# MiRaCLeXeoN/sduss

Hardware: AMD Instinct MI355X
Metric: images/sec (node), SDXL 1024^2 50-step, fixed prompt, CFG (higher is better)
Workload: dtype bf16; 1 GPU; SDXL-base-1.0 UNet 1024x1024 50-step Euler, CFG 5.0, 4 requests/step (denoiser batch 8) per GPU, is_sliced=False, random-init weights of the real architecture (2.57 B params), one data-parallel replica per GPU, no collective; resolution=1024, steps_per_image=50

## Files before the change

include/mxdenoise.h:

```cpp
#ifndef MXDENOISE_H
#define MXDENOISE_H

#include <stddef.h>
#include <stdint.h>

#ifdef __cplusplus
extern "C" {
#endif

enum { MX_F32 = 0, MX_F16 = 1, MX_BF16 = 2 };

const char* mx_last_error(void);
int mx_version(void);
#define MX_PROF_KINDS 12
int mx_profile_enable(int on);
int mx_profile_collect(double* out);
int mx_profile_records(double* out, int max_records);

size_t mx_groupnorm_halo_workspace_bytes(int N, int C, int cpg);
int mx_groupnorm_halo(void* stream, const void* x, const void* gamma, const void* beta, void* y,
                      int N, int C, int H, int W, int cpg, double eps, int padding,
                      const int32_t* latent_offset, int n_latents, const int32_t* patch_map,
                      const int32_t* padding_idx, int dtype, void* workspace);
int mx_halo_only(void* stream, const void* x, void* y, int N, int C, int H, int W,
// ... 67 lines not shown
  const mx_gemm_seg* segs;
  int n_segs;
  int splitk;
  const float* ln_final;
  float* ln_final_out;
  unsigned* ln_final_cnt;
  float* gn_part_out;
  int cin_valid;
} mx_gemm_desc;

int mx_gemm(void* stream, const mx_gemm_desc* d);
int mx_gemm_launches(const mx_gemm_desc* d);
int mx_gemm_stats_slabs(const mx_gemm_desc* d);
int mx_gemm_ln_prefers_pass(const mx_gemm_desc* d);
int mx_gemm_ln_final_supported(const mx_gemm_desc* d);
int mx_gemm_gn_partials_supported(const mx_gemm_desc* d, int conv);
enum { MX_FORM_TILE_GENERIC = 0, MX_FORM_TILE_256 = 1, MX_FORM_TILE_128 = 2, MX_FORM_PERSISTENT_256 = 3, MX_FORM_SMALL_M = 4, MX_FORM_CONV_SMALL_N = 5, MX_FORM_CONV_SMALL_CIN = 6 };
int mx_gemm_form(const mx_gemm_desc* d, int conv);
int mx_gemm_kernel_name(const mx_gemm_desc* d, int conv, int launch, char* buf, int cap);
int mx_gemm_kernel_names(char* buf, int cap);
int mx_attention_kernel_name(int B, int H, int Lq, int Lk, int ldo, int prescaled, int causal, int bias, int key_chunk, int force_cross, char* buf, int cap);
int mx_attention_kernel_names(char* buf, int cap);
#define MX_STATS_PITCH(slabs) (((slabs) + 3) & ~3)
int mx_row_stats(void* stream, const void* x, int ldx, float* stats, int M, int C);
int mx_conv3x3(void* stream, const mx_gemm_desc* d);
int mx_gemm_splitk(const mx_gemm_desc* d, int conv);
void mx_gemm_release_scratch(void* stream, int all);

typedef struct mx_attn_tail_desc {
  mx_gemm_desc out1, to_q, out2;
  const void* k; int ldk;
  const void* vt; int ldvt; int64_t vt_batch_stride;
  int B, heads, L, ctx_len;
  unsigned* sync;
} mx_attn_tail_desc;
size_t mx_attn_tail_sync_bytes(int M);
int mx_attn_tail_supported(const mx_attn_tail_desc* d);
int mx_attn_tail_preferred(void);
int mx_attn_tail(void* stream, const mx_attn_tail_desc* d);
int mx_attn_tail_status(void* stream, const unsigned* sync, unsigned* word);

#define MX_VT_POS(key) (((key) & ~12) | (((key) & 4) << 1) | (((key) & 8) >> 1))
#define MX_VT_LD(Lk) (((Lk) + 15) / 16 * 16)

int mx_attention(void* stream, const void* q, int ldq, const void* k, int ldk, const void* vt, int ldvt,
                 int64_t vt_batch_stride, void* o, int ldo, int B, int H, int Lq, int Lk, float scale);
#define MX_ATTN_QSCALE(scale) ((scale) * 1.4426950408889634f)
int mx_attention_prescaled(void* stream, const void* q, int ldq, const void* k, int ldk, const void* vt, int ldvt,
                           int64_t vt_batch_stride, void* o, int ldo, int B, int H, int Lq, int Lk);
int mx_attention_cross_prescaled(void* stream, const void* q, int ldq, const void* k, int ldk, const void* vt, int ldvt,
                                 int64_t vt_batch_stride, void* o, int ldo, int B, int H, int Lq, int Lk);
typedef struct mx_attn_problem {
  const void* q; const void* k; const void* vt; void* o;
  int64_t vt_batch_stride;
  int B, Lq, Lk, ldvt;
} mx_attn_problem;
int mx_attention_prescaled_grouped(void* stream, const mx_attn_problem* probs, int n, int ldq, int ldk, int ldo, int H);
int mx_attention_prescaled_bias(void* stream, const void* q, int ldq, const void* k, int ldk, const void* vt, int ldvt,
                                int64_t vt_batch_stride, void* o, int ldo, int B, int H, int Lq, int Lk, const float* bias, int ldb);
int mx_attention_prescaled_causal(void* stream, const void* q, int ldq, const void* k, int ldk, const void* vt, int ldvt,
                                  int64_t vt_batch_stride, void* o, int ldo, int B, int H, int L);

int mx_layernorm(void* stream, const void* x, void* y, const float* gamma, const float* beta,
                 int M, int C, float eps);

int mx_rmsnorm(void* stream, const void* x, void* y, const float* w, int M, int C, float eps);

int mx_layernorm_mod(void* stream, const void* x, void* y, void* y2, const float* scale, const float* shift,
                     const float* scale2, const float* shift2, int ldmod, int M, int C, int rows_per_batch, float eps);
int mx_layernorm_mod_grouped(void* stream, const void* x, void* y, void* y2, const float* scale, const float* shift, const float* scale2,
                             const float* shift2, int ldmod, int C, float eps, const int* batches, const int* rows_per_batch, int n);
int mx_rmsnorm_heads(void* stream, void* x, int ld, int nbatch, int rows_per_batch, int batch_rows, int row_off,
                     int heads_total, int heads_q, const float* wq, const float* wk, float eps, float q_scale);

size_t mx_groupnorm_nhwc_workspace_bytes(int B, int H, int W, int C);
int mx_groupnorm_nhwc(void* stream, const void* x, void* y, const float* gamma, const float* beta,
                      int B, int H, int W, int C, int groups, float eps, int silu, int patch,
                      void* workspace);

int mx_groupnorm_nhwc_cat(void* stream, const void* x, int C1, const void* x2, void* y, const float* gamma, const float* beta,
                          int B, int H, int W, int C, int groups, float eps, int silu, int patch, void* workspace);
int mx_groupnorm_nhwc_from_partials(void* stream, const void* x, void* y, const float* gamma, const float* beta, int B, int H, int W, int C, int groups, float eps,
                                    int silu, const float* part, int chunk, const float* add_bias, const float* add_rowbias, int ldrb, void* workspace);

typedef struct mx_gn_problem { const void* x; const void* x2; void* y; int B, H, W; } mx_gn_problem;
size_t mx_groupnorm_nhwc_grouped_workspace_bytes(const mx_gn_problem* probs, int n, int C);
int mx_groupnorm_nhwc_grouped(void* stream, const mx_gn_problem* probs, int n, int C1, const float* gamma, const float* beta, int C, int groups,
                              float eps, int silu, int patch, void* workspace);

typedef struct mx_unet_config {
  int in_channels, out_channels;
  int n_levels;
  int block_out_channels[4];
  int layers_per_block;
  int down_has_attn[4];
  int transformer_layers[4];
  int num_heads[4];
  int cross_attention_dim;
  int addition_time_embed_dim;
  int projection_class_embeddings_input_dim;
  int norm_num_groups;
  float norm_eps, transformer_norm_eps, layer_norm_eps;
} mx_unet_config;

typedef struct mx_weight_entry {
  const char* name;
  uint64_t offset;
  uint64_t bytes;
} mx_weight_entry;

typedef struct mx_unet mx_unet;

mx_unet* mx_unet_create(const mx_unet_config* cfg);
void mx_unet_destroy(mx_unet* u);
int mx_unet_set_weights(mx_unet* u, const void* blob, uint64_t blob_bytes,
                        const mx_weight_entry* table, int n_entries);
int mx_unet_set_context_key(mx_unet* u, uint64_t key);
int mx_unet_context_stats(const mx_unet* u, long* hits, long* misses);
size_t mx_unet_workspace_bytes(const mx_unet* u, int batch, int H, int W, int ctx_len);
int mx_unet_validate(const mx_unet* u, int batch, int H, int W, int ctx_len);
int mx_unet_forward(mx_unet* u, void* stream, const void* latents, int io_dtype, const float* timesteps,
                    const void* ehs, const void* text_embeds, const float* time_ids, void* out,
                    int batch, int H, int W, int ctx_len, int gn_patch, void* workspace, size_t workspace_bytes);
typedef struct mx_unet_group { const void* latents; void* out; int batch, H, W; } mx_unet_group;
size_t mx_unet_workspace_bytes_mixed(const mx_unet* u, const mx_unet_group* groups, int n_groups, int ctx_len);
int mx_unet_forward_mixed(mx_unet* u, void* stream, const mx_unet_group* groups, int n_groups, int io_dtype, const float* timesteps,
                          const void* ehs, const void* text_embeds, const float* time_ids, int ctx_len, int gn_patch, void* workspace,
                          size_t workspace_bytes);
int mx_unet_forward_mixed_trace(mx_unet* u, void* stream, const mx_unet_group* groups, int n_groups, int io_dtype, const float* timesteps,
                                const void* ehs, const void* text_embeds, const float* time_ids, int ctx_len, int gn_patch, void* workspace,
                                size_t workspace_bytes, const char* stage, void* stage_out, size_t stage_out_bytes);
int mx_unet_forward_trace(mx_unet* u, void* stream, const void* latents, int io_dtype, const float* timesteps,
                          const void* ehs, const void* text_embeds, const float* time_ids, void* out,
                          int batch, int H, int W, int ctx_len, int gn_patch, void* workspace,
                          size_t workspace_bytes, const char* stage, void* stage_out, size_t stage_out_bytes);

typedef int (*mx_allgather_fn)(void* ctx, void* stream, const void* send, void* recv, size_t bytes_per_rank);
typedef struct mx_pp_comm { int rank, world; mx_allgather_fn all_gather; void* ctx; } mx_pp_comm;
size_t mx_unet_workspace_bytes_pp(const mx_unet* u, int batch, int H_local, int W, int ctx_len, int world);
int mx_unet_forward_pp(mx_unet* u, void* stream, const void* latents_local, int io_dtype, const float* timesteps, const void* ehs,
                       const void* text_embeds, const float* time_ids, void* out_local, int batch, int H_local, int W, int ctx_len,
                       const mx_pp_comm* comm, void* workspace, size_t workspace_bytes);
#define MX_PP_SYNC 0
#define MX_PP_WARMUP 1
#define MX_PP_STALE 2
typedef int (*mx_allgather_inplace_fn)(void* ctx, void* stream, void* region, size_t bytes_per_rank);
typedef struct mx_pp_stale { void* state; size_t state_bytes; int mode; int corrected_gn; mx_allgather_inplace_fn all_gather_async; } mx_pp_stale;
size_t mx_unet_pp_state_bytes(const mx_unet* u, int batch, int H_local, int W, int ctx_len, int world);
int mx_unet_forward_pp_stale(mx_unet* u, void* stream, const void* latents_local, int io_dtype, const float* timesteps, const void* ehs,
                             const void* text_embeds, const float* time_ids, void* out_local, int batch, int H_local, int W, int ctx_len,
                             const mx_pp_comm* comm, const mx_pp_stale* stale, void* workspace, size_t workspace_bytes);
int mx_unet_pp_comm_plan(const mx_unet* u, int batch, int H_local, int W, int ctx_len, const mx_pp_comm* comm);
int mx_attention_prescaled_chunked(void* stream, const void* q, int ldq, const void* k, int ldk, const void* vt, int ldvt,
                                   int64_t vt_batch_stride, void* o, int ldo, int B, int H, int Lq, int Lk, int key_chunk,
                                   int64_t k_batch_stride, int64_t k_chunk_stride, int64_t vt_chunk_stride);

typedef struct mx_mmdit_config {
  int patch_size, in_channels, out_channels;
  int num_layers;
  int num_attention_heads;
  int joint_attention_dim, pooled_projection_dim, pos_embed_max_size;
  int dual_attention[64];
  float norm_eps;
} mx_mmdit_config;

typedef struct mx_mmdit mx_mmdit;
// ... 124 lines not shown
```

sduss_amd/csrc/gemm_args.h:

```cpp
#pragma once
#include "common.h"
#include "../../include/mxdenoise.h"

namespace mx {

constexpr int kMaxSegs = MX_MAX_SEGS;
struct GemmSeg {
  const bf16_t* a; const bf16_t* a2; void* c; const bf16_t* residual; bf16_t* vt; const float* rowbias; const float* gate;
  const float* ln_stats; float* stats_out;
  int M, tile0, rows_per_batch, ldvt;
  int B, Hin, Win, Hout, Wout;
  int a_batch_rows, a_row_off, c_batch_rows, c_row_off;
};

struct GemmArgs {
  const bf16_t* a;
  const bf16_t* w;
  void* c;
  const float* bias;
  const float* rowbias;
  const bf16_t* residual;
  bf16_t* vt;
  int M, N, K;
  int lda, ldc, ldr, ldrb;
// ... 351 lines not shown
        v[0] += bf16lo_to_f32(r[0]); v[1] += bf16hi_to_f32(r[0]);
        v[2] += bf16lo_to_f32(r[1]); v[3] += bf16hi_to_f32(r[1]);
      }
      if (flags & MX_EPI_SILU) {
#pragma unroll
        for (int q = 0; q < 4; ++q) v[q] = silu_f(v[q]);
      }
      if (flags & MX_EPI_GELU_TANH) {
#pragma unroll
        for (int q = 0; q < 4; ++q) v[q] = gelu_tanh_f(v[q]);
      }
      if (flags & (MX_EPI_GELU | MX_EPI_QUICK_GELU)) {
#pragma unroll
        for (int q = 0; q < 4; ++q) v[q] = (flags & MX_EPI_GELU) ? gelu_fast(v[q]) : quick_gelu_f(v[q]);
      }
      if (qkv) {
        const int nin = n - seg_idx * p.seg;
        if (to_vt) {
          const int key0 = (p.c_batch_rows > 0 ? p.c_row_off : 0) + m - bidx * p.rows_per_batch;
          const int key = MX_VT_POS(key0);
          const int nv = p.N / p.period;
          bf16_t* dst = p.vt + ((long)bidx * nv + (long)seg_grp * p.seg + nin) * p.ldvt + key;
#pragma unroll
          for (int q = 0; q < 4; ++q) dst[(long)q * p.ldvt] = f32_to_bf16(v[q]);
        } else {
          const int ccol = seg_grp * (p.period - 1) * p.seg + seg_pos * p.seg + nin;
          u32x2 o = {pack_bf16x2(v[0], v[1]), pack_bf16x2(v[2], v[3])};
          *reinterpret_cast<u32x2*>(reinterpret_cast<bf16_t*>(p.c) + orow * p.ldc + ccol) = o;
        }
        continue;
      }
      if (flags & MX_EPI_OUT_F32) {
        f32x4 o = {v[0], v[1], v[2], v[3]};
        *reinterpret_cast<f32x4*>(reinterpret_cast<float*>(p.c) + orow * p.ldc + n) = o;
      } else {
        u32x2 o = {pack_bf16x2(v[0], v[1]), pack_bf16x2(v[2], v[3])};
        *reinterpret_cast<u32x2*>(reinterpret_cast<bf16_t*>(p.c) + orow * p.ldc + n) = o;
      }
    }
  }
}


__device__ __forceinline__ void gemm_tile_of_block(const int b, const int mt, const int nt, const int xcd_map, int& tm, int& tn) {
  constexpr int MB = 4;
  if (!xcd_map || (mt & 7) != 0) { tm = b % mt; tn = b / mt; return; }
  const int xcd = b & 7;
  const int local = b >> 3;
  const int mloc = mt >> 3;
  const int band_tiles = MB * nt;
  const int band = local / band_tiles;
  const int r = local - band * band_tiles;
  const int rows = (mloc - band * MB) < MB ? (mloc - band * MB) : MB;
  tn = r / rows;
  tm = ((band * MB + (r - tn * rows)) << 3) + xcd;
}

__device__ __forceinline__ void lane_exchange_pair(float (&a)[4], float (&b)[4]) {
#pragma unroll
  for (int d = 0; d < 4; ++d) {
    unsigned x = __float_as_uint(a[d]), y = __float_as_uint(b[d]);
    auto r = __builtin_amdgcn_permlane32_swap(x, y, false, false);
    auto t = __builtin_amdgcn_permlane16_swap(r[0], r[1], false, false);
    a[d] = __uint_as_float(t[0]);
    b[d] = __uint_as_float(t[1]);
  }
}

__device__ __forceinline__ u32x4 lane_xor1(const u32x4 x) {
  u32x4 r;
#pragma unroll
  for (int d = 0; d < 4; ++d) r[d] = (unsigned)__builtin_amdgcn_update_dpp(0, (int)x[d], 0xB1, 0xF, 0xF, true);
  return r;
}

constexpr int EPI_F_QKV = 1;
constexpr int EPI_F_ACT = 2;
constexpr int EPI_F_ALL = 3;
constexpr int EPI_F_TANH = 4;
__host__ __device__ inline int gemm_epi_features(int flags) {
  const int acts = flags & (MX_EPI_SILU | MX_EPI_GELU | MX_EPI_GELU_TANH | MX_EPI_QUICK_GELU | MX_EPI_GEGLU_TANH);
  return ((flags & MX_EPI_QKV) ? EPI_F_QKV : 0) | (acts == 0 ? 0 : acts == MX_EPI_GELU_TANH ? EPI_F_TANH : EPI_F_ACT);
}
template <int NI, int MI, bool GEGLU, bool VEC = true, bool VPF = true, bool STATS = true, int FEAT = EPI_F_ALL, bool EMIT = STATS, bool RSTD_LOAD = false, bool WT = false>
__device__ __forceinline__ void gemm_epilogue_regs(const GemmArgs& p, f32x4 (&acc)[NI][MI], const int m_wave0, const int wave_n0,
                                                   const int fr, const int fq, const float (&ln_rstd_a)[MI]) {
#pragma clang fp contract(off)
  constexpr int NIO = GEGLU ? NI / 2 : NI;
  constexpr int NP = NIO / 2;
  constexpr bool ODD = (NIO & 1) != 0;
  constexpr int DEPTH = MI <= 4 ? MI : 2;
  static_assert(!GEGLU || NI % 4 == 0, "GEGLU: hidden and gate halves must be whole pairs");
  const int flags = p.flags;
  constexpr bool ACT = (FEAT & EPI_F_ACT) != 0;
  constexpr bool TANH = (FEAT & (EPI_F_ACT | EPI_F_TANH)) != 0;
  const bool qkv = (FEAT & EPI_F_QKV) != 0 && (flags & MX_EPI_QKV) != 0;
  int seg_idx = 0, seg_grp = 0, seg_pos = 0;
  bool to_vt = false;
  if (qkv) {
    seg_idx = wave_n0 / p.seg;
    seg_grp = seg_idx / p.period;
    seg_pos = seg_idx - seg_grp * p.period;
    to_vt = seg_pos == p.period - 1;
  }
  const bool rms = qkv && (flags & MX_EPI_RMSNORM) && !to_vt;
  const float w_scale = (!rms && p.out_scale != 0.f && (!qkv || seg_pos == 0)) ? p.out_scale : 1.0f;
  const int col0 = GEGLU ? wave_n0 / 2 : qkv ? seg_grp * (p.period - 1) * p.seg + seg_pos * p.seg + (wave_n0 - seg_idx * p.seg) : wave_n0;
  const bool has_res = !GEGLU && p.residual != nullptr;
  const bool has_rb = VEC && !GEGLU && p.rowbias != nullptr, has_gate = VEC && !GEGLU && p.gate != nullptr;

  f32x4 bias_r[NI];
#pragma unroll
  for (int i = 0; i < NI; ++i) {
    bias_r[i] = f32x4{0.f, 0.f, 0.f, 0.f};
    if (p.bias && (GEGLU || i < NIO)) bias_r[i] = *reinterpret_cast<const f32x4*>(p.bias + wave_n0 + i * 16 + fq * 4);
  }
  f32x4 rmsw_r[NI];
  if (rms) {
    const float* w = seg_pos == 0 ? p.rms_wq : p.rms_wk;
#pragma unroll
    for (int i = 0; i < NI; ++i) rmsw_r[i] = *reinterpret_cast<const f32x4*>(w + ((wave_n0 - seg_idx * p.seg + i * 16 + fq * 4) & 63));
  }
  const bool stats = EMIT && !GEGLU && !qkv && p.stats_out != nullptr;

  if constexpr ((FEAT & EPI_F_QKV) != 0) {
    if (qkv && to_vt) {
      const int rpb_v = p.rows_per_batch > 0 ? p.rows_per_batch : 0x7fffffff;
      const int m_first = m_wave0 + fr;
      int bv = p.rows_per_batch > 0 ? m_first / p.rows_per_batch : 0;
      int rv = m_first - bv * (p.rows_per_batch > 0 ? p.rows_per_batch : 0);
      const int key_off = p.c_batch_rows > 0 ? p.c_row_off : 0;
      const int nv = p.N / p.period;
      const long feat0 = (long)seg_grp * p.seg + (wave_n0 - seg_idx * p.seg) + fq * 4;
      auto rstd_at = [&](int j) __attribute__((always_inline)) -> float {
        const int m = m_first + 16 * j;
        return p.ln_final[(long)(m < p.M ? m : p.M - 1) * 2 + 1];
      };
      float rs_next = RSTD_LOAD ? rstd_at(0) : 1.0f;
#pragma unroll
      for (int j = 0; j < MI; ++j) {
        const float rs_cur = rs_next;
        if (RSTD_LOAD && j + 1 < MI) rs_next = rstd_at(j + 1);
        if (m_first + 16 * j < p.M) {
          const int key = MX_VT_POS(key_off + rv);
          bf16_t* dst = p.vt + ((long)bv * nv + feat0) * p.ldvt + key;
          const float rs = RSTD_LOAD ? rs_cur : STATS ? ln_rstd_a[j] : 1.0f;
#pragma unroll
          for (int i = 0; i < NIO; ++i) {
            const f32x4 t = STATS ? fma4(acc[i][j], rs, bias_r[i]) : acc[i][j] + bias_r[i];
#pragma unroll
            for (int q = 0; q < 4; ++q) dst[(long)(i * 16 + q) * p.ldvt] = f32_to_bf16(t[q]);
          }
        }
        rv += 16;
        if (rv >= rpb_v) { rv -= rpb_v; ++bv; }
      }
      return;
    }
  }
  const bool odd_lane = (fr & 1) != 0;
  const int rpb = p.rows_per_batch > 0 ? p.rows_per_batch : 0x7fffffff;
  const int cbr = p.c_batch_rows > 0 ? p.c_batch_rows : (p.rows_per_batch > 0 ? p.rows_per_batch : 0);
  const int cro = p.c_batch_rows > 0 ? p.c_row_off : 0;
  const int b_last = p.rows_per_batch > 0 ? (p.M - 1) / p.rows_per_batch : 0;
  const int r_last = p.M - 1 - b_last * (p.rows_per_batch > 0 ? p.rows_per_batch : 0);
  const int row_last = b_last * cbr + cro + r_last;
  const int mA0 = (m_wave0 + fr) & ~1;
  int row_a[MI], row_b[MI];
  int bo_walk = 0, ro_walk = 0;
  {
    int bA = p.rows_per_batch > 0 ? mA0 / p.rows_per_batch : 0;
    int rA = mA0 - bA * (p.rows_per_batch > 0 ? p.rows_per_batch : 0);
#pragma unroll
    for (int j = 0; j < MI; ++j) {
      int bB = bA, rB = rA + 1;
      if (rB >= rpb) { rB = 0; ++bB; }
      const int mA = mA0 + 16 * j;
      row_a[j] = mA < p.M ? bA * cbr + cro + rA : row_last;
      row_b[j] = mA + 1 < p.M ? bB * cbr + cro + rB : row_last;
      if constexpr (VEC) { if (j == 0) { bo_walk = odd_lane ? bB : bA; ro_walk = odd_lane ? rB : rA; } }
      rA += 16;
      if (rA >= rpb) { rA -= rpb; ++bA; }
    }
  }
  auto token = [&](int j) __attribute__((always_inline)) { return m_wave0 + j * 16 + fr; };
  auto row_own = [&](int j) __attribute__((always_inline)) { return odd_lane ? row_b[j] : row_a[j]; };
  const char* const res_base = reinterpret_cast<const char*>(p.residual);
  char* const c_base = reinterpret_cast<char*>(p.c);
  const unsigned ldr_b = (unsigned)p.ldr * 2u, ldc_b = (unsigned)p.ldc * 2u;
  auto res_at = [&](int row, int col) __attribute__((always_inline)) { return res_base + (unsigned long long)(unsigned)row * ldr_b + (unsigned)(col * 2); };
  auto c_at = [&](int row, int col) __attribute__((always_inline)) { return c_base + (unsigned long long)(unsigned)row * ldc_b + (unsigned)(col * 2); };
  const auto c_rsrc = __builtin_amdgcn_make_buffer_rsrc(p.c, 0, WT ? (int)((unsigned)p.M * ldc_b) : 0, 0x00020000);
  auto store_c16 = [&](int row, int col, const u32x4 v) __attribute__((always_inline)) {
    if constexpr (WT) __builtin_amdgcn_raw_buffer_store_b128(v, c_rsrc, (int)((unsigned)row * ldc_b + (unsigned)(col * 2)), 0, 16);
    else *reinterpret_cast<u32x4*>(c_at(row, col)) = v;
  };
  auto store_c8 = [&](int row, int col, const u32x2 v) __attribute__((always_inline)) {
    if constexpr (WT) __builtin_amdgcn_raw_buffer_store_b64(v, c_rsrc, (int)((unsigned)row * ldc_b + (unsigned)(col * 2)), 0, 16);
    else *reinterpret_cast<u32x2*>(c_at(row, col)) = v;
  };

  auto load_res = [&](int j, int pr) __attribute__((always_inline)) -> u32x4 {
    if (!has_res) return u32x4{0u, 0u, 0u, 0u};
    return *reinterpret_cast<const u32x4*>(res_at(row_own(j), col0 + pr * 32 + fq * 8));
  };
  auto load_res_odd = [&](int j) __attribute__((always_inline)) -> u32x2 {
// ... 10 lines not shown
#pragma unroll
      for (int i = 0; i < NIO; ++i) {
        const int n = wave_n0 + i * 16 + fq * 4;
        if (has_rb) rb_r[i] = *reinterpret_cast<const f32x4*>(p.rowbias + (long)bidx * p.ldrb + n);
        if (has_gate) gate_r[i] = *reinterpret_cast<const f32x4*>(p.gate + (long)bidx * p.ldg + n);
      }
    }
  };
  if constexpr (VPF) { if (has_rb || has_gate) load_batch_vectors(0); }
  constexpr int NG = NP / 2;
  constexpr bool fullmode = NG > 0;
  const int col_full = col0 + (odd_lane ? 32 : 0) + fq * 8;
  auto load_res_full = [&](int j, int g, int which) __attribute__((always_inline)) -> u32x4 {
    if (!has_res) return u32x4{0u, 0u, 0u, 0u};
    return *reinterpret_cast<const u32x4*>(res_at(which ? row_b[j] : row_a[j], col_full + 64 * g));
  };
  auto load_res_any = [&](int j, int pr) __attribute__((always_inline)) -> u32x4 {
    if (pr < 2 * NG) return load_res_full(j, pr >> 1, pr & 1);
    return load_res(j, pr);
  };
  u32x4 res_r[DEPTH][NP > 0 ? NP : 1];
  u32x2 res_o[DEPTH];
  {
#pragma unroll
    for (int d = 0; d < DEPTH && d < MI; ++d) {
#pragma unroll
      for (int pr = 0; pr < NP; ++pr) res_r[d][pr] = load_res_any(d, pr);
      if constexpr (ODD) res_o[d] = load_res_odd(d);
    }
  }

  auto rstd_at = [&](int j) __attribute__((always_inline)) -> float {
    const int m = token(j);
    return p.ln_final[(long)(m < p.M ? m : p.M - 1) * 2 + 1];
  };
  float rstd_next = RSTD_LOAD ? rstd_at(0) : 1.0f;
#pragma unroll
  for (int j = 0; j < MI; ++j) {
    const int m = token(j);
    float v[NIO][4];
    float rms_mul = 1.0f;
    if constexpr (!VPF) { if (has_rb || has_gate) load_batch_vectors(j); }
    const float rstd_cur = rstd_next;
    if (RSTD_LOAD && j + 1 < MI) rstd_next = rstd_at(j + 1);
    const float ln_rstd = RSTD_LOAD ? rstd_cur : STATS ? ln_rstd_a[j] : 1.0f;
    float st1 = 0.f, st2 = 0.f;
    if (rms) {
      float ss = 0.f;
#pragma unroll
      for (int i = 0; i < NI; ++i)
#pragma unroll
        for (int q = 0; q < 4; ++q) { const float t = acc[i][j][q] + bias_r[i][q]; ss = fmaf(t, t, ss); }
      ss = sum_over_fq(ss);
      rms_mul = rsqrtf(fmaf(ss, 1.0f / 64.0f, p.rms_eps)) * ((seg_pos == 0 && p.out_scale != 0.f) ? p.out_scale : 1.0f);
    }
#pragma unroll
    for (int i = 0; i < NIO; ++i) {
      f32x4 t = STATS ? fma4(acc[i][j], ln_rstd, bias_r[i]) : acc[i][j] + bias_r[i];
      if constexpr (GEGLU) {
        const f32x4 g = STATS ? fma4(acc[i + NI / 2][j], ln_rstd, bias_r[i + NI / 2]) : acc[i + NI / 2][j] + bias_r[i + NI / 2];
        if (ACT && (flags & MX_EPI_GEGLU_TANH)) {
#pragma unroll
          for (int q = 0; q < 4; ++q) t[q] = t[q] * gelu_tanh_f(g[q]);
        } else {
          const gelu_f32x2 g01 = gelu_fast2(gelu_f32x2{g[0], g[1]}), g23 = gelu_fast2(gelu_f32x2{g[2], g[3]});
          t[0] *= g01[0]; t[1] *= g01[1]; t[2] *= g23[0]; t[3] *= g23[1];
        }
      } else {
        if (rms) {
#pragma unroll
          for (int q = 0; q < 4; ++q) t[q] *= rms_mul * rmsw_r[i][q];
        } else {
          t *= w_scale;
        }
        if constexpr (VEC) {
          if (has_rb) t += rb_r[i];
          if (has_gate) t *= gate_r[i];
        }
      }
#pragma unroll
      for (int q = 0; q < 4; ++q) v[i][q] = t[q];
    }
    if constexpr (VPF) { if (j + 1 < MI && (has_rb || has_gate)) load_batch_vectors(j + 1); }
    auto finish8 = [&](float (&o)[8], const u32x4 rr) __attribute__((always_inline)) {
      if (has_res) {
#pragma unroll
        for (int q = 0; q < 4; ++q) { o[2 * q] += bf16lo_to_f32(rr[q]); o[2 * q + 1] += bf16hi_to_f32(rr[q]); }
      }
      if (ACT && (flags & MX_EPI_SILU)) {
#pragma unroll
        for (int q = 0; q < 8; ++q) o[q] = silu_f(o[q]);
      }
      if (TANH && (flags & MX_EPI_GELU_TANH)) {
#pragma unroll
        for (int q = 0; q < 8; q += 2) { const gelu_f32x2 t2 = gelu_tanh2(gelu_f32x2{o[q], o[q + 1]}); o[q] = t2[0]; o[q + 1] = t2[1]; }
      }
      if (ACT && (flags & (MX_EPI_GELU | MX_EPI_QUICK_GELU))) {
#pragma unroll
        for (int q = 0; q < 8; ++q) o[q] = (flags & MX_EPI_GELU) ? gelu_fast(o[q]) : quick_gelu_f(o[q]);
      }
      if (stats) {
#pragma unroll
        for (int q = 0; q < 8; ++q) { st1 += o[q]; st2 = fmaf(o[q], o[q], st2); }
      }
    };
    if constexpr (fullmode) {
      const bool ok_a = (m & ~1) < p.M, ok_b = (m | 1) < p.M;
#pragma unroll
      for (int g = 0; g < NG; ++g) {
        lane_exchange_pair(v[4 * g], v[4 * g + 1]);
        lane_exchange_pair(v[4 * g + 2], v[4 * g + 3]);
        float oa[8], ob[8];
#pragma unroll
        for (int q = 0; q < 4; ++q) { oa[q] = v[4 * g][q]; oa[4 + q] = v[4 * g + 1][q]; ob[q] = v[4 * g + 2][q]; ob[4 + q] = v[4 * g + 3][q]; }
        const u32x4 ra = res_r[j % DEPTH][2 * g], rb = res_r[j % DEPTH][2 * g + 1];
        if (j + DEPTH < MI) { res_r[j % DEPTH][2 * g] = load_res_full(j + DEPTH, g, 0); res_r[j % DEPTH][2 * g + 1] = load_res_full(j + DEPTH, g, 1); }
        u32x4 res_a = ra, res_b = rb;
        if (has_res) {
          const u32x4 nb_ra = lane_xor1(ra), nb_rb = lane_xor1(rb);
          res_a = odd_lane ? nb_rb : ra;
          res_b = odd_lane ? rb : nb_ra;
        }
        finish8(oa, res_a);
        finish8(ob, res_b);
        const u32x4 wa = {pack_bf16x2(oa[0], oa[1]), pack_bf16x2(oa[2], oa[3]), pack_bf16x2(oa[4], oa[5]), pack_bf16x2(oa[6], oa[7])};
        const u32x4 wb = {pack_bf16x2(ob[0], ob[1]), pack_bf16x2(ob[2], ob[3]), pack_bf16x2(ob[4], ob[5]), pack_bf16x2(ob[6], ob[7])};
        const u32x4 nb_b = lane_xor1(wb), nb_a = lane_xor1(wa);
        const u32x4 st_a = odd_lane ? nb_b : wa;
        const u32x4 st_b = odd_lane ? wb : nb_a;
        if (ok_a) store_c16(row_a[j], col_full + 64 * g, st_a);
        if (ok_b) store_c16(row_b[j], col_full + 64 * g, st_b);
      }
    }
#pragma unroll
    for (int pr = 2 * NG; pr < NP; ++pr) {
      lane_exchange_pair(v[2 * pr], v[2 * pr + 1]);
      float o[8];
#pragma unroll
      for (int q = 0; q < 4; ++q) { o[q] = v[2 * pr][q]; o[4 + q] = v[2 * pr + 1][q]; }
      const u32x4 rr = res_r[j % DEPTH][pr];
      if (j + DEPTH < MI) res_r[j % DEPTH][pr] = load_res(j + DEPTH, pr);
      finish8(o, rr);
      if (m < p.M) {
        const u32x4 w = {pack_bf16x2(o[0], o[1]), pack_bf16x2(o[2], o[3]), pack_bf16x2(o[4], o[5]), pack_bf16x2(o[6], o[7])};
        store_c16(row_own(j), col0 + pr * 32 + fq * 8, w);
      }
    }
    if constexpr (ODD) {
      float o[4];
#pragma unroll
      for (int q = 0; q < 4; ++q) o[q] = v[NIO - 1][q];
      const u32x2 rr = res_o[j % DEPTH];
      if (j + DEPTH < MI) res_o[j % DEPTH] = load_res_odd(j + DEPTH);
      if (has_res) { o[0] += bf16lo_to_f32(rr[0]); o[1] += bf16hi_to_f32(rr[0]); o[2] += bf16lo_to_f32(rr[1]); o[3] += bf16hi_to_f32(rr[1]); }
      if (ACT && (flags & MX_EPI_SILU)) {
#pragma unroll
        for (int q = 0; q < 4; ++q) o[q] = silu_f(o[q]);
      }
      if (TANH && (flags & MX_EPI_GELU_TANH)) {
#pragma unroll
        for (int q = 0; q < 4; q += 2) { const gelu_f32x2 t2 = gelu_tanh2(gelu_f32x2{o[q], o[q + 1]}); o[q] = t2[0]; o[q + 1] = t2[1]; }
      }
      if (ACT && (flags & (MX_EPI_GELU | MX_EPI_QUICK_GELU))) {
#pragma unroll
        for (int q = 0; q < 4; ++q) o[q] = (flags & MX_EPI_GELU) ? gelu_fast(o[q]) : quick_gelu_f(o[q]);
      }
      if (stats) {
#pragma unroll
        for (int q = 0; q < 4; ++q) { st1 += o[q]; st2 = fmaf(o[q], o[q], st2); }
      }
      if (m < p.M) store_c8(row_own(j), col0 + NP * 32 + fq * 4, u32x2{pack_bf16x2(o[0], o[1]), pack_bf16x2(o[2], o[3])});
    }
    if (stats) {
      st1 = sum_over_fq(st1); st2 = sum_over_fq(st2);
      if (fq == 0 && m < p.M) {
        const int slab = wave_n0 / (16 * NI), pitch = (p.N / (16 * NI) + 3) & ~3;
        float* dst = p.stats_out + ((long)m * pitch + slab) * 2;
        if (WT || p.ln_final_out != nullptr) {
          const unsigned long long bits = (unsigned long long)__float_as_uint(st1) | ((unsigned long long)__float_as_uint(st2) << 32);
          __hip_atomic_store(reinterpret_cast<unsigned long long*>(dst), bits, __ATOMIC_RELAXED, __HIP_MEMORY_SCOPE_AGENT);
        } else {
          *reinterpret_cast<f32x2*>(dst) = f32x2{st1, st2};
        }
      }
    }
  }
}

}
```

sduss_amd/csrc/gemm_bf16.hip:

```cpp
#include <algorithm>
#include <cstdlib>

#include <mutex>
#include <unordered_map>

#include "common.h"
#include "../../include/mxdenoise.h"
#include "gemm_args.h"
#include "gemm_forms.h"

namespace mx {

constexpr int BM = 128;
constexpr int BK = 64;

__device__ __forceinline__ int swz(int row, int chunk) { return chunk ^ ((row >> 1) & 7); }

template <int BN, bool CONV>
__global__ __launch_bounds__(256, 2) void gemm_kernel(const GemmArgs pk) {
  constexpr int NI = BN / 32;
  constexpr int MI = 4;
  constexpr int WROWS = BN / 32;
  __shared__ __attribute__((aligned(16))) bf16_t sX[2][BM * BK];
  __shared__ __attribute__((aligned(16))) bf16_t sW[2][BN * BK];
// ... 374 lines not shown
  a.vhalo = conv ? d->vhalo : 0;
  a.a2 = conv ? nullptr : (const bf16_t*)d->a2; a.lda2 = d->lda2; a.k_split = d->k_split;
  a.a = (const bf16_t*)d->a; a.w = (const bf16_t*)d->w; a.c = d->c;
  a.bias = d->bias; a.rowbias = d->rowbias; a.residual = (const bf16_t*)d->residual; a.vt = (bf16_t*)d->vt;
  a.M = d->M; a.N = d->N; a.K = d->K; a.lda = d->lda; a.ldc = d->ldc; a.ldr = d->ldr; a.ldrb = d->ldrb;
  a.rows_per_batch = d->rows_per_batch; a.flags = d->flags; a.seg = d->seg; a.period = d->period; a.ldvt = d->ldvt;
  a.B = d->B; a.Hin = d->Hin; a.Win = d->Win; a.Cin = d->Cin; a.Hout = d->Hout; a.Wout = d->Wout;
  a.stride = d->stride; a.up = d->up; a.corner_patch = d->corner_patch;
  a.a_batch_rows = d->a_batch_rows; a.a_row_off = d->a_row_off; a.c_batch_rows = d->c_batch_rows; a.c_row_off = d->c_row_off;
  a.gate = d->gate; a.ldg = d->ldg; a.out_scale = d->out_scale;
  a.rms_wq = d->rms_wq; a.rms_wk = d->rms_wk; a.rms_eps = d->rms_eps;
  a.ln_stats = d->ln_stats; a.ln_colsum = d->ln_colsum; a.ln_slabs = d->ln_slabs; a.ln_eps = d->ln_eps; a.stats_out = nullptr;
  a.ln_final = nullptr; a.ln_final_out = nullptr; a.ln_final_cnt = nullptr; a.ln_final_slabs = 0;
  if (d->ln_final) {
    MX_CHECK(!conv && !d->ln_stats && d->ln_colsum && d->n_segs == 0, "gemm: ln_final needs ln_colsum, excludes ln_stats and grouped launches (mx_gemm only)");
    MX_CHECK(!(d->flags & MX_EPI_RMSNORM) && d->a_batch_rows <= 0 && d->c_batch_rows <= 0 && !d->a2 && !d->rowbias && !d->gate && !d->stats_out,
             "gemm: ln_final excludes RMSNORM, the row remaps, the split A operand, per-sample vectors and stats_out");
    MX_CHECK((((uintptr_t)d->ln_final & 15) | ((uintptr_t)d->ln_colsum & 15)) == 0, "gemm: ln_final / ln_colsum must be 16-byte aligned");
    a.ln_final = d->ln_final;
  }
  a.nseg = d->n_segs; a.mt_total = 0;
  const bool grouped = d->n_segs > 0;
  if (d->ln_stats) {
    MX_CHECK(!conv && d->ln_colsum && d->ln_slabs > 0, "gemm: folded LayerNorm needs ln_colsum and ln_slabs > 0 (mx_gemm only)");
    MX_CHECK(!(d->flags & MX_EPI_RMSNORM) && d->a_batch_rows <= 0 && d->c_batch_rows <= 0 && !d->a2, "gemm: folded LayerNorm excludes RMSNORM, the row remaps and the split A operand");
    MX_CHECK((((uintptr_t)d->ln_stats & 15) | ((uintptr_t)d->ln_colsum & 15)) == 0, "gemm: ln_stats / ln_colsum must be 16-byte aligned");
  }
  a.xcd_map = 1;

  if (!conv && d->a2) {
    MX_CHECK(d->k_split > 0 && d->k_split < d->K && d->k_split % BK == 0, "gemm: k_split must be a multiple of 64 inside (0, K)");
    MX_CHECK(d->lda >= d->k_split && d->lda % 8 == 0 && d->lda2 >= d->K - d->k_split && d->lda2 % 8 == 0, "gemm: bad lda / lda2 for the split A operand");
    MX_CHECK(d->a_batch_rows <= 0 && ((uintptr_t)d->a2 & 15) == 0 && rows_of(d) * d->lda2 < 2147483647L, "gemm: split A operand excludes the row remap and needs 16-byte alignment");
  } else if (!conv) {
    MX_CHECK(d->lda >= d->K && d->lda % 8 == 0, "gemm: lda must be >= K and a multiple of 8");
  } else {
    MX_CHECK(d->Cin % BK == 0 && d->K == 9 * d->Cin, "conv3x3: Cin must be a multiple of 64 and K = 9*Cin");
    MX_CHECK(d->stride == 1 || d->stride == 2, "conv3x3: stride must be 1 or 2");
    MX_CHECK(d->up == 0 || d->up == 1, "conv3x3: up must be 0 or 1");
    MX_CHECK(!(d->up && d->stride != 1), "conv3x3: upsample only with stride 1");
    if (!grouped) {
      const int Hv = d->Hin << d->up, Wv = d->Win << d->up;
      MX_CHECK(d->Hout == (Hv + d->stride - 1) / d->stride && d->Wout == (Wv + d->stride - 1) / d->stride,
               "conv3x3: output grid does not match input grid / stride");
      MX_CHECK((long)d->B * d->Hout * d->Wout == d->M, "conv3x3: M != B*Hout*Wout");
    }
    MX_CHECK(2 * d->Cin <= 16384, "conv3x3: Cin > 8192 (the pipelined loader walks a 16 KB zero page for padding taps)");
    MX_CHECK(!(d->flags & MX_EPI_GEGLU), "conv3x3: no GEGLU epilogue");
    MX_CHECK(d->vhalo == 0 || (d->vhalo == 1 && d->corner_patch == 0), "conv3x3: vhalo must be 0 or 1 and excludes the sliced corner rule");
  }
  {
    const void* ptrs[] = {d->a, d->w, d->c, d->bias, d->rowbias, d->residual, d->gate, d->rms_wq, d->rms_wk};
    for (const void* q : ptrs) MX_CHECK(((uintptr_t)q & 15) == 0, "gemm: operand pointers must be 16-byte aligned");
  }
  if (!grouped && (d->rowbias || d->gate || d->a_batch_rows > 0 || d->c_batch_rows > 0 || (d->flags & (MX_EPI_QKV | MX_EPI_RES_BCAST))))
    MX_CHECK(d->rows_per_batch > 0, "gemm: rows_per_batch required");
  if (d->gate) MX_CHECK(d->ldg >= d->N && d->ldg % 4 == 0, "gemm: bad ldg");
  if (!grouped && d->a_batch_rows > 0) MX_CHECK(!conv && d->a_row_off >= 0 && d->a_row_off + d->rows_per_batch <= d->a_batch_rows, "gemm: bad input row remap");
  if (!grouped && d->c_batch_rows > 0) MX_CHECK(d->c_row_off >= 0 && d->c_row_off + d->rows_per_batch <= d->c_batch_rows, "gemm: bad output row remap");
  if (d->rowbias) MX_CHECK(d->ldrb >= d->N && d->ldrb % 4 == 0, "gemm: bad ldrb");
  if (!grouped) {
    const long in_rows = (!conv && d->a_batch_rows > 0) ? (long)(d->M / d->rows_per_batch + 1) * d->a_batch_rows : d->M;
    MX_CHECK(in_rows * (conv ? 1 : d->lda) < 2147483647L, "gemm: operand exceeds 32-bit indexing");
  }
  MX_CHECK((long)d->N * d->K < 2147483647L, "gemm: operand exceeds 32-bit indexing");
  if (d->residual) MX_CHECK(d->ldr >= d->N && d->ldr % 4 == 0, "gemm: bad ldr");
  const bool use128 = (d->N % 128 == 0);
  const TileChoice tc = pick_tile(d, conv);
  tc_out = tc;
  a.splitk = 0; a.sk_ws = nullptr; a.sk_cnt = nullptr;
  if (tc.splitk > 1) {
    SplitKScratch sk;
    MX_CHECK(splitk_scratch((hipStream_t)stream, sk), "gemm: the split-K scratch (96 MB per stream) could not be allocated; set mx_gemm_desc.splitk = 1 to run unsplit");
    a.splitk = tc.splitk; a.sk_ws = sk.ws; a.sk_cnt = sk.cnt;
  }
  if (d->stats_out) {
    MX_CHECK(stats_slabs_of(d, conv, tc) > 0, "gemm: stats_out is not supported for this shape / epilogue (see mx_gemm_stats_slabs)");
    MX_CHECK(((uintptr_t)d->stats_out & 15) == 0, "gemm: stats_out must be 16-byte aligned");
    a.stats_out = d->stats_out;
  }
  a.gn_part = nullptr;
  if (d->gn_part_out) {
    MX_CHECK(!grouped && tc.rows == 256 && tc.bn != 256 && tc.bn != 0 && tc.splitk <= 1, "gemm: gn_part_out needs an ungrouped launch on a 256-row tile (mx_gemm_gn_partials_supported)");
    MX_CHECK(d->flags == 0 && !d->residual && !d->gate && d->out_scale == 0.f && !d->ln_stats && !d->ln_final && d->a_batch_rows <= 0 && d->c_batch_rows <= 0,
             "gemm: gn_part_out needs an epilogue of bias (+ row bias) only");
    MX_CHECK(d->M % 64 == 0 && (!d->rowbias || d->rows_per_batch % 64 == 0) && ((uintptr_t)d->gn_part_out & 15) == 0, "gemm: gn_part_out needs M % 64 == 0, rows_per_batch % 64 == 0 and 16-byte alignment");
    a.gn_part = d->gn_part_out;
  }
  if (d->ln_final_out) {
    MX_CHECK(d->stats_out && d->ln_final_cnt && !grouped && tc.rows == 256 && tc.bn != 256 && tc.bn != 0,
             "gemm: ln_final_out needs stats_out, ln_final_cnt and an ungrouped launch on a 256-row tile (mx_gemm_ln_final_supported)");
    MX_CHECK((((uintptr_t)d->ln_final_out & 15) | ((uintptr_t)d->ln_final_cnt & 3)) == 0, "gemm: ln_final_out must be 16-byte aligned");
    a.ln_final_out = d->ln_final_out; a.ln_final_cnt = d->ln_final_cnt; a.ln_final_slabs = stats_slabs_of(d, conv, tc);
  }
  if (grouped) {
    const int rows = tc.rows > 0 ? tc.rows : BM;
    uintptr_t lo = (uintptr_t)d->segs[0].a;
    int t0 = 0;
    for (int i = 0; i < d->n_segs; ++i) {
      const mx_gemm_seg& g = d->segs[i];
      GemmSeg& o = a.prob[i];
      o.a = (const bf16_t*)g.a; o.a2 = conv ? nullptr : (const bf16_t*)g.a2; o.c = g.c; o.residual = (const bf16_t*)g.residual; o.vt = (bf16_t*)g.vt;
      o.rowbias = g.rowbias; o.gate = g.gate; o.ln_stats = g.ln_stats; o.stats_out = d->stats_out ? g.stats_out : nullptr;
      o.M = g.M; o.tile0 = t0; o.rows_per_batch = g.rows_per_batch; o.ldvt = g.ldvt;
      o.B = g.B; o.Hin = g.Hin; o.Win = g.Win; o.Hout = g.Hout; o.Wout = g.Wout;
      o.a_batch_rows = g.a_batch_rows; o.a_row_off = g.a_row_off; o.c_batch_rows = g.c_batch_rows; o.c_row_off = g.c_row_off;
      t0 += cdiv(g.M, rows);
      lo = std::min(lo, (uintptr_t)g.a);
    }
    a.mt_total = t0;
    a.a = (const bf16_t*)lo;
    a.M = (int)rows_of(d);
  }
  if (d->flags & MX_EPI_GEGLU) {
    MX_CHECK(use128, "gemm: GEGLU needs N % 128 == 0");
    MX_CHECK(!(d->flags & (MX_EPI_QKV | MX_EPI_OUT_F32)) && !d->residual && !d->rowbias && d->out_scale == 0.f, "gemm: GEGLU excludes other epilogues");
    MX_CHECK(d->ldc >= d->N / 2 && d->ldc % 4 == 0, "gemm: bad ldc for GEGLU");
  } else if (d->flags & MX_EPI_QKV) {
    MX_CHECK(d->seg > 0 && d->seg % 64 == 0 && d->period >= 2 && d->N % (d->seg * d->period) == 0, "gemm: bad QKV segments");
    MX_CHECK(d->vt != nullptr, "gemm: QKV needs vt");
    if (!grouped) {
      MX_CHECK(d->ldvt >= MX_VT_LD(d->c_batch_rows > 0 ? d->c_batch_rows : d->rows_per_batch), "gemm: QKV needs ldvt >= MX_VT_LD(keys per batch)");
      MX_CHECK(d->M % d->rows_per_batch == 0, "gemm: QKV needs M % rows_per_batch == 0");
    }
    MX_CHECK(d->ldc >= d->N / d->period * (d->period - 1) && d->ldc % 4 == 0, "gemm: bad ldc for QKV");
    MX_CHECK(!(d->flags & MX_EPI_OUT_F32), "gemm: QKV output is bf16");
    MX_CHECK(!d->rowbias && !d->gate && !d->residual, "gemm: QKV excludes the per-sample vectors and the residual (its V^T segment takes none of them)");
    if (d->flags & MX_EPI_RMSNORM)
      MX_CHECK(d->rms_wq && d->rms_wk && d->period == 3 && d->N % 128 == 0 && !conv, "gemm: RMSNORM needs rms_wq/rms_wk, period 3, N % 128 == 0");
  } else {
    MX_CHECK(d->ldc >= d->N && d->ldc % 4 == 0, "gemm: bad ldc");
  }
  return 0;
}

int gemm_prepare_for_chain(void* stream, const mx_gemm_desc* d, GemmArgs& a, int& bn, int& rows, int& splitk) {
  TileChoice tc;
  if (int rc = prepare(stream, d, false, a, tc)) return rc;
  bn = tc.bn; rows = tc.rows; splitk = tc.splitk;
  return 0;
}

static int launch(void* stream, const mx_gemm_desc* d, bool conv) {
  GemmArgs a;
  TileChoice tc;
  if (int rc = prepare(stream, d, conv, a, tc)) return rc;
  const bool grouped = d->n_segs > 0;
  const bool use128 = (d->N % 128 == 0);
  const int v2bn = tc.bn;
  dim3 block(256);
  hipStream_t s = (hipStream_t)stream;
  if (prof_enabled()) {
    const double kk = conv ? 9.0 * d->Cin : (double)d->K;
    const double Mt = (double)rows_of(d);
    double in_elems = conv ? (double)d->B * d->Hin * d->Win * d->Cin : Mt * d->K;
    if (conv && grouped) { in_elems = 0; for (int i = 0; i < d->n_segs; ++i) in_elems += (double)d->segs[i].B * d->segs[i].Hin * d->segs[i].Win * d->Cin; }
    const double flops = 2.0 * Mt * (double)d->N * kk;
    const double bytes = 2.0 * (in_elems + (double)d->N * d->K + Mt * d->N);
    const int kind = v2bn == 256 ? PROF_GEMM_V3_256 : v2bn ? (conv ? PROF_CONV_V2_160 : PROF_GEMM_V2_160) + (v2bn == 160 ? 0 : 2) : (conv ? PROF_CONV128 : PROF_GEMM128) + (use128 ? 0 : 1);
    prof_begin(s, kind, flops, bytes, (int)Mt, d->N, (int)kk);
  }
  const int mt128 = grouped ? a.mt_total : cdiv(d->M, BM);
  if (d->ln_final) MX_CHECK(v2bn == 256, "gemm: ln_final is the 256 x 256 kernel's form of the folded LayerNorm; this shape does not run there (use ln_stats)");
  const int form = gemm_kernel_of(d, conv, tc);
  MX_CHECK(form >= 0, v2bn == 256 ? "gemm: no 256 x 256 instantiation serves ln_final with this epilogue (GEGLU, QKV or plain bias only)"
                                   : "gemm: no kernel instantiation serves this descriptor");
  if (is_small_m_form(form)) {
    MX_CHECK(launch_small_m(s, a, form) == 0, "gemm: the small-M launcher was handed a form outside its list");
// ... 3 lines not shown
    launch_conv_small_cin(s, a);
  } else if (v2bn == 256) {
    MX_CHECK(launch_v4(s, a, form) == 0, "gemm: no 256 x 256 instantiation serves ln_final with this epilogue (GEGLU, QKV or plain bias only)");
  } else if (v2bn) {
    if (tc.rows == 256) MX_CHECK(launch_v5(s, a, v2bn, tc.rows, form) == 0, "gemm: the 256-row launcher was handed a form outside its list");
    else MX_CHECK(launch_v2(s, a, v2bn, form) == 0, "gemm: the 128-row launcher was handed a form outside its list");
  } else {
    const dim3 grid(mt128, use128 ? d->N / 128 : cdiv(d->N, 64));
    switch (form) {
#define MX_GEN(id, k, targs) case id: hipLaunchKernelGGL((k<MX_FORM_UNPAREN targs>), grid, block, 0, s, a); break;
      MX_GEMM_GENERIC_FORMS(MX_GEN)
#undef MX_GEN
      default: MX_CHECK(false, "gemm: the generic launcher was handed a form outside its list");
    }
  }
  prof_end(s);
  MX_LAUNCH_CHECK();
  return 0;
}

}

namespace mx {
static bool tail_split(const mx_gemm_desc* d, mx_gemm_desc& d1, mx_gemm_desc& d2) {
  if (d->n_segs != 0 || d->M <= 0 || d->N <= 0 || d->K <= 0 || d->N % 256 != 0) return false;
  if (d->flags & (MX_EPI_QKV | MX_EPI_OUT_F32 | MX_EPI_RES_BCAST | MX_EPI_RMSNORM)) return false;
  if (d->stats_out || d->ln_stats || d->ln_final || d->ln_final_out || d->a_batch_rows > 0 || d->c_batch_rows > 0 || d->splitk > 1) return false;
  if (pick_tile(d, false).bn != 256) return false;
  const int ncu = cu_count();
  if (ncu <= 0) return false;
  const long mt = cdiv(d->M, 256), nt = d->N / 256, tiles = mt * nt;
  const long full = tiles / ncu, rem = tiles % ncu;
  if (full < 1 || rem == 0 || rem * 2 > ncu || (full * ncu) % mt != 0) return false;
  const long nt1 = full * ncu / mt;
  if (nt1 <= 0 || nt1 >= nt) return false;
  const int N1 = (int)nt1 * 256, N2 = d->N - N1;
  const bool geglu = (d->flags & MX_EPI_GEGLU) != 0;
  const long cofs = geglu ? N1 / 2 : N1;
  d1 = *d; d2 = *d;
  d1.N = N1; d2.N = N2;
  d1.splitk = 1; d2.splitk = 1;
  d2.w = (const char*)d->w + (size_t)N1 * d->K * 2;
  if (d->bias) d2.bias = d->bias + N1;
  d2.c = (char*)d->c + (size_t)cofs * 2;
  if (geglu && d->residual) return false;
  if (d->residual) d2.residual = (const char*)d->residual + (size_t)N1 * 2;
  if (d->rowbias) d2.rowbias = d->rowbias + N1;
  if (d->gate) d2.gate = d->gate + N1;
  const TileChoice t2 = pick_tile(&d2, false);
  if (t2.bn == 0 || t2.bn == 256 || t2.rows + t2.bn > 384) return false;
  if (m_tiles_of(&d2, t2.rows) * (N2 / t2.bn) > ncu) return false;
  return pick_tile(&d1, false).bn == 256;
}
}

extern "C" int mx_gemm(void* stream, const mx_gemm_desc* d) {
  mx_gemm_desc d1, d2;
  if (d != nullptr && mx::tail_split(d, d1, d2)) { if (int rc = mx::launch(stream, &d1, false)) return rc; return mx::launch(stream, &d2, false); }
  return mx::launch(stream, d, false);
}
extern "C" int mx_gemm_launches(const mx_gemm_desc* d) { mx_gemm_desc d1, d2; return d != nullptr && mx::tail_split(d, d1, d2) ? 2 : 1; }
extern "C" int mx_gemm_form(const mx_gemm_desc* d, int conv) {
  if (!d || mx::rows_of(d) <= 0 || d->N <= 0 || d->K <= 0) return MX_FORM_TILE_GENERIC;
  if (mx::small_m_serves(d, conv != 0)) return MX_FORM_SMALL_M;
  if (conv && mx::conv_small_n_serves(d)) return MX_FORM_CONV_SMALL_N;
  if (conv && mx::conv_small_cin_serves(d)) return MX_FORM_CONV_SMALL_CIN;
  const mx::TileChoice tc = mx::pick_tile(d, conv != 0);
  return tc.bn == 256 ? MX_FORM_PERSISTENT_256 : tc.bn == 0 ? MX_FORM_TILE_GENERIC : tc.rows == 256 ? MX_FORM_TILE_256 : MX_FORM_TILE_128;
}
extern "C" int mx_gemm_stats_slabs(const mx_gemm_desc* d) {
  if (!d || mx::rows_of(d) <= 0 || d->N <= 0 || d->K <= 0) return 0;
  mx_gemm_desc q = *d;
  if (!q.stats_out) q.stats_out = reinterpret_cast<float*>(16);
  return mx::stats_slabs_of(&q, false, mx::pick_tile(&q, false));
}
extern "C" int mx_gemm_ln_prefers_pass(const mx_gemm_desc* d) {
  if (!d || mx::rows_of(d) <= 0 || d->N <= 0 || d->K <= 0) return 0;
  mx_gemm_desc plain = *d;
  plain.ln_stats = nullptr; plain.stats_out = nullptr;
  return mx::pick_tile(&plain, false).bn == 256;
}
extern "C" int mx_gemm_gn_partials_supported(const mx_gemm_desc* d, int conv) {
  if (!d || d->n_segs > 0 || d->M <= 0 || d->N <= 0 || d->K <= 0 || d->M % 64 != 0) return 0;
  if (d->flags != 0 || d->residual || d->gate || d->out_scale != 0.f || d->ln_stats || d->ln_final || d->a_batch_rows > 0 || d->c_batch_rows > 0) return 0;
  if (d->rowbias && (d->rows_per_batch <= 0 || d->rows_per_batch % 64 != 0)) return 0;
  const mx::TileChoice tc = mx::pick_tile(d, conv != 0);
  return tc.rows == 256 && tc.bn != 256 && tc.bn != 0 && tc.splitk <= 1;
}
extern "C" int mx_gemm_ln_final_supported(const mx_gemm_desc* d) {
  if (!d || d->n_segs > 0 || d->M <= 0 || d->N <= 0 || d->K <= 0) return 0;
  mx_gemm_desc q = *d;
  if (!q.stats_out) q.stats_out = reinterpret_cast<float*>(16);
  const mx::TileChoice tc = mx::pick_tile(&q, false);
  return tc.rows == 256 && tc.bn != 256 && tc.bn != 0 && mx::stats_slabs_of(&q, false, tc) > 0;
}
extern "C" int mx_conv3x3(void* stream, const mx_gemm_desc* d) { return mx::launch(stream, d, true); }
extern "C" void mx_gemm_release_scratch(void* stream, int all) { mx::splitk_release((hipStream_t)stream, all != 0); }
extern "C" int mx_gemm_splitk(const mx_gemm_desc* d, int conv) {
  if (!d || mx::rows_of(d) <= 0 || d->N <= 0 || d->K <= 0) return 0;
  return mx::pick_tile(d, conv != 0).splitk;
}

namespace mx {
static const char* const kGemmKernelNames[GK_COUNT] = {
  MX_GEMM_GENERIC_FORMS(MX_FORM_NAME_T) MX_GEMM_V2_FORMS(MX_FORM_NAME_T) MX_GEMM_V5_FORMS(MX_FORM_NAME_T) MX_GEMM_V4_FORMS(MX_FORM_NAME_T)
  MX_GEMM_SMALL_M_FORMS(MX_FORM_NAME_T) MX_GEMM_CONV_SMALL_FORMS(MX_FORM_NAME_P)
};
}
extern "C" int mx_gemm_kernel_name(const mx_gemm_desc* d, int conv, int launch, char* buf, int cap) {
  if (!d || mx::rows_of(d) <= 0 || d->N <= 0 || d->K <= 0 || launch < 0) return -1;
  mx_gemm_desc d1, d2;
  const mx_gemm_desc* q = d;
  if (!conv && mx::tail_split(d, d1, d2)) { if (launch > 1) return 0; q = launch == 0 ? &d1 : &d2; }
  else if (launch > 0) return 0;
  const int form = mx::gemm_kernel_of(q, conv != 0, mx::pick_tile(q, conv != 0));
  if (form < 0) return -1;
  return mx::copy_name(mx::kGemmKernelNames[form], buf, cap);
}
extern "C" int mx_gemm_kernel_names(char* buf, int cap) { return mx::join_names(mx::kGemmKernelNames, mx::GK_COUNT, buf, cap); }
```

sduss_amd/csrc/gemm_v5_body.h:

```cpp
#pragma once
#include "common.h"
#include "../../include/mxdenoise.h"
#include "gemm_args.h"
#include "gemm_dma_loader.h"

namespace mx {

constexpr int NSTAGE5 = 3;

#if defined(MX_EXP) && MX_EXP == 8
static __device__ unsigned long long g_v5_stamps[1024 * 2 * 4];
#define MX5_STAMP(slot) do { if (lane == 0 && (wave == 0 || wave == 7) && blockIdx.x < 1024) \
    g_v5_stamps[(blockIdx.x * 2 + (wave == 7)) * 4 + (slot)] = __builtin_amdgcn_s_memrealtime(); } while (0)
#else
#define MX5_STAMP(slot) do {} while (0)
#endif

template <int BN, int MI, bool CONV, int FEAT, bool GEGLU, bool VEC, bool WT = false>
__device__ __forceinline__ void gemm_v5_tile(const GemmArgs& pk, int tm, const int tn, bf16_t* const smem) {
  constexpr int BM5 = 64 * MI;
  constexpr int NI = BN / 32;
  constexpr int LOADS = DmaTile<BN, MI>::LOADS;

  const int tid = threadIdx.x;
  const int lane = tid & 63;
  const int wave = __builtin_amdgcn_readfirstlane(tid >> 6);
  const int wm = wave >> 1;
  const int wn = wave & 1;
  const bool group_b = wave >= 4;
  MX5_STAMP(0);
  GemmArgs p = pk;
  gemm_select_seg(p, pk, tm);
  const int nk = p.K / DMA_BK;
  constexpr bool SPLIT_K = false;
  constexpr int k_first = 0;
#include "gemm_dma_loader.inc"

  const int fr = lane & 15;
  const int fq = lane >> 4;
  unsigned wrd[2], xrd[2];
#pragma unroll
  for (int ks = 0; ks < 2; ++ks) {
    const int wrow = wn * (BN / 2) + fr, xrow = wm * 16 * MI + fr;
    wrd[ks] = (unsigned)(((BM5 * DMA_BK) + wrow * DMA_BK + swz(wrow, ks * 4 + fq) * 8) * 2);
    xrd[ks] = (unsigned)((xrow * DMA_BK + swz(xrow, ks * 4 + fq) * 8) * 2);
  }

  setup_tile();
  issue_group(0); advance_cursor();
  issue_group(1); advance_cursor();
  wait_vmcnt<LOADS>();

  f32x4 acc[NI][MI];
#pragma unroll
  for (int i = 0; i < NI; ++i)
#pragma unroll
    for (int j = 0; j < MI; ++j) acc[i][j] = f32x4{0.f, 0.f, 0.f, 0.f};
  float ln_rstd[MI];
#pragma unroll
  for (int j = 0; j < MI; ++j) ln_rstd[j] = 1.0f;
  if constexpr (!CONV) {
    if (p.ln_stats != nullptr) gemm_ln_init<NI, MI>(p, acc, tm * BM5 + wm * 16 * MI, tn * BN + wn * (BN / 2), fr, fq, ln_rstd);
  }
  MX_BAR();
  if (group_b) MX_BAR();
  MX5_STAMP(1);

  int stage = 0;
  for (int kt = 0; kt < nk; ++kt) {
    const char* sb = reinterpret_cast<const char*>(smem) + stage * (STAGE_ELEMS * 2);
    bf16x8 wf[2][NI], xf[2][MI];
#pragma unroll
    for (int ks = 0; ks < 2; ++ks) {
#pragma unroll
      for (int i = 0; i < NI; ++i) wf[ks][i] = *reinterpret_cast<const bf16x8*>(sb + wrd[ks] + i * (16 * DMA_BK * 2));
#pragma unroll
      for (int j = 0; j < MI; ++j) xf[ks][j] = *reinterpret_cast<const bf16x8*>(sb + xrd[ks] + j * (16 * DMA_BK * 2));
    }
    const int st2 = stage >= 1 ? stage - 1 : NSTAGE5 - 1;
    issue_group(st2);
    advance_cursor();
    wait_vmcnt<LOADS>();
    asm volatile("s_waitcnt lgkmcnt(0)" ::: "memory");
    __builtin_amdgcn_sched_barrier(0);
    MX_BAR();
    __builtin_amdgcn_s_setprio(1);
#pragma unroll
    for (int ks = 0; ks < 2; ++ks)
#pragma unroll
      for (int i = 0; i < NI; ++i)
#pragma unroll
        for (int j = 0; j < MI; ++j) acc[i][j] = __builtin_amdgcn_mfma_f32_16x16x32_bf16(wf[ks][i], xf[ks][j], acc[i][j], 0, 0, 0);
    __builtin_amdgcn_s_setprio(0);
    MX_BAR();
    stage = stage == NSTAGE5 - 1 ? 0 : stage + 1;
  }
  MX5_STAMP(2);
  if (!group_b) MX_BAR();

  const int m0 = tm * BM5, n0 = tn * BN;
  static_assert(!GEGLU || (NI % 4 == 0 && !CONV), "the gated epilogue pairs whole 32-feature halves");
  gemm_epilogue_regs<NI, MI, GEGLU, VEC, true, true, FEAT, true, false, WT>(p, acc, m0 + wm * 16 * MI, n0 + wn * (BN / 2), fr, fq, ln_rstd);
  if constexpr (!GEGLU && FEAT == 0 && MI == 4) {
    if (pk.gn_part != nullptr) gemm_gn_partials<NI, MI>(p, acc, m0 + wm * 16 * MI, n0 + wn * (BN / 2), fr, fq);
  }
  MX5_STAMP(3);
  wait_vmcnt<0>();
  if constexpr (!CONV && !GEGLU && BM5 == 256) {
    if (pk.ln_final_out != nullptr) gemm_ln_finalize(p, tm, pk.N / BN, reinterpret_cast<volatile int*>(smem));
  }
}


}
```

sduss_amd/csrc/norm.hip:

```cpp
#include <cstdlib>

#include "common.h"
#include "../../include/mxdenoise.h"

namespace mx {

struct GnGeom {
  int B, H, W, C;
  int tpr;
  int L;
  int th, tw;
  int tiles_y, tiles_x;
  const bf16_t* x2;
  int C1;
};

struct GnProb {
  GnGeom g;
  const bf16_t* x; bf16_t* y;
  float* part; float* coef;
  float* gpart;
  long y_img;
  int ppb;
  int patch;
};
struct GnGroup {
  GnProb p[MX_MAX_SEGS];
  int blk0[MX_MAX_SEGS + 1];
  int n;
};
__device__ __forceinline__ const GnProb& gn_locate(const GnGroup& G, int& local) {
  local = blockIdx.x;
  int s = 0;
#pragma unroll
  for (int i = 1; i < MX_MAX_SEGS; ++i) if (i < G.n && local >= G.blk0[i]) s = i;
  local -= G.blk0[s];
  return G.p[s];
}

__device__ __forceinline__ const bf16_t* gn_src(const bf16_t* x, const GnGeom& g, long pix, int ch) {
  if (g.x2 == nullptr) return x + pix * g.C + ch;
  return ch < g.C1 ? x + pix * g.C1 + ch : g.x2 + pix * (g.C - g.C1) + (ch - g.C1);
}

__global__ void gn_stats_kernel(const GnGroup G, const int groups) {
  extern __shared__ __attribute__((aligned(16))) float red[];
  const int t = threadIdx.x;
  int local;
  const GnProb& P = gn_locate(G, local);
  const GnGeom& g = P.g;
  const bf16_t* __restrict__ x = P.x;
  float* __restrict__ part = P.part;
  const int ntl = g.tiles_y * g.tiles_x;
  const int b = local / ntl;
  const int tile = local - b * ntl;
  const int ty = tile / g.tiles_x, tx = tile - ty * g.tiles_x;
  const int cv = t % g.tpr;
  const int pl = t / g.tpr;
  float s[8], ss[8];
#pragma unroll
  for (int e = 0; e < 8; ++e) { s[e] = 0.f; ss[e] = 0.f; }
  if (pl < g.L) {
    const int npix = g.th * g.tw;
    for (int pi = pl; pi < npix; pi += g.L) {
      const int py = pi / g.tw, px = pi - py * g.tw;
      const long pix = ((long)b * g.H + ty * g.th + py) * g.W + tx * g.tw + px;
      const u32x4 v = *reinterpret_cast<const u32x4*>(gn_src(x, g, pix, cv * 8));
#pragma unroll
      for (int e = 0; e < 4; ++e) {
        const float lo = bf16lo_to_f32(v[e]), hi = bf16hi_to_f32(v[e]);
        s[2 * e] += lo; ss[2 * e] += lo * lo;
        s[2 * e + 1] += hi; ss[2 * e + 1] += hi * hi;
      }
    }
#pragma unroll
    for (int e = 0; e < 8; ++e) {
      red[((long)pl * g.C + cv * 8 + e) * 2] = s[e];
      red[((long)pl * g.C + cv * 8 + e) * 2 + 1] = ss[e];
    }
  }
  __syncthreads();
  float* __restrict__ gpart = P.gpart;
  float* chs = red + (long)g.L * g.C * 2;
  for (int c = t; c < g.C; c += blockDim.x) {
    float a = 0.f, q = 0.f;
    for (int l = 0; l < g.L; ++l) { a += red[((long)l * g.C + c) * 2]; q += red[((long)l * g.C + c) * 2 + 1]; }
    if (gpart != nullptr) { chs[2 * c] = a; chs[2 * c + 1] = q; continue; }
    float* dst = part + (((long)b * (g.tiles_y * g.tiles_x) + tile) * g.C + c) * 2;
    dst[0] = a; dst[1] = q;
  }
  if (gpart != nullptr) {
    __syncthreads();
    const int cpg = g.C / groups;
    for (int gi = t; gi < groups; gi += blockDim.x) {
      float a = 0.f, q = 0.f;
      for (int i = 0; i < cpg; ++i) { a += chs[(gi * cpg + i) * 2]; q += chs[(gi * cpg + i) * 2 + 1]; }
      *reinterpret_cast<float2*>(gpart + (((long)b * ntl + tile) * groups + gi) * 2) = float2{a, q};
    }
  }
}

__device__ __forceinline__ double wave_sum_d(double v) {
#pragma unroll
  for (int o = 32; o > 0; o >>= 1) v += __shfl_xor(v, o, 64);
  return v;
}

constexpr int kFoldThreads = 256;
__global__ __launch_bounds__(kFoldThreads) void gn_fold_kernel(const GnGroup G, const float* __restrict__ gamma, const float* __restrict__ beta,
                                                               int groups, float eps, const float* __restrict__ add_bias = nullptr,
                                                               const float* __restrict__ add_rowbias = nullptr, int ldrb = 0) {
  int local;
  const GnProb& P = gn_locate(G, local);
  const GnGeom& g = P.g;
  const float* __restrict__ part = P.part;
  float* __restrict__ coef = P.coef;
  const int patch = P.patch;
  const int b = local / groups;
  const int grp = local - b * groups;
  const int cpg = g.C / groups;
  const int ntiles = g.tiles_y * g.tiles_x;
  const int lane = threadIdx.x;
  const int ppy = patch > 0 ? g.H / patch : 1;
  const int ppx = patch > 0 ? g.W / patch : 1;
  const int npatch = ppy * ppx;
  const int tpy = g.tiles_y / ppy, tpx = g.tiles_x / ppx;
  const int nitems = tpy * tpx * cpg;
  const double cnt = (double)tpy * tpx * g.th * g.tw * cpg;
  double acc_mean = 0.0, acc_var = 0.0;
  __shared__ double wsum[kFoldThreads / 64][2];
  for (int pidx = 0; pidx < npatch; ++pidx) {
    const int py = pidx / ppx, px = pidx - py * ppx;
    double s = 0.0, q = 0.0;
    for (int it = lane; it < nitems; it += kFoldThreads) {
      const int tl = it / cpg, c = it - tl * cpg;
      const int iy = tl / tpx, ix = tl - iy * tpx;
      const int tile = (py * tpy + iy) * g.tiles_x + px * tpx + ix;
      const float2 v = *reinterpret_cast<const float2*>(part + (((long)b * ntiles + tile) * g.C + grp * cpg + c) * 2);
      if (add_bias != nullptr) {
        const int chn = grp * cpg + c;
        const double cc = (double)add_bias[chn] + (add_rowbias != nullptr ? (double)add_rowbias[(long)b * ldrb + chn] : 0.0);
        const double npx = (double)(g.th * g.tw);
        s += (double)v.x + npx * cc;
        q += (double)v.y + 2.0 * cc * (double)v.x + npx * cc * cc;
      } else {
        s += (double)v.x;
        q += (double)v.y;
      }
    }
    s = wave_sum_d(s);
    q = wave_sum_d(q);
    __syncthreads();
    if ((lane & 63) == 0) { wsum[lane >> 6][0] = s; wsum[lane >> 6][1] = q; }
    __syncthreads();
    s = (wsum[0][0] + wsum[1][0]) + (wsum[2][0] + wsum[3][0]);
    q = (wsum[0][1] + wsum[1][1]) + (wsum[2][1] + wsum[3][1]);
    const double mean = s / cnt;
    double var = q / cnt - mean * mean;
    if (var < 0.0) var = 0.0;
    acc_mean += mean;
    acc_var += var;
  }
  const double mean = acc_mean / npatch;
  const double rstd = 1.0 / sqrt(acc_var / npatch + (double)eps);
  for (int c = lane; c < cpg; c += kFoldThreads) {
    const int ch = grp * cpg + c;
    const float sc = (float)(rstd * (double)gamma[ch]);
    const float sf = (float)((double)beta[ch] - rstd * (double)gamma[ch] * mean);
    coef[((long)b * g.C + ch) * 2] = sc;
    coef[((long)b * g.C + ch) * 2 + 1] = sf;
  }
}

constexpr int kFoldGroups = 64;
template <bool SILU, bool FOLD>
__global__ void gn_apply_kernel(const GnGroup G, const float* __restrict__ gamma, const float* __restrict__ beta, const int groups, const float eps) {
  const int t = threadIdx.x;
  int local;
  const GnProb& P = gn_locate(G, local);
  const GnGeom& g = P.g;
  const bf16_t* __restrict__ x = P.x;
  bf16_t* __restrict__ y = P.y;
  const float* __restrict__ coef = P.coef;
  const int pix_per_block = P.ppb;
  const long y_img = P.y_img;
  const int nblk = (g.H * g.W + pix_per_block - 1) / pix_per_block;
  const int b = local / nblk;
  const int pblk = local - b * nblk;
  const int cv = t % g.tpr;
  const int pl = t / g.tpr;
  float sc[8], sf[8];
  if constexpr (FOLD) {
    __shared__ double fsub[kFoldGroups][8][2];
    __shared__ double mr[kFoldGroups][2];
    const int ntl = g.tiles_y * g.tiles_x;
    const float* __restrict__ gp = P.gpart + (long)b * ntl * groups * 2;
    for (int it = t; it < groups * 8; it += blockDim.x) {
      const int gi = it >> 3, sub = it & 7;
      double s = 0.0, q = 0.0;
      for (int tl = sub; tl < ntl; tl += 8) {
        const float2 v = *reinterpret_cast<const float2*>(gp + ((long)tl * groups + gi) * 2);
        s += (double)v.x; q += (double)v.y;
      }
      fsub[gi][sub][0] = s; fsub[gi][sub][1] = q;
    }
    __syncthreads();
    const int cpg = g.C / groups;
    const double cnt = (double)g.H * g.W * cpg;
    for (int gi = t; gi < groups; gi += blockDim.x) {
      double s = 0.0, q = 0.0;
#pragma unroll
      for (int sub = 0; sub < 8; ++sub) { s += fsub[gi][sub][0]; q += fsub[gi][sub][1]; }
      const double mean = s / cnt;
      double var = q / cnt - mean * mean;
      if (var < 0.0) var = 0.0;
      mr[gi][0] = mean;
      mr[gi][1] = 1.0 / sqrt(var + (double)eps);
    }
    __syncthreads();
    if (pl >= g.L) return;
#pragma unroll
    for (int e = 0; e < 8; ++e) {
      const int ch = cv * 8 + e;
      const int gi = ch / cpg;
      const double rg = mr[gi][1] * (double)gamma[ch];
      sc[e] = (float)rg;
      sf[e] = (float)((double)beta[ch] - rg * mr[gi][0]);
    }
  } else {
    if (pl >= g.L) return;
// ... 37 lines not shown
__global__ __launch_bounds__(64) void gn_pp_coef_kernel(const double* __restrict__ all_sums, const float* __restrict__ gamma,
                                                        const float* __restrict__ beta, float* __restrict__ coef, int B, int C,
                                                        int groups, int world, double cnt, float eps,
                                                        const double* __restrict__ fresh_own, int own_rank) {
  const int grp = blockIdx.x, b = blockIdx.y, lane = threadIdx.x;
  const int cpg = C / groups;
  double s = 0.0, q = 0.0;
  for (int r = 0; r < world; ++r) {
    s += all_sums[(((long)r * B + b) * groups + grp) * 2];
    q += all_sums[(((long)r * B + b) * groups + grp) * 2 + 1];
  }
  double var_fallback = 0.0;
  if (fresh_own) {
    const long o = (((long)own_rank * B + b) * groups + grp) * 2, f = ((long)b * groups + grp) * 2;
    s += (double)world * (fresh_own[f] - all_sums[o]);
    q += (double)world * (fresh_own[f + 1] - all_sums[o + 1]);
    const double lc = cnt / world, lm = fresh_own[f] / lc;
    var_fallback = fresh_own[f + 1] / lc - lm * lm;
    if (var_fallback < 0.0) var_fallback = 0.0;
  }
  const double mean = s / cnt;
  double var = q / cnt - mean * mean;
  if (var < 0.0) var = var_fallback;
  const double rstd = 1.0 / sqrt(var + (double)eps);
  for (int c = lane; c < cpg; c += 64) {
    const int ch = grp * cpg + c;
    coef[((long)b * C + ch) * 2] = (float)(rstd * (double)gamma[ch]);
    coef[((long)b * C + ch) * 2 + 1] = (float)((double)beta[ch] - rstd * (double)gamma[ch] * mean);
  }
}

static int gn_geom(GnGeom& g, int B, int H, int W, int C, int patch) {
  MX_CHECK(C % 8 == 0 && C / 8 <= 1024, "groupnorm: C must be a multiple of 8 and <= 8192");
  g.B = B; g.H = H; g.W = W; g.C = C;
  g.x2 = nullptr; g.C1 = C;
  g.tpr = C / 8;
  g.L = 1024 / g.tpr;
  if (g.L > 32) g.L = 32;
  constexpr int tile_pix = 256;
  int tw = (patch > 0) ? patch : W;
  int th = tile_pix / tw; if (th < 1) th = 1;
  const int hlim = (patch > 0) ? patch : H;
  while (hlim % th != 0) --th;
  while (th > 1 && th * tw >= 64 && (long)B * (H / th) * (W / tw) < 2L * cu_count()) { th /= 2; while (hlim % th != 0) --th; }
  g.th = th; g.tw = tw;
  if (patch > 0) MX_CHECK(H % patch == 0 && W % patch == 0, "groupnorm: H, W must be multiples of patch");
  g.tiles_y = H / th; g.tiles_x = W / tw;
  return 0;
}

}

namespace mx {
size_t gn_workspace_exact(int B, int H, int W, int C, int patch) {
  GnGeom g;
  if (patch >= H && patch >= W) patch = 0;
  if (gn_geom(g, B, H, W, C, patch)) return 0;
  return ((size_t)B * g.tiles_y * g.tiles_x * C * 2 + (size_t)B * C * 2) * sizeof(float);
}
}

extern "C" size_t mx_groupnorm_nhwc_workspace_bytes(int B, int H, int W, int C) {
  const size_t tiles = (size_t)H * W / 4 + 1;
  return ((size_t)B * tiles * C * 2 + (size_t)B * C * 2) * sizeof(float) + 256;
}

extern "C" int mx_groupnorm_nhwc(void* stream, const void* x, void* y, const float* gamma, const float* beta,
                                 int B, int H, int W, int C, int groups, float eps, int silu, int patch,
                                 void* workspace) {
  return mx_groupnorm_nhwc_cat(stream, x, C, nullptr, y, gamma, beta, B, H, W, C, groups, eps, silu, patch, workspace);
}

namespace mx {
static size_t gn_fill(GnGroup& G, int i, const void* x, int C1, const void* x2, void* y, long y_img, int B, int H, int W, int C, int patch, char* ws) {
  GnProb& P = G.p[i];
  if (patch >= H && patch >= W) patch = 0;
  if (patch != 0 && patch < 2) { set_error("groupnorm: patch must be 0 or >= 2"); return 0; }
  if (gn_geom(P.g, B, H, W, C, patch)) return 0;
  if (x2) { P.g.x2 = (const bf16_t*)x2; P.g.C1 = C1; }
  const size_t ntiles = (size_t)P.g.tiles_y * P.g.tiles_x;
  P.x = (const bf16_t*)x; P.y = (bf16_t*)y; P.y_img = y_img; P.patch = patch;
  P.part = (float*)ws;
  P.gpart = nullptr;
  P.coef = P.part + (size_t)B * ntiles * C * 2;
  const int hw = H * W;
  P.ppb = P.g.L * 8 > hw ? hw : P.g.L * 8;
  return (((size_t)B * ntiles * C * 2 + (size_t)B * C * 2) * sizeof(float) + 255) & ~(size_t)255;
}
static void gn_prefix(GnGroup& G, int which, int groups) {
  long t = 0;
  for (int i = 0; i < G.n; ++i) {
    G.blk0[i] = (int)t;
    const GnGeom& g = G.p[i].g;
    t += which == 0 ? (long)g.B * g.tiles_y * g.tiles_x : which == 1 ? (long)g.B * groups : (long)g.B * cdiv(g.H * g.W, G.p[i].ppb);
  }
  for (int i = G.n; i <= MX_MAX_SEGS; ++i) G.blk0[i] = (int)t;
}
static int gn_launch_stats(hipStream_t s, GnGroup& G, int C, int groups = 0) {
  const GnGeom& g = G.p[0].g;
  const int threads = ((g.tpr * g.L + 63) / 64) * 64;
  const size_t smem = ((size_t)g.L * C * 2 + (groups > 0 ? (size_t)C * 2 : 0)) * sizeof(float);
  MX_CHECK(smem <= 160 * 1024, "groupnorm: LDS budget exceeded");
  gn_prefix(G, 0, 0);
  hipLaunchKernelGGL(gn_stats_kernel, dim3(G.blk0[MX_MAX_SEGS]), dim3(threads), smem, s, G, groups);
  MX_LAUNCH_CHECK();
  return 0;
}
static int gn_launch_apply(hipStream_t s, GnGroup& G, int silu, bool fold = false, const float* gamma = nullptr, const float* beta = nullptr, int groups = 0, float eps = 0.f) {
  const GnGeom& g = G.p[0].g;
  const int threads = ((g.tpr * g.L + 63) / 64) * 64;
  gn_prefix(G, 2, 0);
  const dim3 grid(G.blk0[MX_MAX_SEGS]), block(threads);
  if (fold) {
    if (silu) hipLaunchKernelGGL((gn_apply_kernel<true, true>), grid, block, 0, s, G, gamma, beta, groups, eps);
    else hipLaunchKernelGGL((gn_apply_kernel<false, true>), grid, block, 0, s, G, gamma, beta, groups, eps);
  } else {
    if (silu) hipLaunchKernelGGL((gn_apply_kernel<true, false>), grid, block, 0, s, G, gamma, beta, groups, eps);
    else hipLaunchKernelGGL((gn_apply_kernel<false, false>), grid, block, 0, s, G, gamma, beta, groups, eps);
  }
  MX_LAUNCH_CHECK();
  return 0;
}
static bool gn_fold_in_apply() {
  static const bool on = [] { const char* e = getenv("MX_GN_FOLD"); return !(e && e[0] == '0'); }();
  return on;
}
}

extern "C" size_t mx_groupnorm_nhwc_grouped_workspace_bytes(const mx_gn_problem* probs, int n, int C) {
  size_t t = 0;
  for (int i = 0; probs && i < n; ++i) t += mx_groupnorm_nhwc_workspace_bytes(probs[i].B, probs[i].H, probs[i].W, C);
  return t;
}

extern "C" int mx_groupnorm_nhwc_grouped(void* stream, const mx_gn_problem* probs, int n, int C1, const float* gamma, const float* beta, int C,
                                         int groups, float eps, int silu, int patch, void* workspace) {
  using namespace mx;
  MX_CHECK(probs && n >= 1 && n <= MX_MAX_SEGS && gamma && beta && workspace, "groupnorm: grouped launch needs 1..MX_MAX_SEGS problems and its operands");
  MX_CHECK(groups > 0 && C % groups == 0, "groupnorm: C % groups != 0");
  GnGroup G;
  G.n = n;
  char* ws = (char*)workspace;
  double bytes = 0;
  for (int i = 0; i < n; ++i) {
    const mx_gn_problem& q = probs[i];
    MX_CHECK(q.x && q.y && q.B > 0 && q.H > 0 && q.W > 0, "groupnorm: null operand / empty problem");
    MX_CHECK(q.x2 == nullptr || (C1 > 0 && C1 < C && C1 % 8 == 0 && (C - C1) % 8 == 0), "groupnorm: bad channel split");
    MX_CHECK((q.x2 != nullptr) == (probs[0].x2 != nullptr), "groupnorm: grouped launch: either every problem reads a channel concatenation or none");
    const size_t used = gn_fill(G, i, q.x, C1, q.x2, q.y, (long)q.H * q.W * C, q.B, q.H, q.W, C, patch, ws);
    if (!used) return 1;
    MX_CHECK(used <= mx_groupnorm_nhwc_workspace_bytes(q.B, q.H, q.W, C), "groupnorm: internal workspace bound exceeded");
    ws += mx_groupnorm_nhwc_workspace_bytes(q.B, q.H, q.W, C);
    bytes += 3.0 * 2.0 * q.B * q.H * (double)q.W * C;
  }
  hipStream_t s = (hipStream_t)stream;
  prof_begin(s, PROF_NORM, 0.0, bytes);
  bool fold = gn_fold_in_apply() && groups <= kFoldGroups;
  for (int i = 0; i < n; ++i) fold = fold && G.p[i].patch == 0;
  if (fold) {
    for (int i = 0; i < n; ++i) G.p[i].gpart = G.p[i].part;
    if (gn_launch_stats(s, G, C, groups)) return 1;
    if (gn_launch_apply(s, G, silu, true, gamma, beta, groups, eps)) return 1;
    prof_end(s);
    return 0;
  }
  if (gn_launch_stats(s, G, C)) return 1;
  gn_prefix(G, 1, groups);
  hipLaunchKernelGGL(gn_fold_kernel, dim3(G.blk0[MX_MAX_SEGS]), dim3(kFoldThreads), 0, s, G, gamma, beta, groups, eps);
  MX_LAUNCH_CHECK();
  if (gn_launch_apply(s, G, silu)) return 1;
  prof_end(s);
  return 0;
}

extern "C" int mx_groupnorm_nhwc_cat(void* stream, const void* x, int C1, const void* x2, void* y, const float* gamma, const float* beta,
                                     int B, int H, int W, int C, int groups, float eps, int silu, int patch,
                                     void* workspace) {
  mx_gn_problem q;
  q.x = x; q.x2 = x2; q.y = y; q.B = B; q.H = H; q.W = W;
  return mx_groupnorm_nhwc_grouped(stream, &q, 1, C1, gamma, beta, C, groups, eps, silu, patch, workspace);
}

extern "C" int mx_groupnorm_nhwc_from_partials(void* stream, const void* x, void* y, const float* gamma, const float* beta, int B, int H, int W, int C, int groups,
                                               float eps, int silu, const float* part, int chunk, const float* add_bias, const float* add_rowbias, int ldrb,
                                               void* workspace) {
  using namespace mx;
  MX_CHECK(x && y && gamma && beta && part && workspace && B > 0 && H > 0 && W > 0, "groupnorm: null operand / empty problem");
  MX_CHECK(groups > 0 && C % groups == 0 && chunk > 0 && (H * W) % chunk == 0 && ((uintptr_t)part & 15) == 0, "groupnorm: bad groups / chunk / alignment");
  GnGroup G;
  G.n = 1;
  if (!gn_fill(G, 0, x, C, nullptr, y, (long)H * W * C, B, H, W, C, 0, (char*)workspace)) return 1;
  GnGroup F = G;
  F.p[0].part = const_cast<float*>(part);
  F.p[0].g.tiles_y = H * W / chunk; F.p[0].g.tiles_x = 1; F.p[0].g.th = chunk; F.p[0].g.tw = 1;
  hipStream_t s = (hipStream_t)stream;
  prof_begin(s, PROF_NORM, 0.0, 2.0 * 2.0 * B * H * (double)W * C);
  gn_prefix(F, 1, groups);
  MX_CHECK(add_rowbias == nullptr || (add_bias != nullptr && ldrb >= C), "groupnorm: add_rowbias needs add_bias and ldrb >= C");
  hipLaunchKernelGGL(gn_fold_kernel, dim3(F.blk0[MX_MAX_SEGS]), dim3(kFoldThreads), 0, s, F, gamma, beta, groups, eps, add_bias, add_rowbias, ldrb);
  MX_LAUNCH_CHECK();
  if (gn_launch_apply(s, G, silu)) return 1;
  prof_end(s);
  return 0;
}

namespace mx {
int launch_gn_pp_partial(hipStream_t s, const void* x, int C1, const void* x2, int B, int H, int W, int C, int groups, void* workspace, double* sums) {
  GnGroup G;
  G.n = 1;
  if (!gn_fill(G, 0, x, C1, x2, nullptr, 0, B, H, W, C, 0, (char*)workspace)) return 1;
  if (gn_launch_stats(s, G, C)) return 1;
  hipLaunchKernelGGL(gn_pp_sums_kernel, dim3(groups, B), dim3(64), 0, s, (const float*)G.p[0].part, sums, G.p[0].g, groups);
  MX_LAUNCH_CHECK();
  return 0;
}
int launch_gn_pp_finish(hipStream_t s, const void* x, int C1, const void* x2, void* y, long y_img_elems, const float* gamma, const float* beta, const double* all_sums,
                        int world, int B, int H, int W, int C, int groups, int H_total, float eps, int silu, void* workspace,
                        const double* fresh_own, int own_rank) {
  GnGroup G;
  G.n = 1;
  if (!gn_fill(G, 0, x, C1, x2, y, y_img_elems, B, H, W, C, 0, (char*)workspace)) return 1;
  const double cnt = (double)H_total * W * (C / groups);
  hipLaunchKernelGGL(gn_pp_coef_kernel, dim3(groups, B), dim3(64), 0, s, all_sums, gamma, beta, G.p[0].coef, B, C, groups, world, cnt, eps, fresh_own, own_rank);
  return gn_launch_apply(s, G, silu);
}
}

namespace mx {

template <int VPL>
__global__ __launch_bounds__(256) void layernorm_kernel(const bf16_t* __restrict__ x, bf16_t* __restrict__ y,
                                                        const float* __restrict__ gamma,
                                                        const float* __restrict__ beta, int M, int C, float eps) {
  const int lane = threadIdx.x & 63;
  const int row = blockIdx.x * 4 + (threadIdx.x >> 6);
  if (row >= M) return;
  const int nch = C / 8;
  const bf16_t* xr = x + (long)row * C;
  float v[VPL][8];
  float sum = 0.f;
#pragma unroll
  for (int i = 0; i < VPL; ++i) {
    const int ch = lane + 64 * i;
    if (ch < nch) {
      const u32x4 u = *reinterpret_cast<const u32x4*>(xr + ch * 8);
#pragma unroll
      for (int e = 0; e < 4; ++e) {
        v[i][2 * e] = bf16lo_to_f32(u[e]);
        v[i][2 * e + 1] = bf16hi_to_f32(u[e]);
        sum += v[i][2 * e] + v[i][2 * e + 1];
      }
    } else {
#pragma unroll
      for (int e = 0; e < 8; ++e) v[i][e] = 0.f;
    }
  }
  const float mean = wave_sum(sum) / (float)C;
  float sq = 0.f;
#pragma unroll
  for (int i = 0; i < VPL; ++i) {
    const int ch = lane + 64 * i;
    if (ch < nch) {
#pragma unroll
      for (int e = 0; e < 8; ++e) { const float d = v[i][e] - mean; sq += d * d; }
    }
  }
  const float rstd = rsqrtf(wave_sum(sq) / (float)C + eps);
  bf16_t* yr = y + (long)row * C;
#pragma unroll
  for (int i = 0; i < VPL; ++i) {
    const int ch = lane + 64 * i;
    if (ch < nch) {
      const f32x4 one4 = {1.f, 1.f, 1.f, 1.f}, zero4 = {0.f, 0.f, 0.f, 0.f};
      const f32x4 g0 = gamma ? *reinterpret_cast<const f32x4*>(gamma + ch * 8) : one4;
      const f32x4 g1 = gamma ? *reinterpret_cast<const f32x4*>(gamma + ch * 8 + 4) : one4;
      const f32x4 b0 = gamma ? *reinterpret_cast<const f32x4*>(beta + ch * 8) : zero4;
      const f32x4 b1 = gamma ? *reinterpret_cast<const f32x4*>(beta + ch * 8 + 4) : zero4;
      float o[8];
#pragma unroll
      for (int e = 0; e < 4; ++e) {
        o[e] = (v[i][e] - mean) * rstd * g0[e] + b0[e];
        o[e + 4] = (v[i][e + 4] - mean) * rstd * g1[e] + b1[e];
      }
      u32x4 u = {pack_bf16x2(o[0], o[1]), pack_bf16x2(o[2], o[3]), pack_bf16x2(o[4], o[5]), pack_bf16x2(o[6], o[7])};
      *reinterpret_cast<u32x4*>(yr + ch * 8) = u;
    }
// ... 278 lines not shown
```

sduss_amd/csrc/unet_sdxl.cpp:

```cpp
#include <hip/hip_runtime.h>

#include <algorithm>
#include <cstring>
#include <functional>
#include <map>
#include <string>
#include <vector>

#include "../../include/mxdenoise.h"
#include "common.h"
#include "graph_cache.h"
#include "patch_cache.h"
#include "plan_base.h"

namespace mx {
int launch_prep_latent(hipStream_t s, const void* in, int dtype, void* out, int B, int Cin, int HW, int CP);
int launch_nhwc_to_nchw(hipStream_t s, const void* in, void* out, int dtype, int B, int C, int HW, int ld);
int launch_time_embed(hipStream_t s, const float* timesteps, const void* text_embeds, const float* time_ids,
                      void* tsin, void* addin, int B, int d0, int text_dim, int da);
int launch_concat(hipStream_t s, const void* a, const void* b, void* out, long M, int C1, int C2);
size_t gn_workspace_exact(int B, int H, int W, int C, int patch);
int launch_sq_diff_partial(hipStream_t s, const void* a, const void* b, long elems_per_sample, int B, double* partial, const int* slot = nullptr);
int launch_gn_pp_partial(hipStream_t s, const void* x, int C1, const void* x2, int B, int H, int W, int C, int groups, void* workspace, double* sums);
int launch_gn_pp_finish(hipStream_t s, const void* x, int C1, const void* x2, void* y, long y_img_elems, const float* gamma, const float* beta, const double* all_sums,
                        int world, int B, int H, int W, int C, int groups, int H_total, float eps, int silu, void* workspace,
                        const double* fresh_own = nullptr, int own_rank = 0);
}
extern "C" int mx_attention_prescaled_chunked(void* stream, const void* q, int ldq, const void* k, int ldk, const void* vt, int ldvt,
                                              int64_t vt_batch_stride, void* o, int ldo, int B, int H, int Lq, int Lk, int key_chunk,
                                              int64_t k_batch_stride, int64_t k_chunk_stride, int64_t vt_chunk_stride);

using mx::bf16_t;

struct mx_unet {
  mx_unet_config cfg;
  mx::WeightTable weights;
  mx::GraphCache graphs;
  std::map<std::vector<long>, std::vector<size_t>> pp_sizes;
  struct CtxEntry {
    uint64_t key = 0; int B = 0, ctx_len = 0; bool valid = false; uint64_t stamp = 0;
    std::vector<bf16_t*> k, vt; std::vector<size_t> k_bytes, vt_bytes;
    hipEvent_t ev = nullptr; hipStream_t last = nullptr; bool recorded = false;
  };
  uint64_t ctx_key = 0;
  std::vector<CtxEntry> ctx_store;
  uint64_t ctx_clock = 0;
  long ctx_hits = 0, ctx_misses = 0;
  void ctx_clear() {
    for (auto& e : ctx_store) {
      if (e.last) (void)hipStreamSynchronize(e.last);
      for (auto* q : e.k) if (q) (void)hipFree(q);
      for (auto* q : e.vt) if (q) (void)hipFree(q);
      if (e.ev) (void)hipEventDestroy(e.ev);
    }
    ctx_store.clear();
  }
  ~mx_unet() { ctx_clear(); }
};

namespace {

constexpr int kConvInPad = 64;

static std::vector<std::pair<int, int>> kv_widths(const mx_unet_config& c) {
  const int nlev = c.n_levels;
  std::vector<std::pair<int, int>> widths;
  auto add = [&](int dim, int n) { for (auto& wv : widths) if (wv.first == dim) { wv.second += n; return; } widths.push_back({dim, n}); };
  for (int i = 0; i < nlev; ++i) if (c.down_has_attn[i]) add(c.block_out_channels[i], c.layers_per_block * c.transformer_layers[i]);
  add(c.block_out_channels[nlev - 1], c.transformer_layers[nlev - 1]);
  for (int i = 0; i < nlev; ++i) { const int lv = nlev - 1 - i; if (c.down_has_attn[lv]) add(c.block_out_channels[lv], (c.layers_per_block + 1) * c.transformer_layers[lv]); }
  return widths;
}

struct Plan : mx::DenoiserPlan {
  mx_unet* u;
  int ctx_len, gn_patch;
  int ch[MX_MAX_SEGS], cw[MX_MAX_SEGS];
  long rows() const { long m = 0; for (int g = 0; g < ng; ++g) m += (long)gB[g] * ch[g] * cw[g]; return m; }
  long row0(int g) const { long m = 0; for (int k = 0; k < g; ++k) m += (long)gB[k] * ch[k] * cw[k]; return m; }
  char* bc_top = nullptr;
  std::vector<int> bc_sel;
  static constexpr int kBcTables = 2;
  static int bc_part_rows(int lpb) { return lpb + 2; }
  static size_t bc_scratch_bytes(int lpb, int rows) { return bc_head_bytes(bc_part_rows(lpb), kBcTables, rows); }
  int* bc_dsel() const { return bc_table(bc_part_rows(u->cfg.layers_per_block), 1); }
  bool pc = false;
  int pc_p0 = 0, pc_np = 0, pc_nask = 0, pc_maxh = 0, pc_maxw = 0, pc_slots = 0;
  bool pc_partial = false;
  std::vector<mx::PcSample> pc_samp;
// ... 183 lines not shown
    const int slabs = mx_gemm_stats_slabs(&d);
    if (finalise) {
      if (slabs <= 0 || !mx_gemm_ln_final_supported(&d) || (d.M + 255) / 256 > kLnCnt) return fail("finalised row statistics: the producing launch cannot write them");
      d.ln_final_out = st.fin; d.ln_final_cnt = st.cnt; d.ln_eps = u->cfg.layer_norm_eps;
    }
    if (slabs > 0) { d.stats_out = st.buf; st.slabs = slabs; return gemm(d, false); }
    st.slabs = 1;
    if (!gemm(d, false)) return false;
    if (!quiet() && mx_row_stats(stream, d.c, d.ldc, st.buf, d.M, d.N)) return fail(std::string("row_stats: ") + mx_last_error());
    return true;
  }
  void use_ln(mx_gemm_desc& d, const RowStats& st, const std::string& csname, bool final = false) {
    if (final) d.ln_final = st.fin; else { d.ln_stats = st.buf; d.ln_slabs = st.slabs; }
    d.ln_colsum = wf(csname, d.N); d.ln_eps = u->cfg.layer_norm_eps;
  }
  bool linear(const bf16_t* a, int lda, const std::string& wname, const std::string& bname, void* c, int ldc, int M, int N,
              int K, const void* residual = nullptr, int ldr = 0, int flags = 0, float out_scale = 0.f, const bf16_t* a2 = nullptr, int lda2 = 0,
              const RowStats* ln = nullptr, RowStats* stats_out = nullptr, bool ln_final = false, bool finalise = false) {
    mx_gemm_desc d; std::memset(&d, 0, sizeof(d));
    d.out_scale = out_scale;
    if (a2) { d.a2 = a2; d.lda2 = lda2; d.k_split = lda; }
    d.a = a; d.lda = lda; d.w = wb(wname, (size_t)N * K); d.bias = bname.empty() ? nullptr : wf(bname, N);
    d.c = c; d.ldc = ldc; d.M = M; d.N = N; d.K = K; d.residual = residual; d.ldr = ldr; d.flags = flags;
    if (ln) use_ln(d, *ln, wname.substr(0, wname.size() - 6) + "colsum", ln_final);
    if (stats_out) return gemm_with_stats(d, *stats_out, finalise);
    return gemm(d, false);
  }
  int conv_cin_valid = 0;
  bool conv(const bf16_t* x, int Hin, int Win, int Cin, const std::string& prefix, bf16_t* out, int Cout, int stride, int up,
            int corner_patch, const float* rowbias = nullptr, int ldrb = 0, const void* residual = nullptr, int vhalo = 0, float* gn_part = nullptr,
            bool* gn_done = nullptr) {
    mx_gemm_desc d; std::memset(&d, 0, sizeof(d));
    d.vhalo = vhalo;
    const int Hv = Hin << up, Wv = Win << up;
    d.a = x; d.w = wb(prefix + ".weight", (size_t)Cout * 9 * Cin); d.bias = wf(prefix + ".bias", Cout);
    d.c = out; d.ldc = Cout; d.B = gB[0]; d.Hin = Hin; d.Win = Win; d.Cin = Cin;
    d.Hout = (Hv + stride - 1) / stride; d.Wout = (Wv + stride - 1) / stride; d.stride = stride; d.up = up;
    d.corner_patch = corner_patch;
    d.M = gB[0] * d.Hout * d.Wout; d.N = Cout; d.K = 9 * Cin;
    d.rowbias = rowbias; d.ldrb = ldrb; d.rows_per_batch = d.Hout * d.Wout;
    d.residual = residual; d.ldr = Cout;
    mx_gemm_seg sg[MX_MAX_SEGS];
    if (ng > 1) {
      std::memset(sg, 0, sizeof(sg));
      long in0 = 0, out0 = 0;
      for (int g = 0; g < ng; ++g) {
        mx_gemm_seg& q = sg[g];
        q.B = gB[g]; q.Hin = ch[g]; q.Win = cw[g];
        q.Hout = ((ch[g] << up) + stride - 1) / stride; q.Wout = ((cw[g] << up) + stride - 1) / stride;
        q.M = gB[g] * q.Hout * q.Wout; q.rows_per_batch = q.Hout * q.Wout;
        q.a = x + in0 * Cin; q.c = out + out0 * Cout;
        q.residual = residual ? (const bf16_t*)residual + out0 * Cout : nullptr;
        q.rowbias = rowbias ? rowbias + (long)gb0[g] * ldrb : nullptr;
        in0 += (long)gB[g] * ch[g] * cw[g]; out0 += q.M;
      }
      d.segs = sg; d.n_segs = ng;
    }
    if (gn_part && gn_done && ng == 1 && mx_gemm_gn_partials_supported(&d, 1)) { d.gn_part_out = gn_part; *gn_done = true; }
    d.cin_valid = conv_cin_valid;
    return gemm(d, true);
  }
  bool groupnorm(const bf16_t* x, bf16_t* y, const std::string& prefix, int h, int wd, int C, float eps, bool silu, int patch,
                 const bf16_t* x2 = nullptr, int C1 = 0) {
    if (!ok()) return false;
    const size_t m = ar.mark();
    mx_gn_problem pr[MX_MAX_SEGS];
    long r0 = 0;
    for (int k = 0; k < ng; ++k) {
      pr[k].x = x + r0 * (x2 ? C1 : C); pr[k].x2 = x2 ? x2 + r0 * (C - C1) : nullptr; pr[k].y = y + r0 * C;
      pr[k].B = gB[k]; pr[k].H = ch[k]; pr[k].W = cw[k];
      r0 += (long)gB[k] * ch[k] * cw[k];
    }
    const size_t need = ng > 1 ? mx_groupnorm_nhwc_grouped_workspace_bytes(pr, ng, C) : mx::gn_workspace_exact(gB[0], h, wd, C, patch);
    void* ws = ar.alloc(need);
    if (!ws) return fail("workspace too small");
    const float* g = wf(prefix + ".weight", C); const float* b = wf(prefix + ".bias", C);
    if (ok() && !quiet()) {
      if (mx_groupnorm_nhwc_grouped(stream, pr, ng, x2 ? C1 : C, g, b, C, u->cfg.norm_num_groups, eps, silu ? 1 : 0, patch, ws))
        fail(std::string("groupnorm: ") + mx_last_error());
    }
    ar.release(m);
    return ok();
  }
  bool groupnorm_from_partials(const bf16_t* x, bf16_t* y, const std::string& prefix, int h, int wd, int C, float eps, bool silu, const float* part,
                               const float* add_bias, const float* add_rowbias, int ldrb) {
    if (!ok()) return false;
    const size_t m = ar.mark();
    void* ws = ar.alloc(mx::gn_workspace_exact(gB[0], h, wd, C, 0));
    if (!ws) return fail("workspace too small");
    const float* g = wf(prefix + ".weight", C); const float* b = wf(prefix + ".bias", C);
    if (ok() && !quiet()) {
      if (mx_groupnorm_nhwc_from_partials(stream, x, y, g, b, gB[0], h, wd, C, u->cfg.norm_num_groups, eps, silu ? 1 : 0, part, 64, add_bias, add_rowbias, ldrb, ws))
        fail(std::string("groupnorm: ") + mx_last_error());
    }
    ar.release(m);
    return ok();
  }
  bool attention(const bf16_t* q, int ldq, const bf16_t* k, int ldk, const bf16_t* vt, int ldvt, long vt_bstride, bf16_t* o,
                 int ldo, int heads, int Lq, int Lk) {
    if (!ok()) return false;
    if (quiet()) return true;
    if (mx_attention_prescaled(stream, q, ldq, k, ldk, vt, ldvt, vt_bstride, o, ldo, B, heads, Lq, Lk))
      return fail(std::string("attention: ") + mx_last_error());
    return true;
  }
  bool attention_grouped(const mx_attn_problem* pr, int ldq, int ldk, int ldo, int heads) {
    if (!ok()) return false;
    if (quiet()) return true;
    if (mx_attention_prescaled_grouped(stream, pr, ng, ldq, ldk, ldo, heads)) return fail(std::string("attention: ") + mx_last_error());
    return true;
  }
  int level_patch(int level) const { return gn_patch > 0 ? std::max(gn_patch >> level, 1) : 0; }

  bf16_t* resnet(const std::string& p, const bf16_t* x, int h, int wd, int Cin, int Cout, int level, const bf16_t* x2 = nullptr, int C2 = 0) {
    const int M = (int)rows();
    const int C1 = Cin - C2;
    bf16_t* out = alloc<bf16_t>((size_t)M * Cout);
    const size_t m = ar.mark();
    const int patch = level_patch(level);
    if (is_pp()) {
      bf16_t* n1p = alloc_padded(h, wd, Cin);
      groupnorm_pp(x, interior(n1p, wd, Cin), (long)(h + 2) * wd * Cin, p + ".norm1", h, wd, Cin, u->cfg.norm_eps, true, level, x2, C1);
      halo_exchange(n1p, h, wd, Cin);
      bf16_t* h1 = alloc<bf16_t>((size_t)M * Cout);
      conv(n1p, h, wd, Cin, p + ".conv1", h1, Cout, 1, 0, 0, temb_all ? temb_all + temb_off : nullptr, temb_total, nullptr, 1);
      temb_off += Cout;
      bf16_t* n2p = alloc_padded(h, wd, Cout);
      groupnorm_pp(h1, interior(n2p, wd, Cout), (long)(h + 2) * wd * Cout, p + ".norm2", h, wd, Cout, u->cfg.norm_eps, true, level);
      halo_exchange(n2p, h, wd, Cout);
      const bf16_t* sc = x;
      if (Cin != Cout) {
        bf16_t* s2 = alloc<bf16_t>((size_t)M * Cout);
        if (x2) linear(x, C1, p + ".conv_shortcut.weight", p + ".conv_shortcut.bias", s2, Cout, M, Cout, Cin, nullptr, 0, 0, 0.f, x2, C2);
        else linear(x, Cin, p + ".conv_shortcut.weight", p + ".conv_shortcut.bias", s2, Cout, M, Cout, Cin);
        sc = s2;
      }
      conv(n2p, h, wd, Cout, p + ".conv2", out, Cout, 1, 0, 0, nullptr, 0, sc, 1);
      ar.release(m);
      dump(p, out, (size_t)M * Cout);
      return out;
    }
    if (pc) {
      bf16_t* n1 = alloc<bf16_t>((size_t)M * Cin);
      groupnorm(x, n1, p + ".norm1", h, wd, Cin, u->cfg.norm_eps, true, patch, x2, C1);
      bf16_t* h1 = alloc<bf16_t>((size_t)M * Cout);
      pc_conv(n1, h, wd, Cin, p + ".conv1", h1, Cout, 1, 0, patch, level, temb_all ? temb_all + temb_off : nullptr, temb_total, nullptr);
      temb_off += Cout;
      bf16_t* n2 = alloc<bf16_t>((size_t)M * Cout);
      groupnorm(h1, n2, p + ".norm2", h, wd, Cout, u->cfg.norm_eps, true, patch);
      const bf16_t* sc = x;
      if (Cin != Cout) {
        bf16_t* s2 = alloc<bf16_t>((size_t)M * Cout);
        if (x2) linear(x, C1, p + ".conv_shortcut.weight", p + ".conv_shortcut.bias", s2, Cout, M, Cout, Cin, nullptr, 0, 0, 0.f, x2, C2);
        else linear(x, Cin, p + ".conv_shortcut.weight", p + ".conv_shortcut.bias", s2, Cout, M, Cout, Cin);
        sc = s2;
      }
      pc_conv(n2, h, wd, Cout, p + ".conv2", out, Cout, 1, 0, patch, level, nullptr, 0, sc);
      ar.release(m);
      dump(p, out, (size_t)M * Cout);
      return out;
    }
    bf16_t* n1 = alloc<bf16_t>((size_t)M * Cin);
    groupnorm(x, n1, p + ".norm1", h, wd, Cin, u->cfg.norm_eps, true, patch, x2, C1);
    bf16_t* h1 = alloc<bf16_t>((size_t)M * Cout);
    float* gpart = nullptr;
    bool gdone = false;
    if (ng == 1 && patch == 0 && M % 64 == 0 && (h * wd) % 64 == 0) gpart = (float*)ar.alloc((size_t)(M / 64) * Cout * 2 * sizeof(float));
    conv(n1, h, wd, Cin, p + ".conv1", h1, Cout, 1, 0, patch, temb_all ? temb_all + temb_off : nullptr, temb_total, nullptr, 0, gpart, &gdone);
    temb_off += Cout;
    bf16_t* n2 = alloc<bf16_t>((size_t)M * Cout);
    if (gdone) groupnorm_from_partials(h1, n2, p + ".norm2", h, wd, Cout, u->cfg.norm_eps, true, gpart, wf(p + ".conv1.bias", Cout),
                                       temb_all ? temb_all + (temb_off - Cout) : nullptr, temb_total);
    else groupnorm(h1, n2, p + ".norm2", h, wd, Cout, u->cfg.norm_eps, true, patch);
    const bf16_t* sc = x;
    if (Cin != Cout) {
      bf16_t* s2 = alloc<bf16_t>((size_t)M * Cout);
      if (x2) linear(x, C1, p + ".conv_shortcut.weight", p + ".conv_shortcut.bias", s2, Cout, M, Cout, Cin, nullptr, 0, 0, 0.f, x2, C2);
      else linear(x, Cin, p + ".conv_shortcut.weight", p + ".conv_shortcut.bias", s2, Cout, M, Cout, Cin);
      sc = s2;
    }
    conv(n2, h, wd, Cout, p + ".conv2", out, Cout, 1, 0, patch, nullptr, 0, sc);
    ar.release(m);
    dump(p, out, (size_t)M * Cout);
    return out;
  }

  KV* kv_for(int dim) {
    for (auto& k : kv) if (k.dim == dim) return &k;
    return nullptr;
  }

  bf16_t* transformer(const std::string& p, const bf16_t* x, int h, int wd, int C, int heads, int layers, int level) {
    const int L = h * wd;
    const int M = (int)rows();
    const int ctx = u->cfg.cross_attention_dim;
    int gL[MX_MAX_SEGS], gldvt[MX_MAX_SEGS]; long gr0[MX_MAX_SEGS], gvt0[MX_MAX_SEGS], vt_elems = 0;
    for (int g = 0; g < ng; ++g) {
      gL[g] = ch[g] * cw[g]; gldvt[g] = MX_VT_LD(gL[g]); gr0[g] = row0(g); gvt0[g] = vt_elems;
      vt_elems += (long)gB[g] * C * gldvt[g];
    }
    bf16_t* out = alloc<bf16_t>((size_t)M * C);
    const size_t m0 = ar.mark();
    bf16_t* n = alloc<bf16_t>((size_t)M * C);
    if (is_pp()) groupnorm_pp(x, n, (long)L * C, p + ".norm", h, wd, C, u->cfg.transformer_norm_eps, false, level);
    else groupnorm(x, n, p + ".norm", h, wd, C, u->cfg.transformer_norm_eps, false, level_patch(level));
    bf16_t* y = alloc<bf16_t>((size_t)M * C);
    RowStats st;
    st.buf = (float*)ar.alloc((size_t)M * MX_STATS_PITCH(C / 64) * 2 * sizeof(float));
    if (!st.buf) fail("workspace too small");
    bf16_t* ln = n;
    const int ldvt = MX_VT_LD(L);
    bf16_t* qk = alloc<bf16_t>((size_t)M * 2 * C);
    bf16_t* vt = alloc<bf16_t>((size_t)vt_elems);
    bf16_t* ao = alloc<bf16_t>((size_t)M * C);
    bf16_t* q2 = alloc<bf16_t>((size_t)M * C);
    bf16_t* ff = alloc<bf16_t>((size_t)M * 4 * C);
    mx_gemm_seg qsegs[MX_MAX_SEGS];
    auto qkv_desc = [&](const std::string& b, const bf16_t* a) {
      mx_gemm_desc d; std::memset(&d, 0, sizeof(d));
      d.a = a; d.lda = C; d.w = wb(b + ".attn1.to_qkv.weight", (size_t)3 * C * C); d.bias = wf(b + ".attn1.to_qkv.bias", 3 * C);
      d.c = qk; d.ldc = 2 * C;
      d.M = M; d.N = 3 * C; d.K = C; d.flags = MX_EPI_QKV; d.seg = C; d.period = 3; d.vt = vt; d.ldvt = ldvt;
      d.rows_per_batch = L; d.out_scale = MX_ATTN_QSCALE(0.125f);
      if (ng > 1) {
        std::memset(qsegs, 0, sizeof(qsegs));
        for (int g = 0; g < ng; ++g) {
          qsegs[g].a = a + gr0[g] * C; qsegs[g].c = qk + gr0[g] * 2 * C; qsegs[g].vt = vt + gvt0[g];
          qsegs[g].M = gB[g] * gL[g]; qsegs[g].rows_per_batch = gL[g]; qsegs[g].ldvt = gldvt[g];
        }
        d.segs = qsegs; d.n_segs = ng;
      }
      return d;
    };
    auto use_ln_grouped = [&](mx_gemm_desc& d, const RowStats& st_) {
      if (d.n_segs > 0) for (int g = 0; g < ng; ++g) qsegs[g].ln_stats = st_.buf + gr0[g] * MX_STATS_PITCH(st_.slabs) * 2;
    };
    auto lin_desc = [&](const bf16_t* a, void* c, int ldc, int N, int flags, float out_scale) {
      mx_gemm_desc d; std::memset(&d, 0, sizeof(d));
      d.a = a; d.lda = C; d.w = a; d.c = c; d.ldc = ldc; d.M = M; d.N = N; d.K = C; d.flags = flags; d.out_scale = out_scale;
      return d;
    };
    bool pass1, pass2, pass3;
    {
      mx_gemm_desc d1 = qkv_desc(p + ".transformer_blocks.0", y);
      mx_gemm_desc d2 = lin_desc(y, q2, C, C, 0, MX_ATTN_QSCALE(0.125f));
      mx_gemm_desc d3 = lin_desc(y, ff, 4 * C, 8 * C, MX_EPI_GEGLU, 0.f);
      pass1 = mx_gemm_ln_prefers_pass(&d1) != 0; pass2 = mx_gemm_ln_prefers_pass(&d2) != 0; pass3 = mx_gemm_ln_prefers_pass(&d3) != 0;
    }
    const bool pass3_shape = pass3;
    bool fin1 = false, fin3 = false;
    if (!is_pp() && ln_cnt != nullptr && (M + 255) / 256 <= kLnCnt) {
      auto can_finalise = [&](int K, bool residual) {
        mx_gemm_desc d = lin_desc(y, y, C, C, 0, 0.f);
        d.K = K; d.lda = K; if (residual) { d.residual = y; d.ldr = C; }
        return mx_gemm_ln_final_supported(&d) != 0;
      };
      fin1 = ng == 1 && pass1 && can_finalise(C, false) && (layers == 1 || can_finalise(4 * C, true));
      fin3 = pass3 && can_finalise(C, true);
      if (pc) fin3 = false;
      if (fin1 || fin3 || (pc && pass3_shape)) { st.fin = (float*)ar.alloc((size_t)M * 2 * sizeof(float)); st.cnt = ln_cnt; if (!st.fin) fail("workspace too small"); }
    }
    const bool pc_fin3 = pc && pass3_shape && st.fin != nullptr;
    if (fin1) pass1 = false;
    if (fin3) pass3 = false;
    bool tail = mx_attn_tail_preferred() != 0 && !pc && !is_pp() && ng == 1 && !pass2 && tail_sync != nullptr && M <= tail_rows && L % 256 == 0;
    if (getenv("MX_ATTN_TAIL_DEBUG") && !quiet())
      fprintf(stderr, "[mx attn_tail] transformer %s: tail %d (pc %d pp %d ng %d pass2 %d sync %p M %d rows %ld L %d)\n", p.c_str(), (int)tail, (int)pc, (int)is_pp(), ng,
              (int)pass2, (void*)tail_sync, M, tail_rows, L);
    bf16_t* ao2 = nullptr;
    RowStats stA;
    if (tail) {
      ao2 = alloc<bf16_t>((size_t)M * C);
      stA.buf = (float*)ar.alloc((size_t)M * MX_STATS_PITCH(C / 64) * 2 * sizeof(float));
      if (!stA.buf) fail("workspace too small");
    }
    bf16_t* pqc = nullptr; bf16_t* paoc = nullptr; bf16_t* ptc = nullptr;
    if (pc) { pqc = alloc<bf16_t>((size_t)M * C); paoc = alloc<bf16_t>((size_t)M * C); ptc = alloc<bf16_t>((size_t)M * C); }
    auto normalise = [&]() {
      if (ok() && !quiet() && mx_layernorm(stream, y, ln, nullptr, nullptr, M, C, u->cfg.layer_norm_eps)) fail(std::string("layernorm: ") + mx_last_error());
    };
    linear(n, C, p + ".proj_in.weight", p + ".proj_in.bias", y, C, M, C, C, nullptr, 0, 0, 0.f, nullptr, 0, nullptr, pass1 ? nullptr : &st, false, fin1);
    bf16_t* k_send = nullptr; bf16_t* k_all = nullptr; bf16_t* vt_all = nullptr;
    if (is_pp()) {
      if (L % 64 != 0) fail("patch-parallel: local tokens per image must be a multiple of 64 at every attention level");
      k_send = alloc<bf16_t>((size_t)M * C);
      k_all = alloc<bf16_t>((size_t)pp_world * M * C);
      vt_all = alloc<bf16_t>((size_t)pp_world * B * C * ldvt);
    }
// ... 85 lines not shown
        mx_gemm_desc d = qkv_desc(b, pass1 ? ln : y);
        if (!pass1) { use_ln(d, st, b + ".attn1.to_qkv.colsum", fin1); if (!fin1) use_ln_grouped(d, st); } else wf(b + ".attn1.to_qkv.colsum", 3 * C);
        gemm(d, false);
      }
      if (is_pp()) {
        if (ok() && !dry && hipMemcpy2DAsync(k_send, (size_t)C * 2, qk + C, (size_t)2 * C * 2, (size_t)C * 2, M, hipMemcpyDeviceToDevice, stream) != hipSuccess)
          fail("patch-parallel: K pack failed");
        all_gather(k_send, k_all, (size_t)M * C * 2);
        all_gather(vt, vt_all, (size_t)B * C * ldvt * 2);
        if (ok() && !dry &&
            mx_attention_prescaled_chunked(stream, qk, 2 * C, k_all, C, vt_all, ldvt, (int64_t)C * ldvt, ao, C, B, heads, L, pp_world * L, L,
                                           (int64_t)L * C, (int64_t)M * C, (int64_t)B * C * ldvt))
          fail(std::string("attention: ") + mx_last_error());
      } else if (ng > 1) {
        mx_attn_problem pr[MX_MAX_SEGS];
        for (int g = 0; g < ng; ++g) {
          pr[g].q = qk + gr0[g] * 2 * C; pr[g].k = qk + gr0[g] * 2 * C + C; pr[g].vt = vt + gvt0[g]; pr[g].o = ao + gr0[g] * C;
          pr[g].vt_batch_stride = (int64_t)C * gldvt[g]; pr[g].B = gB[g]; pr[g].Lq = gL[g]; pr[g].Lk = gL[g]; pr[g].ldvt = gldvt[g];
        }
        attention_grouped(pr, 2 * C, 2 * C, C, heads);
      } else {
        attention(qk, 2 * C, qk + C, 2 * C, vt, ldvt, (long)C * ldvt, ao, C, heads, L, L);
      }
      bool chained = false;
      if (tail && ok()) {
        auto lin_d = [&](const bf16_t* a_, const std::string& stem, void* c_, const void* res) {
          mx_gemm_desc d; std::memset(&d, 0, sizeof(d));
          d.a = a_; d.lda = C; d.w = wb(stem + ".weight", (size_t)C * C); d.bias = wf(stem + ".bias", C); d.c = c_; d.ldc = C; d.M = M; d.N = C; d.K = C;
          d.residual = res; d.ldr = res ? C : 0;
          return d;
        };
        mx_attn_tail_desc td; std::memset(&td, 0, sizeof(td));
        td.out1 = lin_d(ao, b + ".attn1.to_out.0", y, y);
        td.out1.stats_out = stA.buf;
        const int slabs = mx_gemm_stats_slabs(&td.out1);
        td.to_q = lin_d(y, b + ".attn2.to_q", q2, nullptr);
        td.to_q.out_scale = MX_ATTN_QSCALE(0.125f);
        td.to_q.ln_stats = stA.buf; td.to_q.ln_slabs = slabs; td.to_q.ln_colsum = wf(b + ".attn2.to_q.colsum", C); td.to_q.ln_eps = u->cfg.layer_norm_eps;
        td.out2 = lin_d(ao2, b + ".attn2.to_out.0", y, y);
        if (!pass3) {
          td.out2.stats_out = st.buf;
          if (fin3) { td.out2.ln_final_out = st.fin; td.out2.ln_final_cnt = st.cnt; td.out2.ln_eps = u->cfg.layer_norm_eps; }
        }
        const int li = kvp->next;
        td.k = kvp->k + (size_t)li * C; td.ldk = kvp->ldk; td.vt = kvp->vt + (size_t)li * C * kvp->ldvt; td.ldvt = kvp->ldvt; td.vt_batch_stride = kvp->vt_bstride;
        td.B = B; td.heads = heads; td.L = L; td.ctx_len = ctx_len; td.sync = tail_sync;
        if (ok() && slabs > 0 && (quiet() || mx_attn_tail_supported(&td) != 0)) {
          chained = true;
          ++kvp->next;
          if (!pass3) st.slabs = slabs;
          if (!quiet() && mx_attn_tail(stream, &td)) fail(std::string("attn_tail: ") + mx_last_error());
        } else {
          if (getenv("MX_ATTN_TAIL_DEBUG")) fprintf(stderr, "[mx attn_tail] layer %s: slabs %d -> separate launches\n", b.c_str(), slabs);
          tail = false;
        }
      }
      if (!chained) {
        linear(ao, C, b + ".attn1.to_out.0.weight", b + ".attn1.to_out.0.bias", y, C, M, C, C, y, C, 0, 0.f, nullptr, 0, nullptr, pass2 ? nullptr : &st);
        if (pass2) normalise();
        linear(pass2 ? ln : y, C, b + ".attn2.to_q.weight", b + ".attn2.to_q.bias", q2, C, M, C, C, nullptr, 0, 0, MX_ATTN_QSCALE(0.125f), nullptr, 0,
               pass2 ? nullptr : &st);
        if (ok()) {
          const int li = kvp->next++;
          if (ng > 1) {
            mx_attn_problem pr[MX_MAX_SEGS];
            for (int g = 0; g < ng; ++g) {
              pr[g].q = q2 + gr0[g] * C; pr[g].k = kvp->k + (size_t)li * C + (size_t)gb0[g] * ctx_len * kvp->ldk;
              pr[g].vt = kvp->vt + (size_t)li * C * kvp->ldvt + (size_t)gb0[g] * kvp->vt_bstride; pr[g].o = ao + gr0[g] * C;
              pr[g].vt_batch_stride = kvp->vt_bstride; pr[g].B = gB[g]; pr[g].Lq = gL[g]; pr[g].Lk = ctx_len; pr[g].ldvt = kvp->ldvt;
            }
            attention_grouped(pr, C, kvp->ldk, C, heads);
          } else
          attention(q2, C, kvp->k + (size_t)li * C, kvp->ldk, kvp->vt + (size_t)li * C * kvp->ldvt, kvp->ldvt, kvp->vt_bstride,
                    ao, C, heads, L, ctx_len);
        }
        linear(ao, C, b + ".attn2.to_out.0.weight", b + ".attn2.to_out.0.bias", y, C, M, C, C, y, C, 0, 0.f, nullptr, 0, nullptr, pass3 ? nullptr : &st, false, fin3);
      }
      if (pass3) normalise();
      linear(pass3 ? ln : y, C, b + ".ff.net.0.proj.weight", b + ".ff.net.0.proj.bias", ff, 4 * C, M, 8 * C, C, nullptr, 0, MX_EPI_GEGLU, 0.f, nullptr, 0,
             pass3 ? nullptr : &st, nullptr, fin3);
      linear(ff, 4 * C, b + ".ff.net.2.weight", b + ".ff.net.2.bias", y, C, M, C, 4 * C, y, C, 0, 0.f, nullptr, 0, nullptr,
             (k + 1 < layers && !pass1) ? &st : nullptr, false, fin1 && k + 1 < layers);
    }
    linear(y, C, p + ".proj_out.weight", p + ".proj_out.bias", out, C, M, C, C, x, C);
    ar.release(m0);
    (void)ctx;
    dump(p, out, (size_t)M * C);
    return out;
  }

  bool run(const void* latents, int io_dtype, const float* timesteps, const void* ehs, const void* text_embeds,
           const float* time_ids, void* outp) {
    const mx_unet_config& c = u->cfg;
    const int nlev = c.n_levels;
    const int C0 = c.block_out_channels[0];
    const int T = 4 * C0;
    const int text_dim = c.projection_class_embeddings_input_dim - 6 * c.addition_time_embed_dim;
    const int addw = c.projection_class_embeddings_input_dim;
    const int ctx = c.cross_attention_dim;

    ln_cnt = (unsigned*)ar.alloc((size_t)kLnCnt * sizeof(unsigned));
    if (ok() && !quiet() && ln_cnt && hipMemsetAsync(ln_cnt, 0, (size_t)kLnCnt * sizeof(unsigned), stream) != hipSuccess) fail("ln tickets: memset failed");
    tail_rows = 0;
    for (int g = 0; g < ng; ++g) tail_rows += (long)gB[g] * gH[g] * gW[g];
    if (tail_rows > 0 && tail_rows < 2147483647L) {
      const size_t nb = mx_attn_tail_sync_bytes((int)tail_rows);
      tail_sync = (unsigned*)ar.alloc(nb);
      if (ok() && !quiet() && tail_sync && hipMemsetAsync(tail_sync, 0, nb, stream) != hipSuccess) fail("attention tail tickets: memset failed");
    }
    bf16_t* tsin = alloc<bf16_t>((size_t)B * C0);
    bf16_t* addin = alloc<bf16_t>((size_t)B * addw);
    if (ok() && !dry &&
        mx::launch_time_embed(stream, timesteps, text_embeds, time_ids, tsin, addin, B, C0, text_dim, c.addition_time_embed_dim))
      fail(mx_last_error());
    bf16_t* t1 = alloc<bf16_t>((size_t)B * T);
    bf16_t* t2 = alloc<bf16_t>((size_t)B * T);
    bf16_t* a1 = alloc<bf16_t>((size_t)B * T);
    bf16_t* semb = alloc<bf16_t>((size_t)B * T);
    linear(tsin, C0, "time_embedding.linear_1.weight", "time_embedding.linear_1.bias", t1, T, B, T, C0, nullptr, 0, MX_EPI_SILU);
    linear(t1, T, "time_embedding.linear_2.weight", "time_embedding.linear_2.bias", t2, T, B, T, T);
    linear(addin, addw, "add_embedding.linear_1.weight", "add_embedding.linear_1.bias", a1, T, B, T, addw, nullptr, 0, MX_EPI_SILU);
    linear(a1, T, "add_embedding.linear_2.weight", "add_embedding.linear_2.bias", semb, T, B, T, T, t2, T, MX_EPI_SILU);
    temb_total = 0;
    {
      int prev = C0;
      for (int i = 0; i < nlev; ++i) { for (int j = 0; j < c.layers_per_block; ++j) temb_total += c.block_out_channels[i]; prev = c.block_out_channels[i]; }
      (void)prev;
      temb_total += 2 * c.block_out_channels[nlev - 1];
      for (int i = 0; i < nlev; ++i) temb_total += (c.layers_per_block + 1) * c.block_out_channels[nlev - 1 - i];
    }
    temb_all = alloc<float>((size_t)B * temb_total);
    temb_off = 0;
    linear(semb, T, "temb_proj_all.weight", "temb_proj_all.bias", temb_all, temb_total, B, temb_total, T, nullptr, 0, MX_EPI_OUT_F32);

    kv.clear();
    {
      const std::vector<std::pair<int, int>> widths = kv_widths(c);
      const int ldvt = MX_VT_LD(ctx_len);
      size_t wi = 0;
      for (auto& wv : widths) {
        const int dim = wv.first, nl = wv.second;
        KV e; e.dim = dim; e.next = 0; e.ldk = nl * dim; e.ldvt = ldvt; e.vt_bstride = (long)nl * dim * ldvt;
        if (ctx_e && !dry) { e.k = ctx_e->k[wi]; e.vt = ctx_e->vt[wi]; }
        else { e.k = alloc<bf16_t>((size_t)B * ctx_len * nl * dim); e.vt = alloc<bf16_t>((size_t)B * nl * dim * ldvt); }
        ++wi;
        if (!(ctx_e && ctx_hit && !dry)) {
          mx_gemm_desc d; std::memset(&d, 0, sizeof(d));
          d.a = ehs; d.lda = ctx; d.w = wb("attn2_kv_all." + std::to_string(dim) + ".weight", (size_t)nl * 2 * dim * ctx);
          d.c = e.k; d.ldc = nl * dim; d.M = B * ctx_len; d.N = nl * 2 * dim; d.K = ctx; d.flags = MX_EPI_QKV; d.seg = dim; d.period = 2;
          d.vt = e.vt; d.ldvt = ldvt; d.rows_per_batch = ctx_len;
          gemm(d, false);
        }
        kv.push_back(e);
      }
    }

    int h = H, wd = W;
    for (int g = 0; g < ng; ++g) { ch[g] = gH[g]; cw[g] = gW[g]; }
    if (ng > 1 && (is_pp() || (bc && !pc))) fail("a mixed-resolution batch runs neither patch-parallel nor through the per-sample block cache");
    bf16_t* x0 = alloc<bf16_t>((size_t)rows() * kConvInPad);
    for (int g = 0; g < ng && ok() && !dry; ++g)
      if (mx::launch_prep_latent(stream, g_lat[g], io_dtype, x0 + row0(g) * kConvInPad, gB[g], c.in_channels, ch[g] * cw[g], kConvInPad)) fail(mx_last_error());
    bf16_t* x = alloc<bf16_t>((size_t)rows() * C0);
    if (is_pp()) {
      bf16_t* x0p = alloc_padded(h, wd, kConvInPad);
      copy_to_padded(x0, x0p, h, wd, kConvInPad);
      halo_exchange(x0p, h, wd, kConvInPad);
      conv(x0p, h, wd, kConvInPad, "conv_in", x, C0, 1, 0, 0, nullptr, 0, nullptr, 1);
    } else
    { conv_cin_valid = c.in_channels <= 8 ? 8 : 0; conv(x0, h, wd, kConvInPad, "conv_in", x, C0, 1, 0, 0); conv_cin_valid = 0; }
    dump("conv_in", x, (size_t)rows() * C0);

    struct Skip { bf16_t* t; int C; int h, wd; int level; };
    std::vector<Skip> skips;
    skips.push_back({x, C0, h, wd, 0});
    int lvl = 0;
    int Ccur = C0;
    auto down_block = [&](int i) {
      const int Cout = c.block_out_channels[i];
      for (int j = 0; j < c.layers_per_block && ok(); ++j) {
        const std::string rp = "down_blocks." + std::to_string(i) + ".resnets." + std::to_string(j);
        x = resnet(rp, x, h, wd, Ccur, Cout, i);
        Ccur = Cout;
        if (c.down_has_attn[i]) {
          const std::string ap = "down_blocks." + std::to_string(i) + ".attentions." + std::to_string(j);
          x = transformer(ap, x, h, wd, Cout, c.num_heads[i], c.transformer_layers[i], i);
        }
        skips.push_back({x, Cout, h, wd, i});
      }
      if (i != nlev - 1) {
        const std::string dp = "down_blocks." + std::to_string(i) + ".downsamplers.0";
        size_t drows = 0;
        for (int g = 0; g < ng; ++g) drows += (size_t)gB[g] * ((ch[g] + 1) / 2) * ((cw[g] + 1) / 2);
        bf16_t* d = alloc<bf16_t>(drows * Cout);
        if (is_pp()) {
          if (h % 2) fail("patch-parallel: local rows must stay even down to the last level");
          const size_t mk = ar.mark();
          bf16_t* xp = alloc_padded(h, wd, Cout);
          copy_to_padded(x, xp, h, wd, Cout);
          halo_exchange(xp, h, wd, Cout);
          conv(xp, h, wd, Cout, dp + ".conv", d, Cout, 2, 0, 0, nullptr, 0, nullptr, 1);
          ar.release(mk);
        } else if (pc)
        pc_conv(x, h, wd, Cout, dp + ".conv", d, Cout, 2, 0, level_patch(i), i, nullptr, 0, nullptr);
        else
        conv(x, h, wd, Cout, dp + ".conv", d, Cout, 2, 0, level_patch(i));
        h /= 2; wd /= 2;
        for (int g = 0; g < ng; ++g) { ch[g] = (ch[g] + 1) / 2; cw[g] = (cw[g] + 1) / 2; }
        x = d;
        lvl = i + 1;
        dump(dp, x, (size_t)rows() * Cout);
        skips.push_back({x, Cout, h, wd, i + 1});
      }
    };
    auto mid_block = [&]() {
      const int Cm = c.block_out_channels[nlev - 1];
      x = resnet("mid_block.resnets.0", x, h, wd, Cm, Cm, nlev - 1);
      x = transformer("mid_block.attentions.0", x, h, wd, Cm, c.num_heads[nlev - 1], c.transformer_layers[nlev - 1], nlev - 1);
      x = resnet("mid_block.resnets.1", x, h, wd, Cm, Cm, nlev - 1);
    };
    auto up_block = [&](int i) {
      const int level = nlev - 1 - i;
      const int Cout = c.block_out_channels[level];
      for (int j = 0; j < c.layers_per_block + 1 && ok(); ++j) {
        const Skip sk = skips.back(); skips.pop_back();
        const std::string rp = "up_blocks." + std::to_string(i) + ".resnets." + std::to_string(j);
        x = resnet(rp, x, h, wd, Ccur + sk.C, Cout, level, sk.t, sk.C);
        Ccur = Cout;
        if (c.down_has_attn[level]) {
          const std::string ap = "up_blocks." + std::to_string(i) + ".attentions." + std::to_string(j);
          x = transformer(ap, x, h, wd, Cout, c.num_heads[level], c.transformer_layers[level], level);
        }
      }
      if (i != nlev - 1) {
        const std::string upn = "up_blocks." + std::to_string(i) + ".upsamplers.0";
        bf16_t* d = alloc<bf16_t>((size_t)rows() * 4 * Cout);
        if (is_pp()) {
          const size_t mk = ar.mark();
          bf16_t* xp = alloc_padded(h, wd, Cout);
          copy_to_padded(x, xp, h, wd, Cout);
          halo_exchange(xp, h, wd, Cout);
          conv(xp, h, wd, Cout, upn + ".conv", d, Cout, 1, 1, 0, nullptr, 0, nullptr, 1);
          ar.release(mk);
        } else if (pc)
        pc_conv(x, h, wd, Cout, upn + ".conv", d, Cout, 1, 1, level_patch(level - 1), level, nullptr, 0, nullptr);
        else
        conv(x, h, wd, Cout, upn + ".conv", d, Cout, 1, 1, level_patch(level - 1));
        h *= 2; wd *= 2;
        for (int g = 0; g < ng; ++g) { ch[g] *= 2; cw[g] *= 2; }
        x = d;
        lvl = level - 1;
        dump(upn, x, (size_t)rows() * Cout);
      }
    };

    struct Ten { bf16_t* p; size_t per_sample; int C = 0; int level = 0; };
    auto run_block_pc = [&](int idx, bool is_up, const std::vector<Ten>& ins, const std::function<void()>& body) {
      const int nf = (int)ins.size();
      std::vector<char*> in_cache(nf);
      for (int f = 0; f < nf; ++f) in_cache[f] = pc_region(ins[f].level, ins[f].C);
      auto outputs = [&](size_t n0) {
        std::vector<Ten> outs;
        if (!is_up) for (size_t k = std::min(n0, skips.size()); k < skips.size(); ++k) outs.push_back({skips[k].t, 0, skips[k].C, skips[k].level});
        if (outs.empty() || outs.back().p != x) outs.push_back({x, 0, Ccur, lvl});
        return outs;
      };
      if (dry) {
        const size_t n0 = skips.size();
        body();
        for (auto& o : outputs(n0)) pc_region(o.level, o.C);
        return;
      }
      if (!ok()) return;
      std::vector<float> mse((size_t)pc_np * nf, MX_MSE_UNCACHED);
      if (bc_any_valid) {
        size_t off = 0;
        std::vector<size_t> offs(nf);
        for (int f = 0; f < nf && ok(); ++f) {
          const int pl = pc_p0 >> ins[f].level;
          offs[f] = off;
          if (mx::launch_pc_patch_sq_diff(stream, ins[f].p, in_cache[f], pc_row_elems(ins[f].level, ins[f].C), ins[f].C, pc_dall, pc_np, pc_dsamp, ins[f].level, pl,
                                          pc_dpart + off)) fail(mx_last_error());
          off += (size_t)pc_np * pl;
        }
        std::vector<double> hp(off);
        if (ok() && (hipMemcpyAsync(hp.data(), pc_dpart, off * sizeof(double), hipMemcpyDeviceToHost, stream) != hipSuccess ||
                     hipStreamSynchronize(stream) != hipSuccess)) fail("patch cache: reading the input differences failed");
        for (int f = 0; f < nf; ++f) {
          const int pl = pc_p0 >> ins[f].level;
          for (int j = 0; j < pc_np; ++j) {
            if (!bc_valid[pc_all[j].b]) continue;
            double t = 0.0;
            for (int r = 0; r < pl; ++r) t += hp[offs[f] + (size_t)j * pl + r];
            mse[(size_t)j * nf + f] = (float)(t / ((double)pl * pl * ins[f].C));
          }
        }
      }
      if (!ok()) return;
      std::vector<unsigned char> run(pc_np, 1);
      std::vector<float> tpp(pc_np);
      for (int j = 0; j < pc_np; ++j) tpp[j] = h_timesteps[pc_all[j].b];
      if (bc->predict(bc->ctx, idx, is_up ? 1 : 0, pc_np, nf, tpp.data(), mse.data(), run.data())) { fail("patch cache: the predictor failed"); return; }
      pc_ask.clear(); pc_ask_first.assign(B + 1, 0);
      for (int j = 0; j < pc_np; ++j) {
        if (!bc_valid[pc_all[j].b]) run[j] = 1;
        if (run[j]) { pc_ask.push_back(pc_all[j]); pc_ask_first[pc_all[j].b + 1]++; }
      }
      for (int b = 0; b < B; ++b) pc_ask_first[b + 1] += pc_ask_first[b];
      pc_nask = (int)pc_ask.size();
      pc_partial = pc_nask < pc_np;
      const bool any = pc_nask > 0;
      pc_total += (unsigned long long)pc_np; pc_asked += (unsigned long long)pc_nask;
      if (any && pc_partial && hipMemcpyAsync(pc_dask, pc_ask.data(), pc_ask.size() * sizeof(mx::PcPatch), hipMemcpyHostToDevice, stream) != hipSuccess) {
        fail("patch cache: sending the list of asking patches failed"); return;
      }
      for (int f = 0; f < nf && ok(); ++f) pc_store(ins[f].p, in_cache[f], ins[f].level, ins[f].C);
      const size_t n0 = skips.size();
      mute = !any;
      body();
      mute = false;
      for (auto& o : outputs(n0)) {
        char* oc = pc_region(o.level, o.C);
        if (!ok()) return;
        if (any ? !pc_store(o.p, oc, o.level, o.C) : !pc_load(o.p, oc, o.level, o.C)) return;
      }
      if (any) blocks_run |= 1u << idx;
    };
    auto run_block = [&](int idx, bool is_up, const std::vector<Ten>& ins, const std::function<void()>& body) {
      if (!bc) { body(); return; }
      if (pc) { run_block_pc(idx, is_up, ins, body); return; }
// ... 21 lines not shown
        for (int f = 0; f < nf && ok(); ++f)
          if (mx::launch_sq_diff_partial(stream, ins[f].p, in_cache[f], (long)ins[f].per_sample, B, part + (size_t)f * B * 64, bc_dslot)) fail(mx_last_error());
        std::vector<double> hp((size_t)nf * B * 64);
        if (ok() && (hipMemcpyAsync(hp.data(), part, hp.size() * sizeof(double), hipMemcpyDeviceToHost, stream) != hipSuccess ||
                     hipStreamSynchronize(stream) != hipSuccess)) fail("block cache: reading the input differences failed");
        for (int f = 0; f < nf; ++f)
          for (int b = 0; b < B; ++b) {
            if (!bc_valid[b]) continue;
            double t = 0.0;
            for (int k = 0; k < 64; ++k) t += hp[((size_t)f * B + b) * 64 + k];
            mse[(size_t)b * nf + f] = (float)(t / (double)ins[f].per_sample);
          }
      }
      if (!ok()) return;
      std::vector<unsigned char> run(B, 1);
      if (bc->predict(bc->ctx, idx, is_up ? 1 : 0, B, nf, h_timesteps.data(), mse.data(), run.data())) { fail("block cache: the predictor failed"); return; }
      bool any = !bc_all_valid;
      for (int b = 0; b < B; ++b) any = any || run[b] != 0;
      std::vector<int>& sel = bc_sel;
      sel.assign(B, -1);
      bool partial = false;
      if (any) for (int b = 0; b < B; ++b) if (!run[b] && bc_valid[b]) { sel[b] = bc->slots ? bc->slots[b] : b; partial = true; }
      if (partial && ok() && hipMemcpyAsync(bc_dsel(), sel.data(), (size_t)B * sizeof(int), hipMemcpyHostToDevice, stream) != hipSuccess)
        fail("block cache: sending the selection table failed");
      for (int f = 0; f < nf && ok(); ++f)
        bc_store(in_cache[f], ins[f].p, ins[f].per_sample * 2);
      const size_t n_skips0 = skips.size();
      mute = !any;
      body();
      mute = false;
      std::vector<Ten> outs;
      if (!is_up) for (size_t k = std::min(n_skips0, skips.size()); k < skips.size(); ++k) outs.push_back({skips[k].t, (size_t)skips[k].h * skips[k].wd * skips[k].C});
      if (outs.empty() || outs.back().p != x) outs.push_back({x, (size_t)h * wd * Ccur});
      for (auto& o : outs) {
        char* oc = region(o.per_sample);
        if ((size_t)(bc_top - (char*)bc->state) > bc->state_bytes) { fail("block cache: state buffer too small (mx_unet_block_cache_bytes)"); return; }
        if (!ok()) return;
        if (any && bc_all_valid && bc->observe && o.p == x) {
          double* part = (double*)bc->state;
          std::vector<double> hp((size_t)B * 64);
          std::vector<float> om(B);
          if (mx::launch_sq_diff_partial(stream, o.p, oc, (long)o.per_sample, B, part, bc_dslot)) { fail(mx_last_error()); return; }
          if (hipMemcpyAsync(hp.data(), part, hp.size() * sizeof(double), hipMemcpyDeviceToHost, stream) != hipSuccess ||
              hipStreamSynchronize(stream) != hipSuccess) { fail("block cache: reading the output differences failed"); return; }
          for (int b = 0; b < B; ++b) {
            double t = 0.0;
            for (int k = 0; k < 64; ++k) t += hp[(size_t)b * 64 + k];
            om[b] = (float)(t / (double)o.per_sample);
          }
          bc->observe(bc->ctx, idx, B, om.data());
        }
        if (any && partial && mx::launch_copy_rows(stream, o.p, oc, o.per_sample * 2, B, bc_dsel(), 0)) { fail(mx_last_error()); return; }
        if (any ? !bc_store(oc, o.p, o.per_sample * 2) : !bc_load(o.p, oc, o.per_sample * 2)) return;
      }
      if (any) blocks_run |= 1u << idx;
    };
    auto up_inputs = [&](int n) {
      std::vector<Ten> v{{x, (size_t)h * wd * Ccur, Ccur, lvl}};
      const int have = std::min<int>(n, (int)skips.size());
      for (int k = 0; k < have; ++k) { const Skip& sk = skips[skips.size() - have + k]; v.push_back({sk.t, (size_t)sk.h * sk.wd * sk.C, sk.C, sk.level}); }
      return v;
    };
    int block = 0;
    if (bc && !pc) {
      if (bc_rows < B) bc_rows = B;
      bc_top = (dry ? (char*)(uintptr_t)0x1000 : (char*)bc->state) + bc_scratch_bytes(c.layers_per_block, bc_rows);
    }
    if (pc) bc_top = (dry ? (char*)(uintptr_t)0x1000 : (char*)bc->state) + pc_head_bytes(pc_slots, pc_maxh, pc_maxw, pc_p0);
    for (int i = 0; i < nlev && ok(); ++i, ++block) run_block(block, false, {{x, (size_t)h * wd * Ccur, Ccur, lvl}}, [&] { down_block(i); });
    if (ok()) { run_block(block, false, {{x, (size_t)h * wd * Ccur, Ccur, lvl}}, [&] { mid_block(); }); ++block; }
    for (int i = 0; i < nlev && ok(); ++i, ++block) run_block(block, true, up_inputs(c.layers_per_block + 1), [&] { up_block(i); });
    {
      const size_t M = (size_t)rows();
      const int Co = c.out_channels;
      const int ldo = (Co + 3) / 4 * 4;
      bf16_t* o = alloc<bf16_t>(M * ldo);
      if (is_pp()) {
        bf16_t* np_ = alloc_padded(h, wd, C0);
        groupnorm_pp(x, interior(np_, wd, C0), (long)(h + 2) * wd * C0, "conv_norm_out", h, wd, C0, c.norm_eps, true, 0);
        halo_exchange(np_, h, wd, C0);
        conv(np_, h, wd, C0, "conv_out", o, ldo, 1, 0, 0, nullptr, 0, nullptr, 1);
      } else {
      bf16_t* n = alloc<bf16_t>(M * C0);
      groupnorm(x, n, "conv_norm_out", h, wd, C0, c.norm_eps, true, level_patch(0));
      conv(n, h, wd, C0, "conv_out", o, ldo, 1, 0, level_patch(0));
      }
      dump("conv_out", o, M * ldo);
      for (int g = 0; g < ng && ok() && !dry; ++g)
        if (mx::launch_nhwc_to_nchw(stream, o + row0(g) * ldo, g_out[g], io_dtype, gB[g], Co, ch[g] * cw[g], ldo)) fail(mx_last_error());
    }
    if (stage && !dry && ok() && !stage_hit) fail(std::string("unknown stage '") + stage + "'");
    return ok();
  }
};

int check_cfg(const mx_unet_config* c) {
  MX_CHECK(c != nullptr, "unet: null config");
  MX_CHECK(c->n_levels >= 1 && c->n_levels <= 4, "unet: n_levels must be 1..4");
  MX_CHECK(c->in_channels > 0 && c->in_channels <= kConvInPad, "unet: in_channels must be <= 64");
  MX_CHECK(c->out_channels > 0 && c->out_channels <= 64, "unet: bad out_channels");
  for (int i = 0; i < c->n_levels; ++i) {
    MX_CHECK(c->block_out_channels[i] % 64 == 0, "unet: block_out_channels must be multiples of 64");
    MX_CHECK(c->block_out_channels[i] % c->norm_num_groups == 0, "unet: channels % norm_num_groups != 0");
    if (c->down_has_attn[i]) MX_CHECK(c->num_heads[i] * 64 == c->block_out_channels[i], "unet: head_dim must be 64");
  }
  MX_CHECK(c->down_has_attn[c->n_levels - 1], "unet: the mid block needs attention at the last level");
  MX_CHECK(c->cross_attention_dim % 64 == 0, "unet: cross_attention_dim must be a multiple of 64");
  MX_CHECK(c->projection_class_embeddings_input_dim % 64 == 0, "unet: projection_class_embeddings_input_dim must be a multiple of 64");
  MX_CHECK(c->addition_time_embed_dim % 2 == 0, "unet: addition_time_embed_dim must be even");
  return 0;
}

mx_unet::CtxEntry* ctx_prepare(mx_unet* u, hipStream_t stream, int B, int ctx_len, bool& hit) {
  hit = false;
  if (u->ctx_key == 0 || mx::GraphCache::env_on()) return nullptr;
  constexpr size_t kMaxEntries = 4;
  mx_unet::CtxEntry* e = nullptr;
  for (auto& q : u->ctx_store) if (q.valid && q.key == u->ctx_key && q.B == B && q.ctx_len == ctx_len) { e = &q; hit = true; break; }
  if (!e) {
    if (u->ctx_store.size() < kMaxEntries) { u->ctx_store.reserve(kMaxEntries); u->ctx_store.emplace_back(); e = &u->ctx_store.back(); }
    else { e = &u->ctx_store[0]; for (auto& q : u->ctx_store) if (q.stamp < e->stamp) e = &q; }
    e->valid = false;
    const std::vector<std::pair<int, int>> widths = kv_widths(u->cfg);
    const int ldvt = MX_VT_LD(ctx_len);
    if (!e->ev && hipEventCreateWithFlags(&e->ev, hipEventDisableTiming) != hipSuccess) { (void)hipGetLastError(); e->ev = nullptr; return nullptr; }
    e->k.resize(widths.size(), nullptr); e->vt.resize(widths.size(), nullptr); e->k_bytes.resize(widths.size(), 0); e->vt_bytes.resize(widths.size(), 0);
    for (size_t i = 0; i < widths.size(); ++i) {
      const size_t kb = (size_t)B * ctx_len * widths[i].second * widths[i].first * sizeof(bf16_t);
      const size_t vb = (size_t)B * widths[i].second * widths[i].first * ldvt * sizeof(bf16_t);
      if (e->k_bytes[i] < kb || e->vt_bytes[i] < vb) {
        if (e->last) (void)hipStreamSynchronize(e->last);
        if (e->k[i]) (void)hipFree(e->k[i]);
        if (e->vt[i]) (void)hipFree(e->vt[i]);
        e->k[i] = nullptr; e->vt[i] = nullptr; e->k_bytes[i] = e->vt_bytes[i] = 0;
        if (hipMalloc(&e->k[i], kb) != hipSuccess || hipMalloc(&e->vt[i], vb) != hipSuccess) { (void)hipGetLastError(); return nullptr; }
        e->k_bytes[i] = kb; e->vt_bytes[i] = vb;
      }
    }
    e->key = u->ctx_key; e->B = B; e->ctx_len = ctx_len;
  }
  if (e->recorded && e->last != stream && hipStreamWaitEvent(stream, e->ev, 0) != hipSuccess) { (void)hipGetLastError(); hit = false; return nullptr; }
  e->stamp = ++u->ctx_clock;
  if (hit) ++u->ctx_hits; else ++u->ctx_misses;
  return e;
}

struct Model {
  const char* name = "unet";
  mx_unet::CtxEntry* ctx_e = nullptr;
  bool ctx_hit = false;
  static int check_shape(const mx_unet* u, int H, int W, int gn_patch) {
    const int div = 1 << (u->cfg.n_levels - 1);
    MX_CHECK(H % div == 0 && W % div == 0, "unet: H, W must be divisible by 2^(levels-1)");
    MX_CHECK(gn_patch >= 0, "unet: gn_patch must be >= 0");
    if (gn_patch > 0) {
      MX_CHECK(H % gn_patch == 0 && W % gn_patch == 0, "unet: H, W must be multiples of gn_patch");
      MX_CHECK((gn_patch >> (u->cfg.n_levels - 1)) >= 2 || gn_patch >= H, "unet: gn_patch too small for the deepest level (needs >= 2 pixels there)");
    }
    return 0;
  }
  int check(const mx_unet* u, const mx::ForwardCall& c) {
    const int div = 1 << (u->cfg.n_levels - 1);
    for (int g = 0; c.groups && g < c.n_groups; ++g) {
      const mx_unet_group& q = c.groups[g];
      MX_CHECK(q.H % div == 0 && q.W % div == 0, "unet: bad group shape");
      if (c.gn_patch > 0)
        MX_CHECK((q.H % c.gn_patch == 0 && q.W % c.gn_patch == 0) || (c.gn_patch >= q.H && c.gn_patch >= q.W), "unet: every group's H, W must be multiples of gn_patch");
// ... 342 lines not shown
```

sduss_amd/lib.py:

```python
from __future__ import annotations

import ctypes as C
import os
from typing import Optional

_HERE = os.path.dirname(os.path.abspath(__file__))
LIB_PATH = os.path.join(_HERE, "libmxdenoise.so")

MX_F32, MX_F16, MX_BF16 = 0, 1, 2
EPI_SILU, EPI_GEGLU, EPI_OUT_F32, EPI_QKV, EPI_GELU_TANH, EPI_RES_BCAST, EPI_RMSNORM, EPI_GELU, EPI_QUICK_GELU, EPI_GEGLU_TANH = 1, 2, 4, 8, 16, 32, 64, 128, 256, 512


class MxError(RuntimeError):
    """Raised for every non-zero status of the C ABI (the reference's launcher only printed
    cudaGetLastError and went on -- norm_silu_concat.cu:434-437; SURVEY.md section 8b asks to raise)."""


MAX_SEGS = 4


class GemmSeg(C.Structure):
    _fields_ = [
        ("a", C.c_void_p), ("a2", C.c_void_p), ("c", C.c_void_p), ("residual", C.c_void_p), ("vt", C.c_void_p), ("rowbias", C.c_void_p),
        ("gate", C.c_void_p), ("ln_stats", C.c_void_p), ("stats_out", C.c_void_p),
# ... 93 lines not shown

class CLIPConfigC(C.Structure):
    _fields_ = [("vocab_size", C.c_int), ("hidden_size", C.c_int), ("intermediate_size", C.c_int), ("num_hidden_layers", C.c_int),
                ("num_attention_heads", C.c_int), ("max_position_embeddings", C.c_int), ("hidden_act", C.c_int), ("projection_dim", C.c_int),
                ("eos_token_id", C.c_int), ("hidden_layer", C.c_int), ("layer_norm_eps", C.c_float)]


class T5ConfigC(C.Structure):
    _fields_ = [("vocab_size", C.c_int), ("d_model", C.c_int), ("d_ff", C.c_int), ("num_layers", C.c_int), ("num_heads", C.c_int),
                ("layer_norm_epsilon", C.c_float)]


class VAEConfigC(C.Structure):
    _fields_ = [("latent_channels", C.c_int), ("out_channels", C.c_int), ("n_levels", C.c_int), ("block_out_channels", C.c_int * 4),
                ("layers_per_block", C.c_int), ("norm_num_groups", C.c_int), ("norm_eps", C.c_float)]


class WeightEntry(C.Structure):
    _fields_ = [("name", C.c_char_p), ("offset", C.c_uint64), ("bytes", C.c_uint64)]


_vp, _i, _f, _d, _i64, _sz = C.c_void_p, C.c_int, C.c_float, C.c_double, C.c_int64, C.c_size_t
SYMBOLS = {
    "mx_last_error": (C.c_char_p, []),
    "mx_version": (_i, []),
    "mx_profile_enable": (_i, [_i]),
    "mx_profile_collect": (_i, [C.POINTER(C.c_double)]),
    "mx_profile_records": (_i, [C.POINTER(C.c_double), _i]),
    "mx_groupnorm_halo_workspace_bytes": (_sz, [_i, _i, _i]),
    "mx_groupnorm_halo": (_i, [_vp, _vp, _vp, _vp, _vp, _i, _i, _i, _i, _i, _d, _i, _vp, _i, _vp, _vp, _i, _vp]),
    "mx_halo_only": (_i, [_vp, _vp, _vp, _i, _i, _i, _i, _vp, _i]),
    "mx_gemm": (_i, [_vp, C.POINTER(GemmDesc)]),
    "mx_conv3x3": (_i, [_vp, C.POINTER(GemmDesc)]),
    "mx_gemm_stats_slabs": (_i, [C.POINTER(GemmDesc)]),
    "mx_gemm_ln_prefers_pass": (_i, [C.POINTER(GemmDesc)]),
    "mx_row_stats": (_i, [_vp, _vp, _i, _vp, _i, _i]),
    "mx_attention": (_i, [_vp, _vp, _i, _vp, _i, _vp, _i, _i64, _vp, _i, _i, _i, _i, _i, _f]),
    "mx_attention_prescaled": (_i, [_vp, _vp, _i, _vp, _i, _vp, _i, _i64, _vp, _i, _i, _i, _i, _i]),
    "mx_attention_cross_prescaled": (_i, [_vp, _vp, _i, _vp, _i, _vp, _i, _i64, _vp, _i, _i, _i, _i, _i]),
    "mx_attn_tail_sync_bytes": (_sz, [_i]),
    "mx_attn_tail_supported": (_i, [C.POINTER(AttnTailDesc)]),
    "mx_attn_tail_preferred": (_i, []),
    "mx_attn_tail": (_i, [_vp, C.POINTER(AttnTailDesc)]),
    "mx_attn_tail_status": (_i, [_vp, _vp, C.POINTER(C.c_uint)]),
    "mx_layernorm": (_i, [_vp, _vp, _vp, _vp, _vp, _i, _i, _f]),
    "mx_groupnorm_nhwc_workspace_bytes": (_sz, [_i, _i, _i, _i]),
    "mx_groupnorm_nhwc": (_i, [_vp, _vp, _vp, _vp, _vp, _i, _i, _i, _i, _i, _f, _i, _i, _vp]),
    "mx_groupnorm_nhwc_cat": (_i, [_vp, _vp, _i, _vp, _vp, _vp, _vp, _i, _i, _i, _i, _i, _f, _i, _i, _vp]),
    "mx_attention_prescaled_grouped": (_i, [_vp, C.POINTER(AttnProblem), _i, _i, _i, _i, _i]),
    "mx_groupnorm_nhwc_grouped_workspace_bytes": (_sz, [C.POINTER(GnProblem), _i, _i]),
    "mx_groupnorm_nhwc_grouped": (_i, [_vp, C.POINTER(GnProblem), _i, _i, _vp, _vp, _i, _i, _f, _i, _i, _vp]),
    "mx_unet_workspace_bytes_mixed": (_sz, [_vp, C.POINTER(UNetGroup), _i, _i]),
    "mx_unet_forward_mixed": (_i, [_vp, _vp, C.POINTER(UNetGroup), _i, _i, _vp, _vp, _vp, _vp, _i, _i, _vp, _sz]),
    "mx_unet_forward_mixed_trace": (_i, [_vp, _vp, C.POINTER(UNetGroup), _i, _i, _vp, _vp, _vp, _vp, _i, _i, _vp, _sz, C.c_char_p, _vp, _sz]),
    "mx_mmdit_workspace_bytes_mixed": (_sz, [_vp, C.POINTER(UNetGroup), _i, _i]),
    "mx_mmdit_forward_mixed": (_i, [_vp, _vp, C.POINTER(UNetGroup), _i, _i, _vp, _vp, _vp, _i, _vp, _sz]),
    "mx_unet_create": (_vp, [C.POINTER(UNetConfigC)]),
    "mx_unet_destroy": (None, [_vp]),
    "mx_unet_set_context_key": (_i, [_vp, C.c_uint64]),
    "mx_unet_context_stats": (_i, [_vp, C.POINTER(C.c_long), C.POINTER(C.c_long)]),
    "mx_unet_set_weights": (_i, [_vp, _vp, C.c_uint64, C.POINTER(WeightEntry), _i]),
    "mx_unet_workspace_bytes": (_sz, [_vp, _i, _i, _i, _i]),
    "mx_unet_validate": (_i, [_vp, _i, _i, _i, _i]),
    "mx_unet_forward": (_i, [_vp, _vp, _vp, _i, _vp, _vp, _vp, _vp, _vp, _i, _i, _i, _i, _i, _vp, _sz]),
    "mx_forest_predict": (_i, [_vp, _vp, _vp, _vp, _vp, _vp, _i, _vp, _i, _i, _vp]),
    "mx_mmdit_workspace_bytes_pp": (_sz, [_vp, _i, _i, _i, _i, _i]),
    "mx_mmdit_pp_state_bytes": (_sz, [_vp, _i, _i, _i, _i, _i]),
    "mx_mmdit_forward_pp": (_i, [_vp, _vp, _vp, _i, _vp, _vp, _vp, _vp, _i, _i, _i, _i, _vp, _vp, _vp, _sz]),
    "mx_mmdit_pp_comm_plan": (_i, [_vp, _i, _i, _i, _i, _vp]),
    "mx_unet_pp_state_bytes": (_sz, [_vp, _i, _i, _i, _i, _i]),
    "mx_unet_forward_pp_stale": (_i, [_vp, _vp, _vp, _i, _vp, _vp, _vp, _vp, _vp, _i, _i, _i, _i, _vp, _vp, _vp, _sz]),
    "mx_unet_block_cache_bytes": (_sz, [_vp, _i, _i, _i]),
    "mx_gemm_splitk": (_i, [_vp, _i]),
    "mx_gemm_release_scratch": (None, [_vp, _i]),
    "mx_gemm_ln_final_supported": (_i, [C.POINTER(GemmDesc)]),
    "mx_gemm_launches": (_i, [C.POINTER(GemmDesc)]),
    "mx_gemm_gn_partials_supported": (_i, [C.POINTER(GemmDesc), _i]),
    "mx_gemm_form": (_i, [C.POINTER(GemmDesc), _i]),
    "mx_gemm_kernel_name": (_i, [C.POINTER(GemmDesc), _i, _i, C.c_char_p, _i]),
    "mx_gemm_kernel_names": (_i, [C.c_char_p, _i]),
    "mx_attention_kernel_name": (_i, [_i, _i, _i, _i, _i, _i, _i, _i, _i, _i, C.c_char_p, _i]),
    "mx_attention_kernel_names": (_i, [C.c_char_p, _i]),
    "mx_groupnorm_nhwc_from_partials": (_i, [_vp, _vp, _vp, _vp, _vp, _i, _i, _i, _i, _i, C.c_float, _i, _vp, _i, _vp, _vp, _i, _vp]),
    "mx_unet_patch_cache_bytes": (_sz, [_vp, _i, _i, _i, _i]),
    "mx_mmdit_patch_cache_bytes": (_sz, [_vp, _i, _i, _i, _i, _i]),
    "mx_mmdit_workspace_bytes_cached_mixed": (_sz, [_vp, C.POINTER(UNetGroup), _i, _i, _i]),
    "mx_mmdit_forward_cached_mixed": (_i, [_vp, _vp, C.POINTER(UNetGroup), _i, _i, _vp, _vp, _vp, _i, _i, _vp, _sz, _vp]),
    "mx_unet_workspace_bytes_cached_mixed": (_sz, [_vp, C.POINTER(UNetGroup), _i, _i, _i]),
    "mx_unet_forward_cached_mixed": (_i, [_vp, _vp, C.POINTER(UNetGroup), _i, _i, _vp, _vp, _vp, _vp, _i, _i, _vp, _sz, _vp]),
    "mx_unet_forward_cached": (_i, [_vp, _vp, _vp, _i, _vp, _vp, _vp, _vp, _vp, _i, _i, _i, _i, _i, _vp, _sz, _vp]),
    "mx_mmdit_block_cache_bytes": (_sz, [_vp, _i, _i, _i, _i]),
    "mx_mmdit_forward_cached": (_i, [_vp, _vp, _vp, _i, _vp, _vp, _vp, _vp, _i, _i, _i, _i, _vp, _sz, _vp]),
    "mx_unet_forward_trace": (_i, [_vp, _vp, _vp, _i, _vp, _vp, _vp, _vp, _vp, _i, _i, _i, _i, _i, _vp, _sz,
                                   C.c_char_p, _vp, _sz]),
    "mx_unet_workspace_bytes_pp": (_sz, [_vp, _i, _i, _i, _i, _i]),
    "mx_unet_forward_pp": (_i, [_vp, _vp, _vp, _i, _vp, _vp, _vp, _vp, _vp, _i, _i, _i, _i, C.POINTER(PPComm), _vp, _sz]),
    "mx_unet_pp_comm_plan": (_i, [_vp, _i, _i, _i, _i, C.POINTER(PPComm)]),
    "mx_attention_prescaled_chunked": (_i, [_vp, _vp, _i, _vp, _i, _vp, _i, _i64, _vp, _i, _i, _i, _i, _i, _i, _i64, _i64, _i64]),
    "mx_layernorm_mod": (_i, [_vp, _vp, _vp, _vp, _vp, _vp, _vp, _vp, _i, _i, _i, _i, _f]),
    "mx_layernorm_mod_grouped": (_i, [_vp, _vp, _vp, _vp, _vp, _vp, _vp, _vp, _i, _i, _f, _vp, _vp, _i]),
    "mx_rmsnorm_heads": (_i, [_vp, _vp, _i, _i, _i, _i, _i, _i, _i, _vp, _vp, _f, _f]),
    "mx_mmdit_create": (_vp, [C.POINTER(MMDiTConfigC)]),
    "mx_mmdit_destroy": (None, [_vp]),
    "mx_mmdit_set_weights": (_i, [_vp, _vp, C.c_uint64, C.POINTER(WeightEntry), _i]),
    "mx_mmdit_workspace_bytes": (_sz, [_vp, _i, _i, _i, _i]),
    "mx_mmdit_validate": (_i, [_vp, _i, _i, _i, _i]),
    "mx_mmdit_forward": (_i, [_vp, _vp, _vp, _i, _vp, _vp, _vp, _vp, _i, _i, _i, _i, _vp, _sz]),
    "mx_mmdit_forward_trace": (_i, [_vp, _vp, _vp, _i, _vp, _vp, _vp, _vp, _i, _i, _i, _i, _vp, _sz, C.c_char_p, _vp, _sz]),
    "mx_vae_create": (_vp, [C.POINTER(VAEConfigC)]),
    "mx_vae_destroy": (None, [_vp]),
    "mx_vae_set_weights": (_i, [_vp, _vp, C.c_uint64, C.POINTER(WeightEntry), _i]),
    "mx_vae_workspace_bytes": (_sz, [_vp, _i, _i, _i]),
    "mx_vae_validate": (_i, [_vp, _i, _i, _i]),
    "mx_vae_decode": (_i, [_vp, _vp, _vp, _i, _vp, _i, _i, _i, _i, _vp, _sz]),
    "mx_clip_create": (_vp, [C.POINTER(CLIPConfigC)]),
    "mx_clip_destroy": (None, [_vp]),
    "mx_clip_set_weights": (_i, [_vp, _vp, C.c_uint64, C.POINTER(WeightEntry), _i]),
    "mx_clip_workspace_bytes": (_sz, [_vp, _i]),
    "mx_clip_validate": (_i, [_vp, _i]),
    "mx_clip_encode": (_i, [_vp, _vp, _vp, _vp, _vp, _i, _vp, _sz]),
    "mx_attention_prescaled_causal": (_i, [_vp, _vp, _i, _vp, _i, _vp, _i, _i64, _vp, _i, _i, _i, _i]),
    "mx_attention_prescaled_bias": (_i, [_vp, _vp, _i, _vp, _i, _vp, _i, _i64, _vp, _i, _i, _i, _i, _i, _vp, _i]),
    "mx_rmsnorm": (_i, [_vp, _vp, _vp, _vp, _i, _i, _f]),
    "mx_t5_create": (_vp, [C.POINTER(T5ConfigC)]),
    "mx_t5_destroy": (None, [_vp]),
    "mx_t5_set_weights": (_i, [_vp, _vp, C.c_uint64, C.POINTER(WeightEntry), _i]),
    "mx_t5_workspace_bytes": (_sz, [_vp, _i, _i]),
    "mx_t5_validate": (_i, [_vp, _i, _i]),
    "mx_t5_encode": (_i, [_vp, _vp, _vp, _vp, _i, _i, _vp, _sz]),
    "mx_cfg_flow_step": (_i, [_vp, _vp, _vp, _vp, _vp, _f, _i, _i64, _i]),
    "mx_euler_scale_input": (_i, [_vp, _vp, _vp, _vp, _i, _i, _i64, _i]),
    "mx_cfg_euler_step": (_i, [_vp, _vp, _vp, _vp, _vp, _f, _i, _i64, _i]),
}

_lib: Optional[C.CDLL] = None


def load() -> C.CDLL:
    global _lib
    if _lib is not None:
        return _lib
    path = os.environ.get("MXDENOISE_LIB", LIB_PATH)
    if not os.path.exists(path):
        raise MxError(f"{path} not found: build it with `python -c 'import __graft_entry__ as g; g.build()'` "
                      f"(or `make -C sduss_amd/csrc`). There is no CPU fallback for the product path.")
    lib = C.CDLL(path)
    for name, (res, args) in SYMBOLS.items():
        fn = getattr(lib, name)
        fn.restype = res
        fn.argtypes = args
    _lib = lib
    return lib


def check(status: int, what: str = "") -> None:
    if status != 0:
        msg = load().mx_last_error().decode("utf-8", "replace")
        raise MxError(f"{what}: {msg}" if what else msg)


def torch_dtype_code(dtype) -> int:
    import torch
    if dtype == torch.float32:
        return MX_F32
    if dtype == torch.float16:
        return MX_F16
# ... 44 lines not shown
```

sduss_amd/ops.py:

```python
from __future__ import annotations

import ctypes as C
from typing import Optional

import torch

from . import lib as _lib


def _p(t: Optional[torch.Tensor]):
    return None if t is None else t.data_ptr()


def _bf16(t):
    assert t.is_cuda and t.dtype == torch.bfloat16 and t.is_contiguous(), "expected a contiguous CUDA bf16 tensor"
    return t


def gemm(a: torch.Tensor, w: torch.Tensor, bias: Optional[torch.Tensor] = None, residual: Optional[torch.Tensor] = None,
         rowbias: Optional[torch.Tensor] = None, rows_per_batch: int = 0, silu: bool = False, geglu: bool = False,
         out_f32: bool = False, out_scale: float = 0.0, ln_stats: Optional[torch.Tensor] = None, ln_colsum: Optional[torch.Tensor] = None,
         ln_eps: float = 1e-5, want_stats: bool = False, splitk: int = 0, ln_final: Optional[torch.Tensor] = None, want_final: bool = False,
         final_buffers=None):
    l = _lib.load()
    _bf16(a); _bf16(w)
    m, k = a.shape
    n = w.shape[0]
    d = _lib.GemmDesc()
    flags = (_lib.EPI_SILU if silu else 0) | (_lib.EPI_GEGLU if geglu else 0) | (_lib.EPI_OUT_F32 if out_f32 else 0)
    nout = n // 2 if geglu else n
    c = torch.empty((m, nout), dtype=torch.float32 if out_f32 else torch.bfloat16, device=a.device)
    d.a, d.w, d.c = a.data_ptr(), w.data_ptr(), c.data_ptr()
    d.bias, d.rowbias, d.residual = _p(bias), _p(rowbias), _p(residual)
    d.M, d.N, d.K, d.lda, d.ldc = m, n, k, k, nout
    d.ldr = residual.shape[1] if residual is not None else 0
    d.ldrb = rowbias.shape[1] if rowbias is not None else 0
    d.rows_per_batch, d.flags, d.out_scale = rows_per_batch, flags, out_scale
    d.splitk = splitk
    if ln_stats is not None:
        st_, slabs_ = ln_stats
        assert st_.dtype == torch.float32 and ln_colsum.dtype == torch.float32 and st_.shape == (m, stats_pitch(slabs_), 2)
        d.ln_stats, d.ln_colsum, d.ln_slabs, d.ln_eps = st_.data_ptr(), ln_colsum.data_ptr(), slabs_, ln_eps
    if ln_final is not None:
        assert ln_final.dtype == torch.float32 and ln_final.shape == (m, 2) and ln_colsum.dtype == torch.float32
        d.ln_final, d.ln_colsum, d.ln_eps = ln_final.data_ptr(), ln_colsum.data_ptr(), ln_eps
    stats = None
    final = None
    if want_stats:
        slabs = l.mx_gemm_stats_slabs(C.byref(d))
        stats = torch.full((m, stats_pitch(max(slabs, 1)), 2), float("nan"), dtype=torch.float32, device=a.device)
        if slabs > 0:
            d.stats_out = stats.data_ptr()
            if want_final and l.mx_gemm_ln_final_supported(C.byref(d)):
                if final_buffers is not None:
                    final, cnt = final_buffers
                else:
                    final = torch.full((m, 2), float("nan"), dtype=torch.float32, device=a.device)
                    cnt = torch.zeros((m + 255) // 256, dtype=torch.int32, device=a.device)
                d.ln_final_out, d.ln_final_cnt, d.ln_eps = final.data_ptr(), cnt.data_ptr(), ln_eps
    _lib.check(l.mx_gemm(_lib.current_stream(), C.byref(d)), "mx_gemm")
    if want_stats:
        if not d.stats_out:
            _lib.check(l.mx_row_stats(_lib.current_stream(), c.data_ptr(), nout, stats.data_ptr(), m, nout), "mx_row_stats")
        if want_final:
            if final is not None and final_buffers is None:
                assert int(cnt.abs().sum()) == 0, "ln_final_cnt must be zero again after the launch"
            return c, (stats, max(slabs, 1)), final
        return c, (stats, max(slabs, 1))
    return c


def stats_pitch(slabs: int) -> int:
    return (slabs + 3) & ~3


def row_stats(x: torch.Tensor) -> torch.Tensor:
    l = _lib.load()
    _bf16(x)
    m, c = x.shape
    st = torch.full((m, 4, 2), float("nan"), dtype=torch.float32, device=x.device)
    _lib.check(l.mx_row_stats(_lib.current_stream(), x.data_ptr(), c, st.data_ptr(), m, c), "mx_row_stats")
    return st, 1


def vt_ld(lk: int) -> int:
    return (lk + 15) // 16 * 16


def vt_pos(lk: int) -> torch.Tensor:
    k = torch.arange(lk)
    return (k & ~12) | ((k & 4) << 1) | ((k & 8) >> 1)


def pack_vt(v: torch.Tensor, pad: float = 0.0) -> torch.Tensor:
    b, lk, c = v.shape
    vt = torch.full((b, c, vt_ld(lk)), pad, dtype=v.dtype, device=v.device)
    vt[:, :, vt_pos(lk).to(v.device)] = v.permute(0, 2, 1)
    return vt


def unpack_vt(vt: torch.Tensor, lk: int) -> torch.Tensor:
    return vt[:, :, vt_pos(lk).to(vt.device)].permute(0, 2, 1)


def gemm_qkv(a: torch.Tensor, w: torch.Tensor, seg: int, period: int, rows_per_batch: int, q_scale: float = 0.0,
             ln_stats: Optional[torch.Tensor] = None, ln_colsum: Optional[torch.Tensor] = None, ln_eps: float = 1e-5,
             bias: Optional[torch.Tensor] = None, ln_final: Optional[torch.Tensor] = None):
    l = _lib.load()
    _bf16(a); _bf16(w)
    m, k = a.shape
    n = w.shape[0]
    nb = m // rows_per_batch
    ldvt = vt_ld(rows_per_batch)
    c = torch.empty((m, n // period * (period - 1)), dtype=torch.bfloat16, device=a.device)
    vt = torch.zeros((nb, n // period, ldvt), dtype=torch.bfloat16, device=a.device)
    d = _lib.GemmDesc()
    d.a, d.w, d.c, d.vt = a.data_ptr(), w.data_ptr(), c.data_ptr(), vt.data_ptr()
    d.M, d.N, d.K, d.lda, d.ldc = m, n, k, k, c.shape[1]
    d.rows_per_batch, d.flags, d.seg, d.period, d.ldvt = rows_per_batch, _lib.EPI_QKV, seg, period, ldvt
    d.out_scale = q_scale
    d.bias = _p(bias)
    if ln_stats is not None:
        d.ln_stats, d.ln_colsum, d.ln_slabs, d.ln_eps = ln_stats[0].data_ptr(), ln_colsum.data_ptr(), ln_stats[1], ln_eps
    if ln_final is not None:
        d.ln_final, d.ln_colsum, d.ln_eps = ln_final.data_ptr(), ln_colsum.data_ptr(), ln_eps
    _lib.check(l.mx_gemm(_lib.current_stream(), C.byref(d)), "mx_gemm(qkv)")
    return c, vt


def conv3x3(x: torch.Tensor, w: torch.Tensor, bias: Optional[torch.Tensor], stride: int = 1, up: int = 0,
            corner_patch: int = 0, rowbias: Optional[torch.Tensor] = None, residual: Optional[torch.Tensor] = None, splitk: int = 0, want_gn_partials: bool = False,
            cin_valid: int = 0):
    l = _lib.load()
    _bf16(x); _bf16(w)
    b, h, wd, cin = x.shape
    cout = w.shape[0]
    hv, wv = h << up, wd << up
    ho, wo = (hv + stride - 1) // stride, (wv + stride - 1) // stride
    c = torch.empty((b, ho, wo, cout), dtype=torch.bfloat16, device=x.device)
    d = _lib.GemmDesc()
    d.a, d.w, d.c, d.bias, d.rowbias, d.residual = x.data_ptr(), w.data_ptr(), c.data_ptr(), _p(bias), _p(rowbias), _p(residual)
    d.M, d.N, d.K, d.ldc, d.ldr = b * ho * wo, cout, 9 * cin, cout, cout
    d.ldrb = rowbias.shape[1] if rowbias is not None else 0
# ... 33 lines not shown
def attn_tail(ao: torch.Tensor, y: torch.Tensor, w1: torch.Tensor, b1: torch.Tensor, wq: torch.Tensor, bq: torch.Tensor, colsum_q: torch.Tensor,
              k: torch.Tensor, vt: torch.Tensor, w2: torch.Tensor, b2: torch.Tensor, heads: int, L: int, ctx_len: int, ln_eps: float = 1e-5,
              chained: bool = True, finalise: bool = True, sync: Optional[torch.Tensor] = None):
    l = _lib.load()
    for t_ in (ao, y, w1, wq, w2, k, vt):
        _bf16(t_)
    m, c = y.shape
    b = m // L
    dev = y.device
    y = y.clone()
    q2 = torch.empty_like(y)
    ao2 = torch.empty_like(y)
    td = _lib.AttnTailDesc()

    def lin(d, a_, w_, bias, c_, res):
        d.a, d.w, d.c, d.bias = a_.data_ptr(), w_.data_ptr(), c_.data_ptr(), bias.data_ptr()
        d.M, d.N, d.K, d.lda, d.ldc = m, c, c, c, c
        if res is not None:
            d.residual, d.ldr = res.data_ptr(), c
    lin(td.out1, ao, w1, b1, y, y)
    lin(td.to_q, y, wq, bq, q2, None)
    lin(td.out2, ao2, w2, b2, y, y)
    td.out1.stats_out = 16
    slabs = l.mx_gemm_stats_slabs(C.byref(td.out1))
    assert slabs > 0, "out1 cannot write slab statistics at this shape"
    st1 = torch.full((m, stats_pitch(slabs), 2), float("nan"), dtype=torch.float32, device=dev)
    st2 = torch.full((m, stats_pitch(slabs), 2), float("nan"), dtype=torch.float32, device=dev)
    td.out1.stats_out = st1.data_ptr()
    td.to_q.ln_stats, td.to_q.ln_colsum, td.to_q.ln_slabs, td.to_q.ln_eps = st1.data_ptr(), colsum_q.data_ptr(), slabs, ln_eps
    td.to_q.out_scale = ATTN_QSCALE
    td.out2.stats_out = st2.data_ptr()
    final = cnt = None
    if finalise:
        final = torch.full((m, 2), float("nan"), dtype=torch.float32, device=dev)
        cnt = torch.zeros((m + 255) // 256, dtype=torch.int32, device=dev)
        td.out2.ln_final_out, td.out2.ln_final_cnt, td.out2.ln_eps = final.data_ptr(), cnt.data_ptr(), ln_eps
    td.k, td.ldk, td.vt, td.ldvt, td.vt_batch_stride = k.data_ptr(), k.shape[1], vt.data_ptr(), vt.shape[2], vt.shape[1] * vt.shape[2]
    td.B, td.heads, td.L, td.ctx_len = b, heads, L, ctx_len
    stream = _lib.current_stream()
    if chained:
        if sync is None:
            sync = torch.zeros(l.mx_attn_tail_sync_bytes(m) // 4, dtype=torch.int32, device=dev)
        td.sync = sync.data_ptr()
        assert l.mx_attn_tail_supported(C.byref(td)), "mx_attn_tail cannot serve this shape"
        _lib.check(l.mx_attn_tail(stream, C.byref(td)), "mx_attn_tail")
    else:
        _lib.check(l.mx_gemm(stream, C.byref(td.out1)), "mx_gemm")
        _lib.check(l.mx_gemm(stream, C.byref(td.to_q)), "mx_gemm")
        _lib.check(l.mx_attention_cross_prescaled(stream, q2.data_ptr(), c, k.data_ptr(), k.shape[1], vt.data_ptr(), vt.shape[2], vt.shape[1] * vt.shape[2],
                                                  ao2.data_ptr(), c, b, heads, L, ctx_len), "mx_attention_cross_prescaled")
        _lib.check(l.mx_gemm(stream, C.byref(td.out2)), "mx_gemm")
    return y, (st2, slabs), final, q2, ao2, sync


def attn_tail_status(sync: torch.Tensor) -> int:
    l = _lib.load()
    w = C.c_uint(0)
    _lib.check(l.mx_attn_tail_status(_lib.current_stream(), sync.data_ptr(), C.byref(w)), "mx_attn_tail_status")
    return w.value


def layernorm(x: torch.Tensor, gamma: torch.Tensor, beta: torch.Tensor, eps: float = 1e-5) -> torch.Tensor:
    l = _lib.load()
    _bf16(x)
    y = torch.empty_like(x)
    _lib.check(l.mx_layernorm(_lib.current_stream(), x.data_ptr(), y.data_ptr(), gamma.data_ptr(), beta.data_ptr(),
                              x.shape[0], x.shape[1], eps), "mx_layernorm")
    return y


def groupnorm_nhwc_from_partials(x: torch.Tensor, gamma: torch.Tensor, beta: torch.Tensor, groups: int, eps: float, silu: bool, part: torch.Tensor,
                                 chunk: int = 64, add_bias: Optional[torch.Tensor] = None, add_rowbias: Optional[torch.Tensor] = None) -> torch.Tensor:
    l = _lib.load()
    _bf16(x)
    b, h, w, c = x.shape
    y = torch.empty_like(x)
    ws = torch.empty(l.mx_groupnorm_nhwc_workspace_bytes(b, h, w, c), dtype=torch.uint8, device=x.device)
    _lib.check(l.mx_groupnorm_nhwc_from_partials(_lib.current_stream(), x.data_ptr(), y.data_ptr(), gamma.data_ptr(), beta.data_ptr(), b, h, w, c, groups, eps,
                                                 1 if silu else 0, part.data_ptr(), chunk, _p(add_bias), _p(add_rowbias),
                                                 add_rowbias.shape[1] if add_rowbias is not None else 0, ws.data_ptr()), "mx_groupnorm_nhwc_from_partials")
    return y


def groupnorm_nhwc(x: torch.Tensor, gamma: torch.Tensor, beta: torch.Tensor, groups: int, eps: float, silu: bool,
                   patch: int = 0) -> torch.Tensor:
    l = _lib.load()
    _bf16(x)
    b, h, w, c = x.shape
    y = torch.empty_like(x)
    ws = torch.empty(l.mx_groupnorm_nhwc_workspace_bytes(b, h, w, c), dtype=torch.uint8, device=x.device)
    _lib.check(l.mx_groupnorm_nhwc(_lib.current_stream(), x.data_ptr(), y.data_ptr(), gamma.data_ptr(), beta.data_ptr(),
                                   b, h, w, c, groups, eps, int(silu), patch, ws.data_ptr()), "mx_groupnorm_nhwc")
    return y


def euler_scale_input(latents: torch.Tensor, sigma: torch.Tensor, n_rows: int) -> torch.Tensor:
    l = _lib.load()
    latents = latents.contiguous()
    n_lat = latents.shape[0]
    elems = latents[0].numel()
    out = torch.empty((n_rows, *latents.shape[1:]), dtype=latents.dtype, device=latents.device)
    sg = sigma.to(device=latents.device, dtype=torch.float32).contiguous()
    _lib.check(l.mx_euler_scale_input(_lib.current_stream(), latents.data_ptr(), out.data_ptr(), sg.data_ptr(), n_lat, n_rows,
                                      elems, _lib.torch_dtype_code(latents.dtype)), "mx_euler_scale_input")
    return out


def cfg_euler_step_(noise: torch.Tensor, latents: torch.Tensor, sigma: torch.Tensor, sigma_next: torch.Tensor,
                    guidance_scale: float) -> torch.Tensor:
    l = _lib.load()
    assert latents.is_contiguous() and noise.is_contiguous() and noise.dtype == latents.dtype
    n_lat = latents.shape[0]
    sg = sigma.to(device=latents.device, dtype=torch.float32).contiguous()
    sn = sigma_next.to(device=latents.device, dtype=torch.float32).contiguous()
    _lib.check(l.mx_cfg_euler_step(_lib.current_stream(), noise.data_ptr(), latents.data_ptr(), sg.data_ptr(), sn.data_ptr(),
                                   float(guidance_scale), n_lat, latents[0].numel(), _lib.torch_dtype_code(latents.dtype)),
               "mx_cfg_euler_step")
    return latents


def layernorm_mod(x: torch.Tensor, scale: torch.Tensor, shift: torch.Tensor, rows_per_batch: int, eps: float = 1e-6,
                  scale2: Optional[torch.Tensor] = None, shift2: Optional[torch.Tensor] = None):
    l = _lib.load()
    _bf16(x)
    m, c = x.shape
    y = torch.empty_like(x)
    y2 = torch.empty_like(x) if scale2 is not None else None
    for t in (scale, shift, scale2, shift2):
        assert t is None or (t.dtype == torch.float32 and t.is_contiguous() and t.shape[1] == c)
    _lib.check(l.mx_layernorm_mod(_lib.current_stream(), x.data_ptr(), y.data_ptr(), _p(y2), scale.data_ptr(), shift.data_ptr(),
                                  _p(scale2), _p(shift2), c, m, c, rows_per_batch, eps), "mx_layernorm_mod")
    return (y, y2) if y2 is not None else y


def rmsnorm_heads_(x: torch.Tensor, nbatch: int, rows_per_batch: int, batch_rows: int, row_off: int, heads_total: int,
                   heads_q: int, wq: torch.Tensor, wk: torch.Tensor, eps: float = 1e-6, q_scale: float = 1.0) -> torch.Tensor:
    l = _lib.load()
    _bf16(x)
    _lib.check(l.mx_rmsnorm_heads(_lib.current_stream(), x.data_ptr(), x.shape[1], nbatch, rows_per_batch, batch_rows, row_off,
                                  heads_total, heads_q, wq.data_ptr(), wk.data_ptr(), eps, q_scale), "mx_rmsnorm_heads")
    return x


def cfg_flow_step_(noise: torch.Tensor, latents: torch.Tensor, sigma: torch.Tensor, sigma_next: torch.Tensor,
                   guidance_scale: float) -> torch.Tensor:
    l = _lib.load()
    assert latents.is_contiguous() and noise.is_contiguous() and noise.dtype == latents.dtype
    sg = sigma.to(device=latents.device, dtype=torch.float32).contiguous()
    sn = sigma_next.to(device=latents.device, dtype=torch.float32).contiguous()
    _lib.check(l.mx_cfg_flow_step(_lib.current_stream(), noise.data_ptr(), latents.data_ptr(), sg.data_ptr(), sn.data_ptr(),
                                  float(guidance_scale), latents.shape[0], latents[0].numel(), _lib.torch_dtype_code(latents.dtype)),
               "mx_cfg_flow_step")
    return latents
```

Measured before the change: 1.411 images/s.

## Emit GroupNorm partial sums from residual GEMM/conv epilogues and fold concatenations

New measurement: 1.417 images/s, median of 6. No clear change (+0.4%).

```diff
diff --git a/include/mxdenoise.h b/include/mxdenoise.h
--- a/include/mxdenoise.h
+++ b/include/mxdenoise.h
@@ -173,6 +173,9 @@
                           int B, int H, int W, int C, int groups, float eps, int silu, int patch, void* workspace);
 int mx_groupnorm_nhwc_from_partials(void* stream, const void* x, void* y, const float* gamma, const float* beta, int B, int H, int W, int C, int groups, float eps,
                                     int silu, const float* part, int chunk, const float* add_bias, const float* add_rowbias, int ldrb, void* workspace);
+int mx_groupnorm_nhwc_from_partials_cat(void* stream, const void* x, int C1, const void* x2, void* y, const float* gamma, const float* beta, int B, int H, int W, int C,
+                                        int groups, float eps, int silu, const float* part, const float* part2, int chunk, const float* add_bias, const float* add_bias2,
+                                        const float* add_rowbias, int ldrb, void* workspace);
 
 typedef struct mx_gn_problem { const void* x; const void* x2; void* y; int B, H, W; } mx_gn_problem;
 size_t mx_groupnorm_nhwc_grouped_workspace_bytes(const mx_gn_problem* probs, int n, int C);
diff --git a/sduss_amd/csrc/gemm_args.h b/sduss_amd/csrc/gemm_args.h
--- a/sduss_amd/csrc/gemm_args.h
+++ b/sduss_amd/csrc/gemm_args.h
@@ -457,7 +457,8 @@
   const int acts = flags & (MX_EPI_SILU | MX_EPI_GELU | MX_EPI_GELU_TANH | MX_EPI_QUICK_GELU | MX_EPI_GEGLU_TANH);
   return ((flags & MX_EPI_QKV) ? EPI_F_QKV : 0) | (acts == 0 ? 0 : acts == MX_EPI_GELU_TANH ? EPI_F_TANH : EPI_F_ACT);
 }
-template <int NI, int MI, bool GEGLU, bool VEC = true, bool VPF = true, bool STATS = true, int FEAT = EPI_F_ALL, bool EMIT = STATS, bool RSTD_LOAD = false, bool WT = false>
+template <int NI, int MI, bool GEGLU, bool VEC = true, bool VPF = true, bool STATS = true, int FEAT = EPI_F_ALL, bool EMIT = STATS, bool RSTD_LOAD = false, bool WT = false,
+          bool GNP = false>
 __device__ __forceinline__ void gemm_epilogue_regs(const GemmArgs& p, f32x4 (&acc)[NI][MI], const int m_wave0, const int wave_n0,
                                                    const int fr, const int fq, const float (&ln_rstd_a)[MI]) {
 #pragma clang fp contract(off)
@@ -497,6 +498,9 @@
     for (int i = 0; i < NI; ++i) rmsw_r[i] = *reinterpret_cast<const f32x4*>(w + ((wave_n0 - seg_idx * p.seg + i * 16 + fq * 4) & 63));
   }
   const bool stats = EMIT && !GEGLU && !qkv && p.stats_out != nullptr;
+  static_assert(!GNP || (!GEGLU && FEAT == 0 && MI == 4), "GroupNorm partial sums: plain epilogue, one 64-token chunk per wave");
+  const bool gnp = GNP && p.gn_part != nullptr && has_res;
+  float gn_s[GNP && NP > 0 ? NP : 1][8], gn_q[GNP && NP > 0 ? NP : 1][8], gn_so[4], gn_qo[4];
 
   if constexpr ((FEAT & EPI_F_QKV) != 0) {
     if (qkv && to_vt) {
@@ -673,10 +677,19 @@
       for (int q = 0; q < 4; ++q) v[i][q] = t[q];
     }
     if constexpr (VPF) { if (j + 1 < MI && (has_rb || has_gate)) load_batch_vectors(j + 1); }
-    auto finish8 = [&](float (&o)[8], const u32x4 rr) __attribute__((always_inline)) {
+    auto finish8 = [&](float (&o)[8], const u32x4 rr, const int pr) __attribute__((always_inline)) {
       if (has_res) {
 #pragma unroll
         for (int q = 0; q < 4; ++q) { o[2 * q] += bf16lo_to_f32(rr[q]); o[2 * q + 1] += bf16hi_to_f32(rr[q]); }
+      }
+      if constexpr (GNP) {
+        if (gnp) {
+#pragma unroll
+          for (int q = 0; q < 8; ++q) {
+            if (j == 0) { gn_s[pr][q] = o[q]; gn_q[pr][q] = o[q] * o[q]; }
+            else { gn_s[pr][q] += o[q]; gn_q[pr][q] = fmaf(o[q], o[q], gn_q[pr][q]); }
+          }
+        }
       }
       if (ACT && (flags & MX_EPI_SILU)) {
 #pragma unroll
@@ -712,8 +725,8 @@
           res_a = odd_lane ? nb_rb : ra;
           res_b = odd_lane ? rb : nb_ra;
         }
-        finish8(oa, res_a);
-        finish8(ob, res_b);
+        finish8(oa, res_a, 2 * g);
+        finish8(ob, res_b, 2 * g + 1);
         const u32x4 wa = {pack_bf16x2(oa[0], oa[1]), pack_bf16x2(oa[2], oa[3]), pack_bf16x2(oa[4], oa[5]), pack_bf16x2(oa[6], oa[7])};
         const u32x4 wb = {pack_bf16x2(ob[0], ob[1]), pack_bf16x2(ob[2], ob[3]), pack_bf16x2(ob[4], ob[5]), pack_bf16x2(ob[6], ob[7])};
         const u32x4 nb_b = lane_xor1(wb), nb_a = lane_xor1(wa);
@@ -731,7 +744,7 @@
       for (int q = 0; q < 4; ++q) { o[q] = v[2 * pr][q]; o[4 + q] = v[2 * pr + 1][q]; }
       const u32x4 rr = res_r[j % DEPTH][pr];
       if (j + DEPTH < MI) res_r[j % DEPTH][pr] = load_res(j + DEPTH, pr);
-      finish8(o, rr);
+      finish8(o, rr, pr);
       if (m < p.M) {
         const u32x4 w = {pack_bf16x2(o[0], o[1]), pack_bf16x2(o[2], o[3]), pack_bf16x2(o[4], o[5]), pack_bf16x2(o[6], o[7])};
         store_c16(row_own(j), col0 + pr * 32 + fq * 8, w);
@@ -744,6 +757,15 @@
       const u32x2 rr = res_o[j % DEPTH];
       if (j + DEPTH < MI) res_o[j % DEPTH] = load_res_odd(j + DEPTH);
       if (has_res) { o[0] += bf16lo_to_f32(rr[0]); o[1] += bf16hi_to_f32(rr[0]); o[2] += bf16lo_to_f32(rr[1]); o[3] += bf16hi_to_f32(rr[1]); }
+      if constexpr (GNP) {
+        if (gnp) {
+#pragma unroll
+          for (int q = 0; q < 4; ++q) {
+            if (j == 0) { gn_so[q] = o[q]; gn_qo[q] = o[q] * o[q]; }
+            else { gn_so[q] += o[q]; gn_qo[q] = fmaf(o[q], o[q], gn_qo[q]); }
+          }
+        }
+      }
       if (ACT && (flags & MX_EPI_SILU)) {
 #pragma unroll
         for (int q = 0; q < 4; ++q) o[q] = silu_f(o[q]);
@@ -776,6 +798,29 @@
       }
     }
   }
-}
-
-}
+  if constexpr (GNP) {
+    if (gnp && m_wave0 < p.M) {
+      float* dst = p.gn_part + ((long)(m_wave0 >> 6) * p.N + col0) * 2;
+#pragma unroll
+      for (int pr = 0; pr < NP; ++pr) {
+#pragma unroll
+        for (int q = 0; q < 8; ++q) { gn_s[pr][q] = row16_sum(gn_s[pr][q]); gn_q[pr][q] = row16_sum(gn_q[pr][q]); }
+        if (fr == 0) {
+#pragma unroll
+          for (int q = 0; q < 8; q += 2)
+            *reinterpret_cast<f32x4*>(dst + (pr * 32 + fq * 8 + q) * 2) = f32x4{gn_s[pr][q], gn_q[pr][q], gn_s[pr][q + 1], gn_q[pr][q + 1]};
+        }
+      }
+      if constexpr (ODD) {
+#pragma unroll
+        for (int q = 0; q < 4; ++q) { gn_so[q] = row16_sum(gn_so[q]); gn_qo[q] = row16_sum(gn_qo[q]); }
+        if (fr == 0) {
+          *reinterpret_cast<f32x4*>(dst + (NP * 32 + fq * 4) * 2) = f32x4{gn_so[0], gn_qo[0], gn_so[1], gn_qo[1]};
+          *reinterpret_cast<f32x4*>(dst + (NP * 32 + fq * 4 + 2) * 2) = f32x4{gn_so[2], gn_qo[2], gn_so[3], gn_qo[3]};
+        }
+      }
+    }
+  }
+}
+
+}
diff --git a/sduss_amd/csrc/gemm_bf16.hip b/sduss_amd/csrc/gemm_bf16.hip
--- a/sduss_amd/csrc/gemm_bf16.hip
+++ b/sduss_amd/csrc/gemm_bf16.hip
@@ -480,8 +480,8 @@
   a.gn_part = nullptr;
   if (d->gn_part_out) {
     MX_CHECK(!grouped && tc.rows == 256 && tc.bn != 256 && tc.bn != 0 && tc.splitk <= 1, "gemm: gn_part_out needs an ungrouped launch on a 256-row tile (mx_gemm_gn_partials_supported)");
-    MX_CHECK(d->flags == 0 && !d->residual && !d->gate && d->out_scale == 0.f && !d->ln_stats && !d->ln_final && d->a_batch_rows <= 0 && d->c_batch_rows <= 0,
-             "gemm: gn_part_out needs an epilogue of bias (+ row bias) only");
+    MX_CHECK(d->flags == 0 && !d->gate && d->out_scale == 0.f && !d->ln_stats && !d->ln_final && d->a_batch_rows <= 0 && d->c_batch_rows <= 0 && !(d->residual && d->rowbias),
+             "gemm: gn_part_out needs an epilogue of bias + row bias or of bias + residual, nothing else");
     MX_CHECK(d->M % 64 == 0 && (!d->rowbias || d->rows_per_batch % 64 == 0) && ((uintptr_t)d->gn_part_out & 15) == 0, "gemm: gn_part_out needs M % 64 == 0, rows_per_batch % 64 == 0 and 16-byte alignment");
     a.gn_part = d->gn_part_out;
   }
@@ -651,7 +651,8 @@
 }
 extern "C" int mx_gemm_gn_partials_supported(const mx_gemm_desc* d, int conv) {
   if (!d || d->n_segs > 0 || d->M <= 0 || d->N <= 0 || d->K <= 0 || d->M % 64 != 0) return 0;
-  if (d->flags != 0 || d->residual || d->gate || d->out_scale != 0.f || d->ln_stats || d->ln_final || d->a_batch_rows > 0 || d->c_batch_rows > 0) return 0;
+  if (d->flags != 0 || d->gate || d->out_scale != 0.f || d->ln_stats || d->ln_final || d->a_batch_rows > 0 || d->c_batch_rows > 0) return 0;
+  if (d->residual && d->rowbias) return 0;
   if (d->rowbias && (d->rows_per_batch <= 0 || d->rows_per_batch % 64 != 0)) return 0;
   const mx::TileChoice tc = mx::pick_tile(d, conv != 0);
   return tc.rows == 256 && tc.bn != 256 && tc.bn != 0 && tc.splitk <= 1;
diff --git a/sduss_amd/csrc/gemm_v5_body.h b/sduss_amd/csrc/gemm_v5_body.h
--- a/sduss_amd/csrc/gemm_v5_body.h
+++ b/sduss_amd/csrc/gemm_v5_body.h
@@ -100,9 +100,10 @@
 
   const int m0 = tm * BM5, n0 = tn * BN;
   static_assert(!GEGLU || (NI % 4 == 0 && !CONV), "the gated epilogue pairs whole 32-feature halves");
-  gemm_epilogue_regs<NI, MI, GEGLU, VEC, true, true, FEAT, true, false, WT>(p, acc, m0 + wm * 16 * MI, n0 + wn * (BN / 2), fr, fq, ln_rstd);
+  constexpr bool GNP = !GEGLU && FEAT == 0 && MI == 4 && !VEC && !WT;
+  gemm_epilogue_regs<NI, MI, GEGLU, VEC, true, true, FEAT, true, false, WT, GNP>(p, acc, m0 + wm * 16 * MI, n0 + wn * (BN / 2), fr, fq, ln_rstd);
   if constexpr (!GEGLU && FEAT == 0 && MI == 4) {
-    if (pk.gn_part != nullptr) gemm_gn_partials<NI, MI>(p, acc, m0 + wm * 16 * MI, n0 + wn * (BN / 2), fr, fq);
+    if (pk.gn_part != nullptr && p.residual == nullptr) gemm_gn_partials<NI, MI>(p, acc, m0 + wm * 16 * MI, n0 + wn * (BN / 2), fr, fq);
   }
   MX5_STAMP(3);
   wait_vmcnt<0>();
diff --git a/sduss_amd/csrc/norm.hip b/sduss_amd/csrc/norm.hip
--- a/sduss_amd/csrc/norm.hip
+++ b/sduss_amd/csrc/norm.hip
@@ -19,6 +19,7 @@
   GnGeom g;
   const bf16_t* x; bf16_t* y;
   float* part; float* coef;
+  const float* part2;
   float* gpart;
   long y_img;
   int ppb;
@@ -109,11 +110,14 @@
 constexpr int kFoldThreads = 256;
 __global__ __launch_bounds__(kFoldThreads) void gn_fold_kernel(const GnGroup G, const float* __restrict__ gamma, const float* __restrict__ beta,
                                                                int groups, float eps, const float* __restrict__ add_bias = nullptr,
-                                                               const float* __restrict__ add_rowbias = nullptr, int ldrb = 0) {
+                                                               const float* __restrict__ add_rowbias = nullptr, int ldrb = 0,
+                                                               const float* __restrict__ add_bias2 = nullptr) {
   int local;
   const GnProb& P = gn_locate(G, local);
   const GnGeom& g = P.g;
   const float* __restrict__ part = P.part;
+  const float* __restrict__ part2 = P.part2;
+  const int pC1 = part2 != nullptr ? g.C1 : g.C;
   float* __restrict__ coef = P.coef;
   const int patch = P.patch;
   const int b = local / groups;
@@ -127,25 +131,41 @@
   const int tpy = g.tiles_y / ppy, tpx = g.tiles_x / ppx;
   const int nitems = tpy * tpx * cpg;
   const double cnt = (double)tpy * tpx * g.th * g.tw * cpg;
+  const double npx = (double)(g.th * g.tw);
   double acc_mean = 0.0, acc_var = 0.0;
   __shared__ double wsum[kFoldThreads / 64][2];
+  auto add_item = [&](const int tile, const int c, double& s, double& q) __attribute__((always_inline)) {
+    const int chn = grp * cpg + c;
+    const bool second = chn >= pC1;
+    const float* src = second ? part2 + (((long)b * ntiles + tile) * (g.C - pC1) + (chn - pC1)) * 2 : part + (((long)b * ntiles + tile) * pC1 + chn) * 2;
+    const float2 v = *reinterpret_cast<const float2*>(src);
+    const float* ab = second ? add_bias2 : add_bias;
+    if (ab != nullptr) {
+      const double cc = (double)ab[second ? chn - pC1 : chn] + (add_rowbias != nullptr ? (double)add_rowbias[(long)b * ldrb + chn] : 0.0);
+      s += (double)v.x + npx * cc;
+      q += (double)v.y + 2.0 * cc * (double)v.x + npx * cc * cc;
+    } else {
+      s += (double)v.x;
+      q += (double)v.y;
+    }
+  };
   for (int pidx = 0; pidx < npatch; ++pidx) {
     const int py = pidx / ppx, px = pidx - py * ppx;
     double s = 0.0, q = 0.0;
-    for (int it = lane; it < nitems; it += kFoldThreads) {
-      const int tl = it / cpg, c = it - tl * cpg;
-      const int iy = tl / tpx, ix = tl - iy * tpx;
-      const int tile = (py * tpy + iy) * g.tiles_x + px * tpx + ix;
-      const float2 v = *reinterpret_cast<const float2*>(part + (((long)b * ntiles + tile) * g.C + grp * cpg + c) * 2);
-      if (add_bias != nullptr) {
-        const int chn = grp * cpg + c;
-        const double cc = (double)add_bias[chn] + (add_rowbias != nullptr ? (double)add_rowbias[(long)b * ldrb + chn] : 0.0);
-        const double npx = (double)(g.th * g.tw);
-        s += (double)v.x + npx * cc;
-        q += (double)v.y + 2.0 * cc * (double)v.x + npx * cc * cc;
-      } else {
-        s += (double)v.x;
-        q += (double)v.y;
+    if (patch == 0) {
+      const int dtl = kFoldThreads / cpg, dc = kFoldThreads - dtl * cpg;
+      int tl = lane / cpg, c = lane - tl * cpg;
+#pragma unroll 4
+      for (int it = lane; it < nitems; it += kFoldThreads) {
+        add_item(tl, c, s, q);
+        tl += dtl; c += dc;
+        if (c >= cpg) { c -= cpg; ++tl; }
+      }
+    } else {
+      for (int it = lane; it < nitems; it += kFoldThreads) {
+        const int tl = it / cpg, c = it - tl * cpg;
+        const int iy = tl / tpx, ix = tl - iy * tpx;
+        add_item((py * tpy + iy) * g.tiles_x + px * tpx + ix, c, s, q);
       }
     }
     s = wave_sum_d(s);
@@ -349,6 +369,7 @@
   P.x = (const bf16_t*)x; P.y = (bf16_t*)y; P.y_img = y_img; P.patch = patch;
   P.part = (float*)ws;
   P.gpart = nullptr;
+  P.part2 = nullptr;
   P.coef = P.part + (size_t)B * ntiles * C * 2;
   const int hw = H * W;
   P.ppb = P.g.L * 8 > hw ? hw : P.g.L * 8;
@@ -448,27 +469,38 @@
   return mx_groupnorm_nhwc_grouped(stream, &q, 1, C1, gamma, beta, C, groups, eps, silu, patch, workspace);
 }
 
-extern "C" int mx_groupnorm_nhwc_from_partials(void* stream, const void* x, void* y, const float* gamma, const float* beta, int B, int H, int W, int C, int groups,
-                                               float eps, int silu, const float* part, int chunk, const float* add_bias, const float* add_rowbias, int ldrb,
-                                               void* workspace) {
+extern "C" int mx_groupnorm_nhwc_from_partials_cat(void* stream, const void* x, int C1, const void* x2, void* y, const float* gamma, const float* beta, int B, int H, int W,
+                                                   int C, int groups, float eps, int silu, const float* part, const float* part2, int chunk, const float* add_bias,
+                                                   const float* add_bias2, const float* add_rowbias, int ldrb, void* workspace) {
   using namespace mx;
   MX_CHECK(x && y && gamma && beta && part && workspace && B > 0 && H > 0 && W > 0, "groupnorm: null operand / empty problem");
   MX_CHECK(groups > 0 && C % groups == 0 && chunk > 0 && (H * W) % chunk == 0 && ((uintptr_t)part & 15) == 0, "groupnorm: bad groups / chunk / alignment");
+  MX_CHECK((x2 != nullptr) == (part2 != nullptr) && (x2 == nullptr || (C1 > 0 && C1 < C && C1 % 8 == 0 && (C - C1) % 8 == 0 && ((uintptr_t)part2 & 7) == 0)),
+           "groupnorm: a channel concatenation needs both tensors' partial sums and a split at multiples of 8");
+  MX_CHECK(x2 != nullptr || add_bias2 == nullptr, "groupnorm: add_bias2 belongs to the second tensor of a concatenation");
+  MX_CHECK(add_rowbias == nullptr || (x2 == nullptr && add_bias != nullptr && ldrb >= C), "groupnorm: add_rowbias needs one source, add_bias and ldrb >= C");
   GnGroup G;
   G.n = 1;
-  if (!gn_fill(G, 0, x, C, nullptr, y, (long)H * W * C, B, H, W, C, 0, (char*)workspace)) return 1;
+  if (!gn_fill(G, 0, x, C1, x2, y, (long)H * W * C, B, H, W, C, 0, (char*)workspace)) return 1;
   GnGroup F = G;
   F.p[0].part = const_cast<float*>(part);
+  F.p[0].part2 = part2;
   F.p[0].g.tiles_y = H * W / chunk; F.p[0].g.tiles_x = 1; F.p[0].g.th = chunk; F.p[0].g.tw = 1;
   hipStream_t s = (hipStream_t)stream;
   prof_begin(s, PROF_NORM, 0.0, 2.0 * 2.0 * B * H * (double)W * C);
   gn_prefix(F, 1, groups);
-  MX_CHECK(add_rowbias == nullptr || (add_bias != nullptr && ldrb >= C), "groupnorm: add_rowbias needs add_bias and ldrb >= C");
-  hipLaunchKernelGGL(gn_fold_kernel, dim3(F.blk0[MX_MAX_SEGS]), dim3(kFoldThreads), 0, s, F, gamma, beta, groups, eps, add_bias, add_rowbias, ldrb);
+  hipLaunchKernelGGL(gn_fold_kernel, dim3(F.blk0[MX_MAX_SEGS]), dim3(kFoldThreads), 0, s, F, gamma, beta, groups, eps, add_bias, add_rowbias, ldrb, add_bias2);
   MX_LAUNCH_CHECK();
   if (gn_launch_apply(s, G, silu)) return 1;
   prof_end(s);
   return 0;
+}
+
+extern "C" int mx_groupnorm_nhwc_from_partials(void* stream, const void* x, void* y, const float* gamma, const float* beta, int B, int H, int W, int C, int groups,
+                                               float eps, int silu, const float* part, int chunk, const float* add_bias, const float* add_rowbias, int ldrb,
+                                               void* workspace) {
+  return mx_groupnorm_nhwc_from_partials_cat(stream, x, C, nullptr, y, gamma, beta, B, H, W, C, groups, eps, silu, part, nullptr, chunk, add_bias, nullptr, add_rowbias,
+                                             ldrb, workspace);
 }
 
 namespace mx {
diff --git a/sduss_amd/csrc/unet_sdxl.cpp b/sduss_amd/csrc/unet_sdxl.cpp
--- a/sduss_amd/csrc/unet_sdxl.cpp
+++ b/sduss_amd/csrc/unet_sdxl.cpp
@@ -5,6 +5,7 @@
 #include <functional>
 #include <map>
 #include <string>
+#include <unordered_map>
 #include <vector>
 
 #include "../../include/mxdenoise.h"
@@ -354,15 +355,36 @@
     ar.release(m);
     return ok();
   }
+  struct GnSrc { const float* part; const float* add_bias; };
+  std::unordered_map<const void*, GnSrc> gn_src;
+  bool gn_chain() const { return ng == 1 && gn_patch == 0 && !is_pp() && !pc && !bc; }
+  const GnSrc* gn_find(const void* t) const { auto it = gn_src.find(t); return it == gn_src.end() ? nullptr : &it->second; }
+  float* gn_part_alloc(long M, int C, long hw) {
+    if (!gn_chain() || M % 64 != 0 || hw % 64 != 0) return nullptr;
+    return (float*)ar.alloc((size_t)(M / 64) * C * 2 * sizeof(float));
+  }
+  void gn_note(const void* t, bool done, const float* part, const float* add_bias) {
+    if (done) gn_src[t] = GnSrc{part, add_bias}; else gn_src.erase(t);
+  }
+  bool groupnorm_chained(const bf16_t* x, bf16_t* y, const std::string& prefix, int h, int wd, int C, float eps, bool silu, int patch, const bf16_t* x2 = nullptr,
+                         int C1 = 0) {
+    const GnSrc* s1 = gn_chain() && patch == 0 ? gn_find(x) : nullptr;
+    const GnSrc* s2 = s1 && x2 ? gn_find(x2) : nullptr;
+    if (s1 && (!x2 || s2))
+      return groupnorm_from_partials(x, y, prefix, h, wd, C, eps, silu, s1->part, s1->add_bias, nullptr, 0, x2, C1, s2 ? s2->part : nullptr, s2 ? s2->add_bias : nullptr);
+    return groupnorm(x, y, prefix, h, wd, C, eps, silu, patch, x2, C1);
+  }
   bool groupnorm_from_partials(const bf16_t* x, bf16_t* y, const std::string& prefix, int h, int wd, int C, float eps, bool silu, const float* part,
-                               const float* add_bias, const float* add_rowbias, int ldrb) {
+                               const float* add_bias, const float* add_rowbias, int ldrb, const bf16_t* x2 = nullptr, int C1 = 0, const float* part2 = nullptr,
+                               const float* add_bias2 = nullptr) {
     if (!ok()) return false;
     const size_t m = ar.mark();
     void* ws = ar.alloc(mx::gn_workspace_exact(gB[0], h, wd, C, 0));
     if (!ws) return fail("workspace too small");
     const float* g = wf(prefix + ".weight", C); const float* b = wf(prefix + ".bias", C);
     if (ok() && !quiet()) {
-      if (mx_groupnorm_nhwc_from_partials(stream, x, y, g, b, gB[0], h, wd, C, u->cfg.norm_num_groups, eps, silu ? 1 : 0, part, 64, add_bias, add_rowbias, ldrb, ws))
+      if (mx_groupnorm_nhwc_from_partials_cat(stream, x, x2 ? C1 : C, x2, y, g, b, gB[0], h, wd, C, u->cfg.norm_num_groups, eps, silu ? 1 : 0, part, part2, 64, add_bias,
+                                              add_bias2, add_rowbias, ldrb, ws))
         fail(std::string("groupnorm: ") + mx_last_error());
     }
     ar.release(m);
@@ -388,6 +410,7 @@
     const int M = (int)rows();
     const int C1 = Cin - C2;
     bf16_t* out = alloc<bf16_t>((size_t)M * Cout);
+    float* opart = gn_part_alloc(M, Cout, (long)h * wd);
     const size_t m = ar.mark();
     const int patch = level_patch(level);
     if (is_pp()) {
@@ -433,7 +456,7 @@
       return out;
     }
     bf16_t* n1 = alloc<bf16_t>((size_t)M * Cin);
-    groupnorm(x, n1, p + ".norm1", h, wd, Cin, u->cfg.norm_eps, true, patch, x2, C1);
+    groupnorm_chained(x, n1, p + ".norm1", h, wd, Cin, u->cfg.norm_eps, true, patch, x2, C1);
     bf16_t* h1 = alloc<bf16_t>((size_t)M * Cout);
     float* gpart = nullptr;
     bool gdone = false;
@@ -451,7 +474,9 @@
       else linear(x, Cin, p + ".conv_shortcut.weight", p + ".conv_shortcut.bias", s2, Cout, M, Cout, Cin);
       sc = s2;
     }
-    conv(n2, h, wd, Cout, p + ".conv2", out, Cout, 1, 0, patch, nullptr, 0, sc);
+    bool odone = false;
+    conv(n2, h, wd, Cout, p + ".conv2", out, Cout, 1, 0, patch, nullptr, 0, sc, 0, opart, &odone);
+    gn_note(out, odone, opart, nullptr);
     ar.release(m);
     dump(p, out, (size_t)M * Cout);
     return out;
@@ -472,10 +497,11 @@
       vt_elems += (long)gB[g] * C * gldvt[g];
     }
     bf16_t* out = alloc<bf16_t>((size_t)M * C);
+    float* opart = gn_part_alloc(M, C, L);
     const size_t m0 = ar.mark();
     bf16_t* n = alloc<bf16_t>((size_t)M * C);
     if (is_pp()) groupnorm_pp(x, n, (long)L * C, p + ".norm", h, wd, C, u->cfg.transformer_norm_eps, false, level);
-    else groupnorm(x, n, p + ".norm", h, wd, C, u->cfg.transformer_norm_eps, false, level_patch(level));
+    else groupnorm_chained(x, n, p + ".norm", h, wd, C, u->cfg.transformer_norm_eps, false, level_patch(level));
     bf16_t* y = alloc<bf16_t>((size_t)M * C);
     RowStats st;
     st.buf = (float*)ar.alloc((size_t)M * MX_STATS_PITCH(C / 64) * 2 * sizeof(float));
@@ -727,7 +753,15 @@
       linear(ff, 4 * C, b + ".ff.net.2.weight", b + ".ff.net.2.bias", y, C, M, C, 4 * C, y, C, 0, 0.f, nullptr, 0, nullptr,
              (k + 1 < layers && !pass1) ? &st : nullptr, false, fin1 && k + 1 < layers);
     }
-    linear(y, C, p + ".proj_out.weight", p + ".proj_out.bias", out, C, M, C, C, x, C);
+    {
+      mx_gemm_desc d; std::memset(&d, 0, sizeof(d));
+      d.a = y; d.lda = C; d.w = wb(p + ".proj_out.weight", (size_t)C * C); d.bias = wf(p + ".proj_out.bias", C);
+      d.c = out; d.ldc = C; d.M = M; d.N = C; d.K = C; d.residual = x; d.ldr = C;
+      const bool odone = opart != nullptr && mx_gemm_gn_partials_supported(&d, 0) != 0;
+      if (odone) d.gn_part_out = opart;
+      gemm(d, false);
+      gn_note(out, odone, opart, nullptr);
+    }
     ar.release(m0);
     (void)ctx;
     dump(p, out, (size_t)M * C);
@@ -744,11 +778,13 @@
     const int addw = c.projection_class_embeddings_input_dim;
     const int ctx = c.cross_attention_dim;
 
+    gn_src.clear();
     ln_cnt = (unsigned*)ar.alloc((size_t)kLnCnt * sizeof(unsigned));
     if (ok() && !quiet() && ln_cnt && hipMemsetAsync(ln_cnt, 0, (size_t)kLnCnt * sizeof(unsigned), stream) != hipSuccess) fail("ln tickets: memset failed");
     tail_rows = 0;
     for (int g = 0; g < ng; ++g) tail_rows += (long)gB[g] * gH[g] * gW[g];
-    if (tail_rows > 0 && tail_rows < 2147483647L) {
+    tail_sync = nullptr;
+    if (mx_attn_tail_preferred() != 0 && tail_rows > 0 && tail_rows < 2147483647L) {
       const size_t nb = mx_attn_tail_sync_bytes((int)tail_rows);
       tail_sync = (unsigned*)ar.alloc(nb);
       if (ok() && !quiet() && tail_sync && hipMemsetAsync(tail_sync, 0, nb, stream) != hipSuccess) fail("attention tail tickets: memset failed");
@@ -838,6 +874,8 @@
         size_t drows = 0;
         for (int g = 0; g < ng; ++g) drows += (size_t)gB[g] * ((ch[g] + 1) / 2) * ((cw[g] + 1) / 2);
         bf16_t* d = alloc<bf16_t>(drows * Cout);
+        float* dpart = gn_part_alloc((long)drows, Cout, (long)((h + 1) / 2) * ((wd + 1) / 2));
+        bool ddone = false;
         if (is_pp()) {
           if (h % 2) fail("patch-parallel: local rows must stay even down to the last level");
           const size_t mk = ar.mark();
@@ -849,7 +887,8 @@
         } else if (pc)
         pc_conv(x, h, wd, Cout, dp + ".conv", d, Cout, 2, 0, level_patch(i), i, nullptr, 0, nullptr);
         else
-        conv(x, h, wd, Cout, dp + ".conv", d, Cout, 2, 0, level_patch(i));
+        conv(x, h, wd, Cout, dp + ".conv", d, Cout, 2, 0, level_patch(i), nullptr, 0, nullptr, 0, dpart, &ddone);
+        gn_note(d, ddone, dpart, wf(dp + ".conv.bias", Cout));
         h /= 2; wd /= 2;
         for (int g = 0; g < ng; ++g) { ch[g] = (ch[g] + 1) / 2; cw[g] = (cw[g] + 1) / 2; }
         x = d;
@@ -880,6 +919,8 @@
       if (i != nlev - 1) {
         const std::string upn = "up_blocks." + std::to_string(i) + ".upsamplers.0";
         bf16_t* d = alloc<bf16_t>((size_t)rows() * 4 * Cout);
+        float* dpart = gn_part_alloc(rows() * 4, Cout, (long)h * wd * 4);
+        bool ddone = false;
         if (is_pp()) {
           const size_t mk = ar.mark();
           bf16_t* xp = alloc_padded(h, wd, Cout);
@@ -890,7 +931,8 @@
         } else if (pc)
         pc_conv(x, h, wd, Cout, upn + ".conv", d, Cout, 1, 1, level_patch(level - 1), level, nullptr, 0, nullptr);
         else
-        conv(x, h, wd, Cout, upn + ".conv", d, Cout, 1, 1, level_patch(level - 1));
+        conv(x, h, wd, Cout, upn + ".conv", d, Cout, 1, 1, level_patch(level - 1), nullptr, 0, nullptr, 0, dpart, &ddone);
+        gn_note(d, ddone, dpart, wf(upn + ".conv.bias", Cout));
         h *= 2; wd *= 2;
         for (int g = 0; g < ng; ++g) { ch[g] *= 2; cw[g] *= 2; }
         x = d;
@@ -1078,7 +1120,7 @@
         conv(np_, h, wd, C0, "conv_out", o, ldo, 1, 0, 0, nullptr, 0, nullptr, 1);
       } else {
       bf16_t* n = alloc<bf16_t>(M * C0);
-      groupnorm(x, n, "conv_norm_out", h, wd, C0, c.norm_eps, true, level_patch(0));
+      groupnorm_chained(x, n, "conv_norm_out", h, wd, C0, c.norm_eps, true, level_patch(0));
       conv(n, h, wd, C0, "conv_out", o, ldo, 1, 0, level_patch(0));
       }
       dump("conv_out", o, M * ldo);
diff --git a/sduss_amd/lib.py b/sduss_amd/lib.py
--- a/sduss_amd/lib.py
+++ b/sduss_amd/lib.py
@@ -199,6 +199,7 @@
     "mx_attention_kernel_name": (_i, [_i, _i, _i, _i, _i, _i, _i, _i, _i, _i, C.c_char_p, _i]),
     "mx_attention_kernel_names": (_i, [C.c_char_p, _i]),
     "mx_groupnorm_nhwc_from_partials": (_i, [_vp, _vp, _vp, _vp, _vp, _i, _i, _i, _i, _i, C.c_float, _i, _vp, _i, _vp, _vp, _i, _vp]),
+    "mx_groupnorm_nhwc_from_partials_cat": (_i, [_vp, _vp, _i, _vp, _vp, _vp, _vp, _i, _i, _i, _i, _i, C.c_float, _i, _vp, _vp, _i, _vp, _vp, _vp, _i, _vp]),
     "mx_unet_patch_cache_bytes": (_sz, [_vp, _i, _i, _i, _i]),
     "mx_mmdit_patch_cache_bytes": (_sz, [_vp, _i, _i, _i, _i, _i]),
     "mx_mmdit_workspace_bytes_cached_mixed": (_sz, [_vp, C.POINTER(UNetGroup), _i, _i, _i]),
diff --git a/sduss_amd/ops.py b/sduss_amd/ops.py
--- a/sduss_amd/ops.py
+++ b/sduss_amd/ops.py
@@ -21,7 +21,7 @@
          rowbias: Optional[torch.Tensor] = None, rows_per_batch: int = 0, silu: bool = False, geglu: bool = False,
          out_f32: bool = False, out_scale: float = 0.0, ln_stats: Optional[torch.Tensor] = None, ln_colsum: Optional[torch.Tensor] = None,
          ln_eps: float = 1e-5, want_stats: bool = False, splitk: int = 0, ln_final: Optional[torch.Tensor] = None, want_final: bool = False,
-         final_buffers=None):
+         final_buffers=None, want_gn_partials: bool = False):
     l = _lib.load()
     _bf16(a); _bf16(w)
     m, k = a.shape
@@ -58,7 +58,13 @@
                     final = torch.full((m, 2), float("nan"), dtype=torch.float32, device=a.device)
                     cnt = torch.zeros((m + 255) // 256, dtype=torch.int32, device=a.device)
                 d.ln_final_out, d.ln_final_cnt, d.ln_eps = final.data_ptr(), cnt.data_ptr(), ln_eps
+    part = None
+    if want_gn_partials and l.mx_gemm_gn_partials_supported(C.byref(d), 0):
+        part = torch.full((m // 64, n, 2), float("nan"), dtype=torch.float32, device=a.device)
+        d.gn_part_out = part.data_ptr()
     _lib.check(l.mx_gemm(_lib.current_stream(), C.byref(d)), "mx_gemm")
+    if want_gn_partials:
+        return c, part
     if want_stats:
         if not d.stats_out:
             _lib.check(l.mx_row_stats(_lib.current_stream(), c.data_ptr(), nout, stats.data_ptr(), m, nout), "mx_row_stats")
@@ -258,6 +264,21 @@
     return y
 
 
+def groupnorm_nhwc_from_partials_cat(x: torch.Tensor, x2: torch.Tensor, gamma: torch.Tensor, beta: torch.Tensor, groups: int, eps: float, silu: bool,
+                                     part: torch.Tensor, part2: torch.Tensor, chunk: int = 64, add_bias: Optional[torch.Tensor] = None,
+                                     add_bias2: Optional[torch.Tensor] = None) -> torch.Tensor:
+    l = _lib.load()
+    _bf16(x); _bf16(x2)
+    b, h, w, c1 = x.shape
+    c = c1 + x2.shape[3]
+    y = torch.empty((b, h, w, c), dtype=torch.bfloat16, device=x.device)
+    ws = torch.empty(l.mx_groupnorm_nhwc_workspace_bytes(b, h, w, c), dtype=torch.uint8, device=x.device)
+    _lib.check(l.mx_groupnorm_nhwc_from_partials_cat(_lib.current_stream(), x.data_ptr(), c1, x2.data_ptr(), y.data_ptr(), gamma.data_ptr(), beta.data_ptr(), b, h, w, c,
+                                                     groups, eps, 1 if silu else 0, part.data_ptr(), part2.data_ptr(), chunk, _p(add_bias), _p(add_bias2), None, 0,
+                                                     ws.data_ptr()), "mx_groupnorm_nhwc_from_partials_cat")
+    return y
+
+
 def groupnorm_nhwc(x: torch.Tensor, gamma: torch.Tensor, beta: torch.Tensor, groups: int, eps: float, silu: bool,
                    patch: int = 0) -> torch.Tensor:
     l = _lib.load()
```
